# jdm365/SuffixArray

Hardware: AMD Instinct MI355X
Metric: sa_build_chars_per_s (higher is better)
Workload: dtype u8 text / u32 narrow keys / u32 suffix indices / i64 output

## Files before the change

### suffixarray_amd/csrc/big_build.hpp

```cpp
#pragma once
#include "sa_build.hpp"

namespace sa {
namespace big {

constexpr int BG_BLOCK = 512;
constexpr int BG_ITEMS = 16;
constexpr u32 BG_TILE = BG_BLOCK * BG_ITEMS;
constexpr int BG_WAVES = BG_BLOCK / WAVE;

__global__ __launch_bounds__(BG_BLOCK) void bg_hist_kernel(const u64* __restrict__ keys, u64 cnt, int shift, u32 ntiles, u32* __restrict__ th) {
    constexpr int CS = 257;
    __shared__ u32 s_h[8 * CS];
    for (int i = threadIdx.x; i < 8 * CS; i += BG_BLOCK) s_h[i] = 0;
    __syncthreads();
    u32* my = s_h + (threadIdx.x & 7) * CS;
    const u64 base = (u64)blockIdx.x * BG_TILE;
#pragma unroll 4
    for (int it = 0; it < BG_ITEMS; ++it) {
        const u64 j = base + (u64)it * BG_BLOCK + threadIdx.x;
        if (j < cnt) atomicAdd(&my[(u32)(keys[j] >> shift) & 255u], 1u);
    }
    sync_lds();
    if (threadIdx.x < 256) {
// ... 294 lines not shown
                ok = ea ? !eb : (!eb && inv[a + 1] < inv[b + 1]);
            }
        }
        if (!ok) atomicAdd(bad, 1ull);
    }
}

struct BigStats {
    u32 sigma = 0, bits_per_symbol = 0, initial_chars = 0, sort_passes = 0, rounds = 0;
    u64 tied_after_sort = 0, tied_total = 0;
    float total_ms = 0.f;
};

struct BigBuilder {
    hipStream_t stream = nullptr;
    DevBuf keysA, keysB, idxB, isa, th, off, part, fpart, small;
    DevBuf l_slot[2], l_idx[2], l_gid[2], r_key2, r_perm, r_k1, r_p1, r_gk, r_nk2;
    BigStats stats;

    void destroy() {
        DevBuf* all[] = {&keysA, &keysB, &idxB, &isa, &th, &off, &part, &fpart, &small, &l_slot[0], &l_slot[1], &l_idx[0], &l_idx[1], &l_gid[0],
                         &l_gid[1], &r_key2, &r_perm, &r_k1, &r_p1, &r_gk, &r_nk2};
        for (DevBuf* b : all) b->release();
    }
    ~BigBuilder() { destroy(); }

    int sort_pairs(u64* k0, u64* v0, u64* k1, u64* v1, u64 cnt, int bits, u64** kres, u64** vres) {
        *kres = k0; *vres = v0;
        if (cnt < 2 || bits <= 0) return 0;
        const u64 nt64 = (cnt + BG_TILE - 1) / BG_TILE;
        if (nt64 > 0x7FFFFFFFull) return fail(SA_HIP_EINVAL, "big sort: too many tiles");
        const u32 ntiles = (u32)nt64;
        const u64 len = (u64)RADIX * ntiles;
        const u64 nparts = (len + SC_TILE - 1) / SC_TILE;
        int rc;
        if ((rc = th.ensure(len * 4 + 64))) return rc;
        if ((rc = off.ensure(len * 8 + 64))) return rc;
        if ((rc = part.ensure((nparts + 1) * 8 + 64))) return rc;
        u64 *ki = k0, *vi = v0, *ko = k1, *vo = v1;
        for (int shift = 0; shift < bits; shift += 8) {
            hipLaunchKernelGGL(bg_hist_kernel, dim3(ntiles), dim3(BG_BLOCK), 0, stream, (const u64*)ki, cnt, shift, ntiles, th.as<u32>());
            hipLaunchKernelGGL(bg_scan_reduce_kernel, dim3((u32)nparts), dim3(SC_BLOCK), 0, stream, (const u32*)th.as<u32>(), len, part.as<u64>());
            hipLaunchKernelGGL(bg_scan_parts_kernel, dim3(1), dim3(SC_BLOCK), 0, stream, part.as<u64>(), nparts);
            hipLaunchKernelGGL(bg_scan_apply_kernel, dim3((u32)nparts), dim3(SC_BLOCK), 0, stream, (const u32*)th.as<u32>(), len, (const u64*)part.as<u64>(),
                               off.as<u64>());
            hipLaunchKernelGGL(bg_scatter_kernel, dim3(ntiles), dim3(BG_BLOCK), 0, stream, (const u64*)ki, (const u64*)vi, ko, vo, cnt, shift, ntiles,
                               (const u64*)off.as<u64>());
            u64* t = ki; ki = ko; ko = t;
            t = vi; vi = vo; vo = t;
            ++stats.sort_passes;
        }
        SA_HIP_CHECK(hipGetLastError());
        *kres = ki; *vres = vi;
        return 0;
    }

    int flags_pass(const u64* kA, const u64* kB, const u64* slot, const u64* idx, u64 m, int out, u64* m_out, u64* g_out) {
        const u64 nt64 = (m + BG_TILE - 1) / BG_TILE;
        if (nt64 > 0x7FFFFFFFull) return fail(SA_HIP_EINVAL, "big flags: too many tiles");
        const u32 ntiles = (u32)nt64;
        int rc;
        if ((rc = fpart.ensure(((size_t)ntiles + 1) * sizeof(FlagAgg) + 64))) return rc;
        FlagArgs a{};
        a.kA = kA; a.kB = kB; a.slot = slot; a.idx = idx; a.m = m; a.isa = isa.as<u64>();
        hipLaunchKernelGGL(bg_flags_reduce_kernel, dim3(ntiles), dim3(BG_BLOCK), 0, stream, a, fpart.as<FlagAgg>());
        hipLaunchKernelGGL(bg_flags_scan_kernel, dim3(1), dim3(BG_BLOCK), 0, stream, fpart.as<FlagAgg>(), (u64)ntiles);
        FlagAgg tot;
        SA_HIP_CHECK(hipMemcpyAsync(&tot, fpart.as<FlagAgg>() + ntiles, sizeof tot, hipMemcpyDeviceToHost, stream));
        SA_HIP_CHECK(hipStreamSynchronize(stream));
        *m_out = tot.nact; *g_out = tot.nhead;
        if ((rc = l_slot[out].ensure((size_t)tot.nact * 8 + 64))) return rc;
        if ((rc = l_idx[out].ensure((size_t)tot.nact * 8 + 64))) return rc;
        if ((rc = l_gid[out].ensure((size_t)tot.nact * 8 + 64))) return rc;
        a.out_slot = l_slot[out].as<u64>(); a.out_idx = l_idx[out].as<u64>(); a.out_gid = l_gid[out].as<u64>();
        hipLaunchKernelGGL(bg_flags_apply_kernel, dim3(ntiles), dim3(BG_BLOCK), 0, stream, a, (const FlagAgg*)fpart.as<FlagAgg>());
        SA_HIP_CHECK(hipGetLastError());
        return 0;
    }

    int build(const u8* text_dev, u64 n, u64* sa_out) {
        return build_with(n, sa_out, [&](u64* keys, u64* idx, int* key_bits, u64* h0) -> int {
            u64* dh = small.as<u64>();
            SA_HIP_CHECK(hipMemsetAsync(dh, 0, 256 * sizeof(u64), stream));
            hipLaunchKernelGGL(byte_hist_kernel, dim3(stream_grid(n, 256 * 64)), dim3(256), 0, stream, text_dev, n, dh);
            u64 freq[256];
            SA_HIP_CHECK(hipMemcpyAsync(freq, dh, sizeof freq, hipMemcpyDeviceToHost, stream));
            SA_HIP_CHECK(hipStreamSynchronize(stream));
            CodeMap map;
            memset(&map, 0, sizeof map);
            u32 sigma = 0;
            for (int c = 0; c < 256; ++c) if (freq[c]) map.code[c] = (u16)(++sigma);
            int b = bits_for((u64)sigma + 1);
            if (b == 0) b = 1;
            int k = 64 / b;
            if ((u64)k > n) k = (int)n;
            if (k < 1) k = 1;
            stats.sigma = sigma; stats.bits_per_symbol = (u32)b; stats.initial_chars = (u32)k;
            hipLaunchKernelGGL(bg_keygen_kernel, dim3((u32)((n + 4095) / 4096)), dim3(256), 0, stream, text_dev, n, map, b, k, keys, idx);
            *key_bits = k * b;
            *h0 = (u64)k;
            return 0;
        });
    }

    template <class KeyGen>
    int build_with(u64 n, u64* sa_out, KeyGen&& keygen) {
        stats = BigStats{};
        if (n == 0) return 0;
        int rc;
        hipEvent_t e0 = nullptr, e1 = nullptr;
        SA_HIP_CHECK(hipEventCreate(&e0));
        SA_HIP_CHECK(hipEventCreate(&e1));
        struct EvGuard { hipEvent_t a, b; ~EvGuard() { (void)hipEventDestroy(a); (void)hipEventDestroy(b); } } guard{e0, e1};
        if ((rc = small.ensure(4096))) return rc;
        if ((rc = keysA.ensure(n * 8 + 64))) return rc;
        if ((rc = keysB.ensure(n * 8 + 64))) return rc;
        if ((rc = idxB.ensure(n * 8 + 64))) return rc;
        if ((rc = isa.ensure(n * 8 + 64))) return rc;
        {
            const u64 ntiles = (n + BG_TILE - 1) / BG_TILE, len = (u64)RADIX * ntiles;
            if ((rc = th.ensure(len * 4 + 64)) || (rc = off.ensure(len * 8 + 64)) || (rc = part.ensure(((len + SC_TILE - 1) / SC_TILE + 1) * 8 + 64)) ||
                (rc = fpart.ensure((ntiles + 1) * sizeof(FlagAgg) + 64))) return rc;
        }
        SA_HIP_CHECK(hipEventRecord(e0, stream));
        int key_bits = 0;
        u64 h0 = 1;
        if ((rc = keygen(keysA.as<u64>(), sa_out, &key_bits, &h0))) return rc;
        if (h0 < 1) h0 = 1;
        u64 *kres, *vres;
        if ((rc = sort_pairs(keysA.as<u64>(), sa_out, keysB.as<u64>(), idxB.as<u64>(), n, key_bits, &kres, &vres))) return rc;
        if (vres != sa_out) SA_HIP_CHECK(hipMemcpyAsync(sa_out, vres, n * 8, hipMemcpyDeviceToDevice, stream));
        u64 M = 0, G = 0;
        int cur = 0;
        if ((rc = flags_pass(kres, nullptr, nullptr, sa_out, n, cur, &M, &G))) return rc;
        stats.tied_after_sort = M;
        keysA.release(); keysB.release(); idxB.release(); th.release(); off.release();
        const int rbits = bits_for(n + 2);
        for (u64 h = h0; M > 0; h *= 2) {
            stats.tied_total += M;
            ++stats.rounds;
            if ((rc = r_key2.ensure(M * 8 + 64)) || (rc = r_perm.ensure(M * 8 + 64)) || (rc = r_k1.ensure(M * 8 + 64)) || (rc = r_p1.ensure(M * 8 + 64)) ||
                (rc = r_gk.ensure(M * 8 + 64)) || (rc = r_nk2.ensure(M * 8 + 64))) return rc;
            const u32 grid = stream_grid(M, 1024);
            hipLaunchKernelGGL(bg_key2_kernel, dim3(grid), dim3(256), 0, stream, (const u64*)l_idx[cur].as<u64>(), M, n, h, (const u64*)isa.as<u64>(),
                               r_key2.as<u64>(), r_perm.as<u64>());
            SA_HIP_CHECK(hipMemcpyAsync(r_gk.p, r_key2.p, M * 8, hipMemcpyDeviceToDevice, stream));
            u64 *k1, *p1;
            if ((rc = sort_pairs(r_gk.as<u64>(), r_perm.as<u64>(), r_k1.as<u64>(), r_p1.as<u64>(), M, rbits, &k1, &p1))) return rc;
            u64* gk = (k1 == r_gk.as<u64>()) ? r_k1.as<u64>() : r_gk.as<u64>();
            u64* pfree = (p1 == r_perm.as<u64>()) ? r_p1.as<u64>() : r_perm.as<u64>();
            hipLaunchKernelGGL(bg_gather_kernel, dim3(grid), dim3(256), 0, stream, (const u64*)l_gid[cur].as<u64>(), (const u64*)p1, M, gk);
            u64 *k2, *p2;
            if ((rc = sort_pairs(gk, p1, k1, pfree, M, bits_for(G + 1), &k2, &p2))) return rc;
            const int nxt = cur ^ 1;
            if ((rc = l_idx[nxt].ensure(M * 8 + 64))) return rc;
            hipLaunchKernelGGL(bg_permute_kernel, dim3(grid), dim3(256), 0, stream, (const u64*)l_idx[cur].as<u64>(), (const u64*)r_key2.as<u64>(),
                               (const u64*)p2, (const u64*)l_slot[cur].as<u64>(), M, l_idx[nxt].as<u64>(), r_nk2.as<u64>(), sa_out);
            SA_HIP_CHECK(hipMemcpyAsync(r_perm.p, l_idx[nxt].p, M * 8, hipMemcpyDeviceToDevice, stream));
            u64 M2 = 0, G2 = 0;
            if ((rc = flags_pass(l_gid[cur].as<u64>(), r_nk2.as<u64>(), l_slot[cur].as<u64>(), r_perm.as<u64>(), M, nxt, &M2, &G2))) return rc;
            M = M2; G = G2; cur = nxt;
            if (h > n) break;
        }
        SA_HIP_CHECK(hipEventRecord(e1, stream));
        SA_HIP_CHECK(hipStreamSynchronize(stream));
        (void)hipEventElapsedTime(&stats.total_ms, e0, e1);
        if (M) return fail(SA_HIP_EHIP, "big build: rounds ended with tied suffixes");
// ... 27 lines not shown
```

### suffixarray_amd/csrc/common.hpp

```cpp
#pragma once
#include <hip/hip_runtime.h>
#include <cstdint>
#include <cstdio>
#include <cstdlib>
#include <cstring>
#include <string>
#include <new>

#include "../../include/sa_hip.h"

namespace sa {

using u8 = uint8_t;
using u16 = uint16_t;
using u32 = uint32_t;
using u64 = uint64_t;

constexpr int WAVE = 64;

inline std::string& last_error() {
    static thread_local std::string s;
    return s;
}
inline int fail(int code, const char* what, const char* detail = nullptr) {
    std::string& e = last_error();
    e = what;
    if (detail) { e += ": "; e += detail; }
    return code;
}

#define SA_HIP_CHECK(expr)                                                                 \
    do {                                                                                   \
        hipError_t _e = (expr);                                                            \
        if (_e != hipSuccess) {                                                            \
            char _b[256];                                                                  \
            snprintf(_b, sizeof _b, "%s:%d %s", __FILE__, __LINE__, hipGetErrorString(_e)); \
            return ::sa::fail(_e == hipErrorOutOfMemory ? SA_HIP_ENOMEM : SA_HIP_EHIP, #expr, _b); \
        }                                                                                  \
    } while (0)

__host__ __device__ inline u32 div_up(u64 a, u64 b) { return (u32)((a + b - 1) / b); }

__host__ __device__ __forceinline__ u32 hits_of_range(const sa_hip_pair_u32 rg) {
    return (rg.first != 0xFFFFFFFFu && (u32)(rg.second - rg.first + 1u) != 0u) ? rg.second - rg.first + 1u : 0u;
}

inline int bits_for(u64 count) {
    int b = 0;
    while (b < 64 && (1ull << b) < count) ++b;
    return b;
}

#if defined(__HIPCC__)
__device__ __forceinline__ u64 lanemask_lt() {
    return (1ull << (threadIdx.x & 63)) - 1ull;
}

__device__ __forceinline__ void sync_lds() {
    asm volatile("s_waitcnt lgkmcnt(0)" ::: "memory");
    __syncthreads();
}
#endif

struct HostU64Array {
    u64* p = nullptr;
    size_t n = 0;
    HostU64Array() = default;
    HostU64Array(const HostU64Array&) = delete;
    HostU64Array& operator=(const HostU64Array&) = delete;
    ~HostU64Array() { free(p); }
    void clear() { free(p); p = nullptr; n = 0; }
    void adopt(u64* malloced, size_t count) { clear(); p = malloced; n = count; }
    void assign(const u64* first, const u64* last) {
        const size_t count = (size_t)(last - first);
        u64* q = static_cast<u64*>(malloc((count ? count : 1) * sizeof(u64)));
        if (!q) throw std::bad_alloc();
        if (count) memcpy(q, first, count * sizeof(u64));
        clear(); p = q; n = count;
    }
    size_t size() const { return n; }
    bool empty() const { return n == 0; }
    const u64* data() const { return p; }
    const u64* begin() const { return p; }
    const u64* end() const { return p + n; }
    const u64& operator[](size_t i) const { return p[i]; }
    const u64& back() const { return p[n - 1]; }
};

inline const char* diag_env(const char* name) {
    static const bool on = [] { const char* d = getenv("SA_HIP_DIAG"); return d && atoi(d) != 0; }();
    return on ? getenv(name) : nullptr;
}

struct CodeMap {
    u16 code[256];
};

struct DeviceStatus {
    u32 error;
    u32 pad[3];
};

}
```

### suffixarray_amd/csrc/radix_narrow.hpp

```cpp
#pragma once
#include "radix_sort.hpp"
#include <vector>

namespace sa {

constexpr int NARROW_MAX_PASSES = 6;
constexpr int SEG_ITEMS = 24;

struct SegPlan {
    u32 bstart[RADIX + 1];
    u32 tprefix[RADIX + 1];
    u32 cfirst[NCHUNK + 1];
};

__global__ __launch_bounds__(256) void seg_plan_kernel(const u32* __restrict__ hist_top, u32 tile, SegPlan* __restrict__ plan) {
    __shared__ uint2 s_w[4];
    __shared__ u32 s_tp[RADIX + 1];
    const int d = threadIdx.x;
    u32 size = 0;
#pragma unroll
    for (int c = 0; c < NCHUNK; ++c) size += hist_top[c * RADIX + d];
    const u32 tiles = (u32)(((u64)size + tile - 1) / tile);
    uint2 tot;
    const uint2 ex = block_scan_excl<4>(make_uint2(size, tiles), make_uint2(0, 0), ScanSum{}, s_w, &tot);
// ... 195 lines not shown
        }
    }
    sync_lds();
    if (has_next) {
        for (int i = tid; i < RADIX; i += BLOCK) {
            const u32 v = s_whist[i];
            if (v) atomicAdd(&a.next_hist[bucket * RADIX + i], v);
        }
    }
    if (LATEV) load_vals();
    u32* s_vals = s_keys;
#pragma unroll
    for (int j = 0; j < ITEMS; ++j)
        if (FULL || (woff + j * WAVE) < tile_n) s_vals[pos[j]] = val[j];
    __syncthreads();
    if (LAST && a.vals_out64) {
#pragma unroll
        for (int k = 0; k < ITEMS; ++k) {
            const u32 p = k * BLOCK + tid;
            if (FULL || p < tile_n) { const u32 v = s_vals[p]; a.vals_out[gidx[k]] = v; a.vals_out64[gidx[k]] = (int64_t)v; }
        }
        return;
    }
#pragma unroll
    for (int k = 0; k < ITEMS; ++k) {
        const u32 p = k * BLOCK + tid;
        if (FULL || p < tile_n) a.vals_out[gidx[k]] = s_vals[p];
    }
}

template <int BLOCK, int ITEMS, bool LAST, bool LATEV = true>
__global__ __launch_bounds__(BLOCK, (ITEMS > 16) ? 4 : (LATEV ? 6 : 4)) void seg_onesweep_kernel(SegPassArgs a) {
    constexpr int WAVES = BLOCK / WAVE;
    constexpr u32 TILE = BLOCK * ITEMS;
    __shared__ __attribute__((aligned(16))) u32 s_keys[TILE];
    __shared__ u32 s_whist[WAVES * RADIX];
    __shared__ u32 s_gdelta[RADIX];
    __shared__ u32 s_wsum[RADIX / WAVE];
    __shared__ u32 s_t[RADIX + 1];
    __shared__ u32 s_b[RADIX + 1];
    __shared__ u32 s_c[NCHUNK + 1];
    __shared__ u32 s_flat;

    const int tid = threadIdx.x;
    u32 home = 0, t_home = 0;
    if (tid == 0) {
        home = xcc_id();
        t_home = atomicAdd(&a.ticket[home], 1u);
    }
    for (int i = tid; i <= RADIX; i += BLOCK) { s_t[i] = a.plan->tprefix[i]; s_b[i] = a.plan->bstart[i]; }
    if (tid <= NCHUNK) s_c[tid] = a.plan->cfirst[tid];
    for (int i = tid; i < WAVES * RADIX; i += BLOCK) s_whist[i] = 0;
    __syncthreads();
    if (tid == 0) {
        u32 flat = 0xFFFFFFFFu;
        if (t_home < s_c[home + 1] - s_c[home]) flat = s_c[home] + t_home;
        for (int k = 1; k < NCHUNK && flat == 0xFFFFFFFFu; ++k) {
            const u32 c = (home + k) & (NCHUNK - 1);
            const u32 cnt = s_c[c + 1] - s_c[c];
            if (cnt == 0) continue;
            const u32 t = atomicAdd(&a.ticket[c], 1u);
            if (t < cnt) flat = s_c[c] + t;
        }
        s_flat = flat;
    }
    __syncthreads();
    const u32 flat = s_flat;
    if (flat == 0xFFFFFFFFu) return;
    const u32 bucket = seg_bucket_of(s_t, flat);
    const u32 first_flat = s_t[bucket];
    const u32 start = s_b[bucket] + (flat - first_flat) * TILE;
    const u32 rest = s_b[bucket + 1] - start;
    if (rest >= TILE)
        seg_tile<true, BLOCK, ITEMS, LAST, LATEV>(a, flat, first_flat, bucket, start, TILE, s_keys, s_whist, s_gdelta, s_wsum);
    else
        seg_tile<false, BLOCK, ITEMS, LAST, LATEV>(a, flat, first_flat, bucket, start, rest, s_keys, s_whist, s_gdelta, s_wsum);
}

}
#include "radix_split.hpp"
namespace sa {

constexpr int TOP_HIST_COPIES = 8;
template <int C8>
__global__ __launch_bounds__(256) void top_hist_kernel(const u8* __restrict__ text, const u16* __restrict__ map, u64 n, int b,
                                                       SortGeom g, u32* __restrict__ hist, int low_k0 = 0) {
    constexpr int CS = RADIX + 1;
    constexpr u32 SPAN = 256 * 16;
    __shared__ u32 s_h[TOP_HIST_COPIES * CS];
    __shared__ u8 s_map[256];
    s_map[threadIdx.x] = (u8)map[threadIdx.x];
    for (int i = threadIdx.x; i < TOP_HIST_COPIES * CS; i += 256) s_h[i] = 0;
    __syncthreads();
    u32* my = s_h + (threadIdx.x & (TOP_HIST_COPIES - 1)) * CS;
    constexpr int c8 = C8;
    const u32 wmask = (1u << (c8 * b)) - 1u;
    const int dshift = c8 * b - 8;
    const u64 nspans = (n + SPAN - 1) / SPAN;
    const u64 per = (nspans + gridDim.x - 1) / gridDim.x;
    const u64 s_lo = (u64)blockIdx.x * per;
    const u64 s_hi = (s_lo + per < nspans) ? s_lo + per : nspans;
    auto flush = [&](u32 chunk) {
        sync_lds();
        u32 v = 0;
#pragma unroll
        for (int k = 0; k < TOP_HIST_COPIES; ++k) { v += s_h[k * CS + threadIdx.x]; s_h[k * CS + threadIdx.x] = 0; }
        if (v) atomicAdd(&hist[chunk * RADIX + threadIdx.x], v);
        sync_lds();
    };
    if (s_lo >= s_hi) return;
    u32 cur = chunk_of_tile((u32)((s_lo * SPAN) / g.tile), g.tpc);
    for (u64 sp = s_lo; sp < s_hi; ++sp) {
        const u64 base = sp * SPAN;
        const u32 c = chunk_of_tile((u32)(base / g.tile), g.tpc);
        if (c != cur) { flush(cur); cur = c; }
        const u64 p0 = base + (u64)threadIdx.x * 16;
        if (p0 < n) {
            const u64 off = low_k0 ? (u64)(low_k0 - c8) : 0;
            uint4 x0, x1;
            __builtin_memcpy(&x0, text + p0 + off, 16);
            __builtin_memcpy(&x1, text + p0 + off + 16, 16);
            const u32 w[8] = {x0.x, x0.y, x0.z, x0.w, x1.x, x1.y, x1.z, x1.w};
            const u64 first = p0 + off;
            const u32 live = (first >= n) ? 0u : ((n - first < 32) ? (u32)(n - first) : 32u);
            const u32 npos = (n - p0 < 16) ? (u32)(n - p0) : 16u;
            u32 win = 0;
#pragma unroll
            for (int k = 0; k < 16 + c8 - 1; ++k) {
                const u32 byte = (w[k >> 2] >> ((k & 3) * 8)) & 255u;
                const u32 code = ((u32)k < live) ? (u32)s_map[byte] : 0u;
                win = ((win << b) | code) & wmask;
                const int i = k - (c8 - 1);
                if (i >= 0 && (u32)i < npos) atomicAdd(&my[low_k0 ? (win & 255u) : (win >> dshift)], 1u);
            }
        }
    }
    flush(cur);
}

struct TextPassArgs {
    const u8* text;
    const u16* map;
    u64 n;
    int b, k0, begin_bit;
    u32* keys_out32;
    u16* ext_out16;
    u32* vals_out;
    SortGeom g;
    const u32* digit_base;
    u64* status;
    u32* ticket;
    u32 epoch;
    DeviceStatus* dstat;
    u32 incl_mask;
    u32* cursor;
    int owned;
};
constexpr u32 TOP_CURSOR_STRIDE = 64;
constexpr int TEXT_HALO = 64;
#ifndef SA_TEXT_ITEMS
#define SA_TEXT_ITEMS 16
#endif
constexpr int TEXT_ITEMS = SA_TEXT_ITEMS;
constexpr u32 TEXT_TILE = 512u * TEXT_ITEMS;

__device__ __forceinline__ void shl_or_inplace(u32& acc, u32 x, int s) {
    asm("v_lshl_or_b32 %0, %1, %2, %0" : "+v"(acc) : "v"(x), "s"(s));
}

template <bool FULL, int BLOCK, bool EXT, bool CLAIM = false>
__device__ __forceinline__ void text_top_tile(const TextPassArgs& a, const u32 tile, const u32 chunk,
                                              const u32 tile_n, u32* s_keys, u32* s_whist, u32* s_gdelta, u32* s_wsum,
                                              u8* s_code, const u8* s_map, u16* s_ext) {
    constexpr int WAVES = BLOCK / WAVE;
    constexpr int ITEMS = TEXT_ITEMS;
    constexpr u32 TILE = BLOCK * ITEMS;
    static_assert(TILE % 16 == 0, "16-byte text loads");
    const int tid = threadIdx.x, lane = tid & 63, wave = tid >> 6;
    const u32 first_tile = chunk * a.g.tpc;
    const u64 tile_base = (u64)tile * TILE;
    const u32 woff = (u32)wave * (WAVE * ITEMS) + lane;

    const u32 dbase = (tid < RADIX) ? a.digit_base[(CLAIM ? 0u : chunk) * RADIX + tid] : 0u;

    auto stage16 = [&](u32 local, auto checked) {
        constexpr bool CHECK = decltype(checked)::value;
        const u64 p0 = tile_base + local;
        uint4 x = make_uint4(0, 0, 0, 0);
        if (!CHECK || p0 < a.n) x = *reinterpret_cast<const uint4*>(a.text + p0);
        const u32 w[4] = {x.x, x.y, x.z, x.w};
        const u32 live = CHECK ? (u32)((a.n > p0) ? ((a.n - p0 < 16) ? (a.n - p0) : 16) : 0) : 16u;
        u32 o[4] = {0, 0, 0, 0};
#pragma unroll
        for (int k = 0; k < 16; ++k) {
            const u32 byte = (w[k >> 2] >> ((k & 3) * 8)) & 255u;
            const u32 code = (!CHECK || (u32)k < live) ? (u32)s_map[byte] : 0u;
            o[k >> 2] |= code << ((k & 3) * 8);
        }
        *reinterpret_cast<uint4*>(s_code + local) = make_uint4(o[0], o[1], o[2], o[3]);
    };
    for (u32 local = (u32)tid * 16u; local < TILE; local += BLOCK * 16u) {
        if (FULL) stage16(local, std::false_type{}); else stage16(local, std::true_type{});
    }
    if (tid < TEXT_HALO / 16) stage16(TILE + (u32)tid * 16u, std::true_type{});
    __syncthreads();

    u32 hi[ITEMS], lo[ITEMS];
#pragma unroll
    for (int j = 0; j < ITEMS; ++j) { hi[j] = 0; lo[j] = 0; }
    const u8* cp = s_code + woff;
    {
        int c = 0;
        for (; c < a.k0 && 64 - a.b * (c + 1) >= 32; ++c, ++cp) {
            const int s_hi = 32 - a.b * (c + 1);
#pragma unroll
            for (int j = 0; j < ITEMS; ++j) shl_or_inplace(hi[j], (u32)cp[j * WAVE], s_hi);
        }
        if (c < a.k0 && 64 - a.b * c > 32) {
            const int sh = 64 - a.b * (c + 1);
#pragma unroll
            for (int j = 0; j < ITEMS; ++j) {
                const u32 code = cp[j * WAVE];
                hi[j] |= code >> (32 - sh);
                lo[j] |= code << sh;
            }
            ++c; ++cp;
        }
        for (; c < a.k0; ++c, ++cp) {
            const int sh = 64 - a.b * (c + 1);
#pragma unroll
            for (int j = 0; j < ITEMS; ++j) shl_or_inplace(lo[j], (u32)cp[j * WAVE], sh);
        }
    }
    u32 key[ITEMS];
    u32 ext[EXT ? ITEMS : 1];
    const int kb0 = EXT ? a.begin_bit + 16 : a.begin_bit;
#pragma unroll
    for (int j = 0; j < ITEMS; ++j) {
        key[j] = (kb0 >= 32) ? (hi[j] >> (kb0 - 32)) : __builtin_amdgcn_alignbit(hi[j], lo[j], (u32)kb0);
// ... 28 lines not shown
    if (tid < RADIX) {
        for (int i = 0; i < wave; ++i) excl += s_wsum[i];
#pragma unroll
        for (int w = 0; w < WAVES; ++w) s_whist[w * RADIX + tid] += excl;
    }
    __syncthreads();

    u8* s_dig = s_code;
    u32 pos[ITEMS];
#pragma unroll
    for (int j = 0; j < ITEMS; ++j) {
        const u32 d = rd[j] >> 16;
        pos[j] = wh[d] + (rd[j] & 0xFFFFu);
        if (FULL || (woff + j * WAVE) < tile_n) {
            s_keys[pos[j]] = key[j]; s_dig[pos[j]] = (u8)d;
            if (EXT) s_ext[pos[j]] = (u16)ext[j];
        }
    }
    __syncthreads();

    if (tid < RADIX) {
        u32 prefix = claim;
        if (!CLAIM && tile > first_tile) {
            prefix = lookback_prefix(a.status, tile, first_tile, (u32)tid, a.epoch, a.dstat);
            if (((tile - first_tile) & a.incl_mask) == a.incl_mask)
                __hip_atomic_store(&a.status[(u64)tile * RADIX + tid], pack_status(a.epoch, FLAG_INCL, prefix + count),
                                   __ATOMIC_RELAXED, __HIP_MEMORY_SCOPE_AGENT);
        }
        s_gdelta[tid] = dbase + prefix - excl;
    }
    __syncthreads();

    u32 gidx[ITEMS];
#pragma unroll
    for (int k = 0; k < ITEMS; ++k) {
        const u32 p = k * BLOCK + tid;
        if (FULL || p < tile_n) {
            gidx[k] = s_gdelta[s_dig[p]] + p;
            a.keys_out32[gidx[k]] = s_keys[p];
            if (EXT) a.ext_out16[gidx[k]] = s_ext[p];
        }
    }
    __syncthreads();
    u32* s_vals = s_keys;
#pragma unroll
    for (int j = 0; j < ITEMS; ++j)
        if (FULL || (woff + j * WAVE) < tile_n) s_vals[pos[j]] = (u32)tile_base + woff + j * WAVE;
    __syncthreads();
#pragma unroll
    for (int k = 0; k < ITEMS; ++k) {
        const u32 p = k * BLOCK + tid;
        if (FULL || p < tile_n) a.vals_out[gidx[k]] = s_vals[p];
    }
}

constexpr int TOP_OWNED_W = 24;
constexpr int TOP_OWNED_KMAX = TOP_OWNED_W - 15;
constexpr int TOP_FINE_BITS = 3;
constexpr u32 TOP_FINE_BINS = (u32)RADIX << TOP_FINE_BITS;
inline bool text_owned_applies(int b, int k0) { return k0 >= 1 && k0 <= TOP_OWNED_KMAX && b * k0 >= 8 + TOP_FINE_BITS && b * k0 <= 40; }

template <bool FULL, int BLOCK>
__device__ __forceinline__ void text_top_owned_tile(const TextPassArgs& a, const u32 tile, const u32 chunk, const u32 tile_n, u32* s_keys,
                                                    u32* s_fine, u32* s_gdelta, u32* s_wsum, u8* s_dig, const u8* s_map) {
    constexpr int ITEMS = 16, W = TOP_OWNED_W, F = TOP_FINE_BITS;
    constexpr u32 TILE = BLOCK * ITEMS;
    static_assert(TEXT_ITEMS == ITEMS, "the tiles of the pass's geometry");
    static_assert(TOP_FINE_BINS == 4u * BLOCK, "four fine bins per thread");
    static_assert((TILE & (TILE - 1)) == 0 && TILE <= (1u << 13) && 8 + F + 13 <= 32, "(fine bin, rank) in one register");
    static_assert(W % 4 == 0 && W > 16 && W <= 32, "a 16-byte load and a shorter one");
    const int tid = threadIdx.x, lane = tid & 63, wave = tid >> 6;
    const u64 tile_base = (u64)tile * TILE;
    const u32 own = (u32)tid * ITEMS;

    const u32 cd = chunk * RADIX + (u32)(tid >> 1);
    const u32 dbase = (tid & 1) ? 0u : a.digit_base[cd];

    const long long start = (long long)(tile_base + own) + (a.k0 - (W - 15));
    const long long n = (long long)a.n;
    u32 x[W / 4];
#pragma unroll
    for (int i = 0; i < W / 4; ++i) x[i] = 0;
    if (start >= 0) {
        if (FULL || start < n) __builtin_memcpy(&x[0], a.text + start, 16);
        if (FULL || start + 16 < n) __builtin_memcpy(&x[4], a.text + start + 16, W - 16);
    } else {
#pragma unroll
        for (int i = 0; i < W; ++i) {
            const long long q = start + i;
            if (q >= 0 && q < n) x[i >> 2] |= (u32)a.text[q] << ((i & 3) * 8);
        }
    }
    const u32 live = FULL ? (u32)W : (u32)((start >= n) ? 0 : ((n - start < W) ? (n - start) : W));

    const u32 up = 32u - (u32)a.b;
    const u32 fshift = (u32)(a.b * a.k0 - 8 - F);
    const u32 kmask = (a.b * a.k0 >= 32) ? 0xFFFFFFFFu : ((1u << (a.b * a.k0)) - 1u);
    u32 whi = 0, wlo = 0;
    u32 key[ITEMS], pk[ITEMS];
#pragma unroll
    for (int i = 0; i < W; ++i) {
        const u32 byte = (x[i >> 2] >> ((i & 3) * 8)) & 255u;
        const u32 code = (FULL || (u32)i < live) ? (u32)s_map[byte] : 0u;
        whi = __builtin_amdgcn_alignbit(whi, wlo, up);
        wlo = (wlo << a.b) | code;
        if (i >= W - ITEMS) {
            const int j = i - (W - ITEMS);
            key[j] = wlo & kmask;
            const u32 fine = __builtin_amdgcn_alignbit(whi, wlo, fshift) & (TOP_FINE_BINS - 1u);
            const u32 slot = (FULL || own + (u32)j < tile_n) ? fine : TOP_FINE_BINS;
            pk[j] = (fine << 13) | atomicAdd(&s_fine[slot], 1u);
        }
    }
    sync_lds();

    const uint4 c = *reinterpret_cast<const uint4*>(s_fine + 4 * tid);
    const u32 tot = c.x + c.y + c.z + c.w;
    const u32 dcount = tot + __shfl_xor(tot, 1);
    u32 claim = 0;
    if (!(tid & 1) && dcount) claim = atomicAdd(&a.cursor[cd * TOP_CURSOR_STRIDE], dcount);
    const u32 incl = wave_scan_incl(tot, ScanSum{});
    if (lane == 63) s_wsum[wave] = incl;
    __syncthreads();
    u32 excl = incl - tot;
    for (int i = 0; i < wave; ++i) excl += s_wsum[i];
    *reinterpret_cast<uint4*>(s_fine + 4 * tid) = make_uint4(excl, excl + c.x, excl + c.x + c.y, excl + c.x + c.y + c.z);
    __syncthreads();

    u32 pos[ITEMS];
#pragma unroll
    for (int j = 0; j < ITEMS; ++j) {
        const u32 fine = pk[j] >> 13;
        pos[j] = (s_fine[fine] + (pk[j] & 0x1FFFu)) & (TILE - 1u);
        if (FULL || own + (u32)j < tile_n) { s_keys[pos[j]] = key[j]; s_dig[pos[j]] = (u8)(fine >> F); }
    }
    if (!(tid & 1)) s_gdelta[tid >> 1] = dbase + claim - excl;
    __syncthreads();

    u32 gidx[ITEMS];
#pragma unroll
    for (int k = 0; k < ITEMS; ++k) {
        const u32 p = k * BLOCK + tid;
        if (FULL || p < tile_n) {
            gidx[k] = s_gdelta[s_dig[p]] + p;
            a.keys_out32[gidx[k]] = s_keys[p];
        }
    }
    __syncthreads();
    u32* s_vals = s_keys;
#pragma unroll
    for (int j = 0; j < ITEMS; ++j)
        if (FULL || own + (u32)j < tile_n) s_vals[pos[j]] = (u32)tile_base + own + (u32)j;
    __syncthreads();
#pragma unroll
    for (int k = 0; k < ITEMS; ++k) {
        const u32 p = k * BLOCK + tid;
        if (FULL || p < tile_n) a.vals_out[gidx[k]] = s_vals[p];
    }
}

template <int BLOCK, bool EXT = false, bool CLAIM = false>
__global__ __launch_bounds__(BLOCK, (TEXT_ITEMS > 16 || EXT) ? 4 : 6) void text_top_pass_kernel(TextPassArgs a) {
    constexpr int WAVES = BLOCK / WAVE;
    constexpr u32 TILE = BLOCK * TEXT_ITEMS;
    __shared__ __attribute__((aligned(16))) u32 s_keys[TILE];
    __shared__ __attribute__((aligned(16))) u32 s_whist[WAVES * RADIX + 4];
    __shared__ u32 s_gdelta[RADIX];
    __shared__ u32 s_wsum[WAVES];
// ... 189 lines not shown
            }
        }
    }
    sync_lds();
    if (has_next) {
        for (int i = tid; i < NCHUNK * RADIX; i += BLOCK) {
            const u32 v = s_whist[i];
            if (v) atomicAdd(&a.next_hist[i], v);
        }
    }
    u32* s_vals = reinterpret_cast<u32*>(s_keys);
#pragma unroll
    for (int j = 0; j < ITEMS; ++j)
        if (FULL || (woff + j * WAVE) < tile_n) s_vals[pos[j]] = (u32)tile_base + woff + j * WAVE;
    __syncthreads();
#pragma unroll
    for (int k = 0; k < ITEMS; ++k) {
        const u32 p = k * BLOCK + tid;
        if (FULL || p < tile_n) a.vals_out[gidx[k]] = s_vals[p];
    }
}

template <int BLOCK>
__global__ __launch_bounds__(BLOCK, 4) void text_low_pass_kernel(TextLowArgs t) {
    constexpr int WAVES = BLOCK / WAVE;
    constexpr u32 TILE = BLOCK * SORT_ITEMS;
    constexpr int WH = (WAVES * RADIX > NCHUNK * RADIX) ? WAVES * RADIX : NCHUNK * RADIX;
    static_assert(TILE * 8 >= TILE + TEXT_HALO, "the staged codes fit the key array's LDS");
    __shared__ __attribute__((aligned(16))) u64 s_keys[TILE];
    __shared__ u32 s_whist[WH];
    __shared__ uint2 s_tab[RADIX];
    __shared__ u32 s_wsum[RADIX / WAVE];
    __shared__ u8 s_map[256];
    __shared__ u32 s_tile;
    __shared__ u32 s_chunk;
    const SortPassArgs& a = t.p;
    const int tid = threadIdx.x;
    if (tid == 0) {
        u32 tile = 0xFFFFFFFFu, chunk = 0;
        const u32 home = xcc_id();
        for (int k = 0; k < NCHUNK; ++k) {
            const u32 c = (home + k) & (NCHUNK - 1);
            const u32 first = c * a.g.tpc;
            if (first >= a.g.tiles) continue;
            const u32 cnt = (a.g.tiles - first) < a.g.tpc ? (a.g.tiles - first) : a.g.tpc;
            const u32 x = atomicAdd(&a.ticket[c], 1u);
            if (x < cnt) { tile = first + x; chunk = c; break; }
        }
        s_tile = tile;
        s_chunk = chunk;
    }
    if (tid < 256) s_map[tid] = (u8)t.map[tid];
    for (int i = tid; i < WAVES * RADIX; i += BLOCK) s_whist[i] = 0;
    __syncthreads();
    const u32 tile = s_tile;
    if (tile == 0xFFFFFFFFu) return;
    const u32 chunk = s_chunk;
    const u64 rest = t.n - (u64)tile * TILE;
    if (rest >= (u64)TILE)
        text_low_tile<true, BLOCK>(t, tile, chunk, TILE, s_keys, s_whist, s_tab, s_wsum, s_map);
    else
        text_low_tile<false, BLOCK>(t, tile, chunk, (u32)rest, s_keys, s_whist, s_tab, s_wsum, s_map);
}

struct NarrowWorkspace {
    SegPlan* plan = nullptr;
    u32* hist = nullptr;
    u32* base = nullptr;
    u32* tickets = nullptr;
    u16* map_dev = nullptr;
    CodeMap map_host;
    bool split_enabled = true;
    u32* split_hist = nullptr;
    u32* split_base = nullptr;
    u32* split_cursor = nullptr;
    u32* top_cursor = nullptr;
    static size_t top_cursor_bytes() { return (size_t)NCHUNK * RADIX * TOP_CURSOR_STRIDE * sizeof(u32); }
    bool top_claims = true;
    bool top_owned = true;
    u32* split_sub = nullptr;
    u32* host_word = nullptr;
    static size_t split_table_bytes() { return (size_t)RADIX * SPLIT_NB * sizeof(u32); }
    static size_t split_sub_words() { return ((size_t)RADIX << SPLIT_BITS) + 1; }
    u32* split_levels_dev() const { return split_sub + split_sub_words(); }
    u32 split_cap = LOCAL_CAP;
    int local_bin_bits = 12;
    bool split_flags = true;
    bool local_big = false;
    bool local_persist = true;
    u32 local_grid_force = 0;
    u32 local_grid[6] = {};
    int persist_grid(const void* kernel, int block, int slot, u32 nsub, u32* grid) {
        if (!local_grid[slot]) {
            int dev = 0, cus = 0, per_cu = 0;
            SA_HIP_CHECK(hipGetDevice(&dev));
            SA_HIP_CHECK(hipDeviceGetAttribute(&cus, hipDeviceAttributeMultiprocessorCount, dev));
            SA_HIP_CHECK(hipOccupancyMaxActiveBlocksPerMultiprocessor(&per_cu, kernel, block, 0));
            local_grid[slot] = (u32)((per_cu > 0 ? per_cu : 1) * (cus > 0 ? cus : 1));
        }
        const u32 g = local_grid_force ? local_grid_force : local_grid[slot];
        *grid = g < nsub ? g : nsub;
        return 0;
    }
    int split_items = 28;
    static size_t hist_bytes() { return (size_t)NARROW_MAX_PASSES * RADIX * RADIX * sizeof(u32); }
    int init() {
        SA_HIP_CHECK(hipMalloc(&plan, sizeof(SegPlan)));
        SA_HIP_CHECK(hipMalloc(&hist, hist_bytes()));
        SA_HIP_CHECK(hipMalloc(&base, (size_t)RADIX * RADIX * sizeof(u32)));
        SA_HIP_CHECK(hipMalloc(&tickets, (size_t)NARROW_MAX_PASSES * NCHUNK * sizeof(u32)));
        SA_HIP_CHECK(hipMalloc(&map_dev, sizeof(CodeMap)));
        SA_HIP_CHECK(hipMalloc(&split_hist, split_table_bytes()));
        SA_HIP_CHECK(hipMalloc(&split_base, split_table_bytes()));
        SA_HIP_CHECK(hipMalloc(&split_cursor, split_table_bytes()));
        SA_HIP_CHECK(hipMalloc(&top_cursor, top_cursor_bytes()));
        SA_HIP_CHECK(hipMalloc(&split_sub, (split_sub_words() + 16) * sizeof(u32)));
        SA_HIP_CHECK(hipHostMalloc(reinterpret_cast<void**>(&host_word), 64, hipHostMallocDefault));
        if (const char* e = diag_env("SA_HIP_SPLIT")) split_enabled = atoi(e) != 0;
        if (const char* e = diag_env("SA_HIP_TOP_CLAIMS")) top_claims = atoi(e) != 0;
        if (const char* e = diag_env("SA_HIP_TOP_OWNED")) top_owned = atoi(e) != 0;
        if (const char* e = diag_env("SA_HIP_LOCAL_BIG")) local_big = atoi(e) != 0;
        if (const char* e = diag_env("SA_HIP_LOCAL_PERSIST")) local_persist = atoi(e) != 0;
        if (const char* e = diag_env("SA_HIP_LOCAL_GRID")) { const int v = atoi(e); local_grid_force = v > 0 ? (u32)v : 0u; }
        if (const char* e = diag_env("SA_HIP_SPLIT_FLAGS")) split_flags = atoi(e) != 0;
        if (const char* e = diag_env("SA_HIP_LOCAL_BINS")) local_bin_bits = (atoi(e) == 11) ? 11 : 12;
        if (const char* e = diag_env("SA_HIP_SPLIT_ITEMS")) { const int v = atoi(e); split_items = (v == 24 || v == 28) ? v : 32; }
        if (const char* e = diag_env("SA_HIP_SPLIT_CAP")) { const int v = atoi(e); if (v >= 64 && v <= (int)LOCAL_CAP) split_cap = (u32)v; }
        return 0;
    }
    void destroy() {
        if (plan) (void)hipFree(plan);
        if (hist) (void)hipFree(hist);
        if (base) (void)hipFree(base);
        if (tickets) (void)hipFree(tickets);
        if (map_dev) (void)hipFree(map_dev);
        if (split_hist) (void)hipFree(split_hist);
        if (split_base) (void)hipFree(split_base);
        if (split_cursor) (void)hipFree(split_cursor);
        if (top_cursor) (void)hipFree(top_cursor);
        if (split_sub) (void)hipFree(split_sub);
        if (host_word) (void)hipHostFree(host_word);
        map_dev = nullptr;
        plan = nullptr; hist = nullptr; base = nullptr; tickets = nullptr;
        split_hist = split_base = split_sub = split_cursor = top_cursor = nullptr; host_word = nullptr;
    }
};

inline bool narrow_sort_applies(const RadixWorkspace& ws, u64 n, int begin_bit) {
    return ws.block == 512 && begin_bit >= 24 && begin_bit < 56 && n >= (1u << 22) &&
           n / ws.tile() + RADIX + 1 <= ws.max_tiles;
}

struct TextSource {
    const u8* text;
    int b, k0;
};
inline bool text_pass_applies(int b, int k0) { return b <= 8 && k0 - 1 <= TEXT_HALO; }

inline int text_histogram(RadixWorkspace& ws, NarrowWorkspace& nw, hipStream_t stream, const u8* text, const CodeMap& map,
                          u32 n, int b, u32 tile, int low_k0) {
    nw.map_host = map;
    SA_HIP_CHECK(hipMemcpyAsync(nw.map_dev, nw.map_host.code, sizeof(CodeMap), hipMemcpyHostToDevice, stream));
    const SortGeom g = make_geom(n, tile);
    const u32 spans = div_up(n, 4096);
    const dim3 grid(spans < 2048u ? spans : 2048u), block(256);
    decltype(&top_hist_kernel<1>) kernel;
    switch ((8 + b - 1) / b) {
        case 1: kernel = top_hist_kernel<1>; break;
        case 2: kernel = top_hist_kernel<2>; break;
        case 3: kernel = top_hist_kernel<3>; break;
        case 4: kernel = top_hist_kernel<4>; break;
        default: kernel = top_hist_kernel<8>; break;
    }
    hipLaunchKernelGGL(kernel, grid, block, 0, stream, text, nw.map_dev, (u64)n, b, g, ws.hist(0), low_k0);
    return 0;
}

struct WideTextCtx {
    const u8* text;
    const u16* map;
    u64 n;
    int b, k0;
};
inline void launch_text_low_pass(void* ctx, hipStream_t stream, const SortPassArgs& a, u32 grid) {
    const WideTextCtx* c = static_cast<const WideTextCtx*>(ctx);
    TextLowArgs t;
    t.p = a; t.text = c->text; t.map = c->map; t.n = c->n; t.b = c->b; t.k0 = c->k0;
    hipLaunchKernelGGL((text_low_pass_kernel<512>), dim3(grid), dim3(512), 0, stream, t);
}

enum TopForm { TOP_STABLE, TOP_CLAIM, TOP_EXT };
inline int launch_text_top(RadixWorkspace& ws, NarrowWorkspace& nw, hipStream_t stream, const TextSource& src, u32 n, int begin_bit,
                           TopForm form, u32* keys_out32, u16* ext_out16, u32* vals_out) {
    const bool claim = form == TOP_CLAIM, ext = form == TOP_EXT;
    const SortGeom g = make_geom(n, TEXT_TILE);
    TextPassArgs t;
    t.text = src.text; t.map = nw.map_dev; t.n = n; t.b = src.b; t.k0 = src.k0; t.begin_bit = begin_bit;
    t.keys_out32 = keys_out32; t.ext_out16 = ext_out16; t.vals_out = vals_out; t.g = g; t.digit_base = ws.base();
    t.status = ws.status; t.ticket = ws.tickets(); t.epoch = ws.epoch; t.dstat = ws.dstat; t.incl_mask = SA_INCL_MASK;
    t.cursor = ext ? nullptr : nw.top_cursor;
    t.owned = (claim && nw.top_owned && TEXT_ITEMS == 16 && text_owned_applies(src.b, src.k0)) ? 1 : 0;
    if (claim) SA_HIP_CHECK(hipMemsetAsync(nw.top_cursor, 0, NarrowWorkspace::top_cursor_bytes(), stream));
    return ws.timed_pass(stream, 1, n, (u64)n * (ext ? 11u : 9u), [&] {
        if (claim) hipLaunchKernelGGL((text_top_pass_kernel<512, false, true>), dim3(g.tiles), dim3(512), 0, stream, t);
        else if (!ext) hipLaunchKernelGGL((text_top_pass_kernel<512>), dim3(g.tiles), dim3(512), 0, stream, t);
        else hipLaunchKernelGGL((text_top_pass_kernel<512, true>), dim3(g.tiles), dim3(512), 0, stream, t);
    });
}

struct NarrowSortResult {
    u64* keys = nullptr;
    u32* vals = nullptr;
    int rb = 0;
    u32 max_group = 0;
    bool flags_done = false;
};

inline int narrow_top_digit(RadixWorkspace& ws, NarrowWorkspace& nw, hipStream_t stream, const u64* keys_in, u32* keys_out32, u32* vals_out,
                            u32 n, int begin_bit, const TextSource* src, bool claim) {
    int rc;
    if ((rc = ws.next_epoch(stream))) return rc;
    hipLaunchKernelGGL(radix_scan_hist_kernel, dim3(1), dim3(256), 0, stream, ws.hist(0), ws.base());
    if (src) return launch_text_top(ws, nw, stream, *src, n, begin_bit, claim ? TOP_CLAIM : TOP_STABLE, keys_out32, nullptr, vals_out);
    SortPassArgs a;
    a.keys_in = keys_in; a.vals_in = nullptr; a.keys_out = nullptr; a.vals_out = vals_out;
    a.g = make_geom(n, ws.tile()); a.shift = 56; a.mask = 255u; a.next_shift = -1; a.next_mask = 0; a.digit_base = ws.base();
    a.next_hist = nullptr; a.status = ws.status; a.ticket = ws.tickets(); a.epoch = ws.epoch; a.dstat = ws.dstat;
    a.home_mode = 0; a.incl_mask = SA_INCL_MASK;
    a.keys_out32 = keys_out32; a.narrow_shift = begin_bit;
    return ws.timed_pass(stream, 1, n, (u64)n * 16u, [&] {
        hipLaunchKernelGGL((radix_onesweep_kernel<512, 0, true>), dim3(a.g.tiles), dim3(512), 0, stream, a);
    });
}

struct SplitKernels {
    using Hist = decltype(&split_hist_kernel<512, 24>);
    using Split = decltype(&seg_split_kernel<512, 24>);
    Hist hist;
    Split split;
};
inline SplitKernels split_kernels(int split_items) {
    const int i = (split_items == 32) ? 0 : (split_items == 28) ? 1 : 2;
    static const SplitKernels::Hist hist[3] = {split_hist_kernel<512, 32>, split_hist_kernel<512, 28>, split_hist_kernel<512, 24>};
    static const SplitKernels::Split split[3] = {seg_split_kernel<512, 32>, seg_split_kernel<512, 28>, seg_split_kernel<512, 24>};
    return {hist[i], split[i]};
}

struct SplitLevel {
    int rb;
    bool big;
};
inline SplitLevel choose_split_level(const u32* host_word, int hb, int lo_bits, u32 split_cap, bool local_big) {
    int rb = -1;
    bool big = local_big;
    if (!big)
        for (int k = 1; k <= hb; ++k)
            if (host_word[k] <= split_cap) { rb = k; break; }
    if (rb < 0 && split_cap == LOCAL_CAP) {
        for (int k = 1; k <= hb; ++k)
            if (host_word[k] <= LOCAL_CAP_BIG && lo_bits - k >= 12) { rb = k; big = true; break; }
        if (rb < 0) big = false;
    }
    return {rb, big};
}

inline int narrow_plan_look(NarrowWorkspace& nw, hipStream_t stream, const u32* keys32, int lo_bits, int hb, u32 split_flat_max,
                            SplitLevel* level) {
    SA_HIP_CHECK(hipMemsetAsync(nw.split_hist, 0, NarrowWorkspace::split_table_bytes(), stream));
    SA_HIP_CHECK(hipMemsetAsync(nw.split_levels_dev(), 0, 16 * sizeof(u32), stream));
    const u32 tpb = 4;
    hipLaunchKernelGGL(split_kernels(nw.split_items).hist, dim3(div_up(split_flat_max, tpb)), dim3(512), 0, stream, keys32, nw.plan,
                       lo_bits - hb, (1u << hb) - 1u, nw.split_hist, tpb);
    hipLaunchKernelGGL(split_levels_kernel, dim3(RADIX), dim3(SPLIT_NB), 0, stream, (const u32*)nw.split_hist, hb, nw.split_levels_dev());
    SA_HIP_CHECK(hipMemcpyAsync(nw.host_word, nw.split_levels_dev(), 16 * sizeof(u32), hipMemcpyDeviceToHost, stream));
    SA_HIP_CHECK(hipStreamSynchronize(stream));
    *level = choose_split_level(nw.host_word, hb, lo_bits, nw.split_cap, nw.local_big);
    return 0;
}

inline int narrow_split_pass(RadixWorkspace& ws, NarrowWorkspace& nw, hipStream_t stream, const u32* keys_in, const u32* vals_in,
                             u32* keys_out, u32* vals_out, u32 n, int lo_bits, int hb, int rb, u32 split_flat_max) {
    int rc;
    hipLaunchKernelGGL(split_scan_kernel, dim3(RADIX), dim3(SPLIT_NB), 0, stream, (const u32*)nw.split_hist, nw.plan, hb, rb,
                       nw.split_base, nw.split_sub);
    SA_HIP_CHECK(hipMemsetAsync(nw.split_cursor, 0, NarrowWorkspace::split_table_bytes(), stream));
    if ((rc = ws.next_epoch(stream))) return rc;
    SplitPassArgs a;
    a.keys_in = keys_in; a.vals_in = vals_in;
    a.keys_out = keys_out; a.vals_out = vals_out;
    a.plan = nw.plan; a.shift = lo_bits - rb; a.mask = (1u << rb) - 1u; a.digit_base = nw.split_base;
    a.ticket = nw.tickets; a.cursor = nw.split_cursor;
    return ws.timed_pass(stream, 2, n, (u64)n * 16u, [&] {
        hipLaunchKernelGGL(split_kernels(nw.split_items).split, dim3(split_flat_max), dim3(512), 0, stream, a);
    });
}

struct LocalKernels {
    using Persist = decltype(&local_persist_kernel<12, true>);
    using Finish = decltype(&local_finish_kernel<12, true>);
    Persist persist;
    Finish finish;
    int block, row;
};
inline LocalKernels local_kernels(bool big, bool flags, int bb) {
    const int row = big ? (flags ? 0 : 1) : 2 + (flags ? 0 : 2) + (bb == 12 ? 0 : 1);
    static const LocalKernels::Persist persist[6] = {
        local_persist_kernel<12, true, LOCAL_BLOCK_BIG>, local_persist_kernel<12, false, LOCAL_BLOCK_BIG>,
        local_persist_kernel<12, true>, local_persist_kernel<11, true>, local_persist_kernel<12, false>, local_persist_kernel<11, false>};
    static const LocalKernels::Finish finish[6] = {
        local_finish_kernel<12, true, LOCAL_BLOCK_BIG>, local_finish_kernel<12, false, LOCAL_BLOCK_BIG>,
        local_finish_kernel<12, true>, local_finish_kernel<11, true>, local_finish_kernel<12, false>, local_finish_kernel<11, false>};
    return {persist[row], finish[row], big ? LOCAL_BLOCK_BIG : LOCAL_BLOCK, row};
}

inline int narrow_local_pass(RadixWorkspace& ws, NarrowWorkspace& nw, hipStream_t stream, const u32* keys_in, const u32* vals_in,
                             u32* keys_out, u32* vals_out, int64_t* vals_out64, u32 n, int begin_bit, int rb, bool big,
                             const LocalFlagsRequest* flags_req, bool* flags_done) {
    int rc;
    const int lo_bits = 56 - begin_bit;
    const int rest_bits = lo_bits - rb;
    LocalArgs l;
    l.keys_in = keys_in; l.vals_in = vals_in;
    l.keys_out = keys_out; l.vals_out = vals_out; l.vals_out64 = vals_out64;
    l.sub = nw.split_sub;
    const int bb = (big || (rest_bits >= 12 && nw.local_bin_bits == 12)) ? 12 : 11;
    l.bin_shift = rest_bits - bb;
    l.dstat = ws.dstat;
    l.dir = DirArgs{}; l.counts = nullptr; l.lite = LiteArgs{}; l.lo_shift = begin_bit; l.rb = rb; l.n = n;
    const u32 nsub = (u32)RADIX << rb;
    bool with_flags = false;
    if (nw.split_flags && flags_req && flags_req->prepare) {
        const int fr = flags_req->prepare(flags_req->ctx, nsub, &l);
        if (fr < 0) return fr;
        with_flags = (fr == 0) && l.dir.dir && l.dir.dbits >= 8 + rb && l.dir.dbits - 8 - rb <= bb && l.dir.dbits - 8 <= lo_bits;
    }
    const LocalKernels k = local_kernels(big, with_flags, bb);
    u32 pgrid = 0;
    if (nw.local_persist && (rc = nw.persist_grid(reinterpret_cast<const void*>(k.persist), k.block, k.row, nsub, &pgrid))) return rc;
    rc = ws.timed_pass(stream, 3, n, (u64)n * 16u + (vals_out64 ? (u64)n * 8u : 0u), [&] {
        if (nw.local_persist) hipLaunchKernelGGL(k.persist, dim3(pgrid), dim3(k.block), 0, stream, l, (const u32*)nw.split_sub, nsub, nw.tickets + NCHUNK, LOCAL_RUN);
        else hipLaunchKernelGGL(k.finish, dim3(nsub), dim3(k.block), 0, stream, l);
    });
    if (rc) return rc;
    *flags_done = with_flags;
    SA_HIP_CHECK(hipGetLastError());
    return 0;
}

inline int split_debug_check(NarrowWorkspace& nw, hipStream_t stream, const u32* keys_split, const u32* keys_out, const u32* vals_out,
                             u32 n, int lo_bits, int hb, int rb) {
    const int dshift = lo_bits - rb;
    const u32 dmask = (1u << rb) - 1u;
    const u32 nsub = (u32)RADIX << rb;
    std::vector<u32> sub(nsub + 1), k1(n), k2(n), v2(n), bst(RADIX + 1);
    SA_HIP_CHECK(hipStreamSynchronize(stream));
    SA_HIP_CHECK(hipMemcpy(sub.data(), nw.split_sub, (size_t)(nsub + 1) * 4, hipMemcpyDeviceToHost));
    SA_HIP_CHECK(hipMemcpy(k1.data(), keys_split, (size_t)n * 4, hipMemcpyDeviceToHost));
    SA_HIP_CHECK(hipMemcpy(k2.data(), keys_out, (size_t)n * 4, hipMemcpyDeviceToHost));
    SA_HIP_CHECK(hipMemcpy(v2.data(), vals_out, (size_t)n * 4, hipMemcpyDeviceToHost));
    SA_HIP_CHECK(hipMemcpy(bst.data(), nw.plan->bstart, (size_t)(RADIX + 1) * 4, hipMemcpyDeviceToHost));
    u64 bad_sub = 0, bad_split = 0, bad_sorted = 0, bad_mono = 0;
    u32 first_split = ~0u, first_sorted = ~0u;
    for (u32 i = 0; i < nsub; ++i) {
        if (sub[i] > sub[i + 1] || sub[i + 1] > n) { ++bad_mono; continue; }
        if ((i & (((u32)1 << rb) - 1)) == 0 && sub[i] != bst[i >> rb]) ++bad_sub;
        for (u32 j = sub[i]; j < sub[i + 1]; ++j) {
            if (((k1[j] >> dshift) & dmask) != (i & dmask)) { ++bad_split; if (first_split == ~0u) first_split = j; }
            if (j > sub[i] && (k2[j - 1] > k2[j] || (k2[j - 1] == k2[j] && v2[j - 1] >= v2[j]))) { ++bad_sorted; if (first_sorted == ~0u) first_sorted = j; }
        }
    }
    fprintf(stderr, "[sa_hip] split debug: n=%u rb=%d hb=%d nsub=%u sub[0]=%u sub[last]=%u | table: %llu not monotone, %llu off the bucket starts | split pass: %llu records in the wrong group (first %u) | local pass: %llu out of order (first %u)\n",
            n, rb, hb, nsub, sub[0], sub[nsub], (unsigned long long)bad_mono, (unsigned long long)bad_sub, (unsigned long long)bad_split, first_split,
            (unsigned long long)bad_sorted, first_sorted);
    return 0;
}

inline int narrow_declined(RadixWorkspace& ws, NarrowWorkspace& nw, hipStream_t stream, u32* keys_out32, u32* vals_out, u32 n,
                           int begin_bit, const TextSource* src, bool top_claimed, u32 split_tile_n, u32 seg_tile_n) {
    int rc;
    if (top_claimed) {
        SA_HIP_CHECK(hipMemsetAsync(ws.tickets(), 0, NCHUNK * sizeof(u32), stream));
        if ((rc = ws.next_epoch(stream))) return rc;
        if ((rc = launch_text_top(ws, nw, stream, *src, n, begin_bit, TOP_STABLE, keys_out32, nullptr, vals_out))) return rc;
    }
    if (split_tile_n != seg_tile_n)
        hipLaunchKernelGGL(seg_plan_kernel, dim3(1), dim3(256), 0, stream, ws.hist(0), seg_tile_n, nw.plan);
    return 0;
}

inline int narrow_lsd_passes(RadixWorkspace& ws, NarrowWorkspace& nw, hipStream_t stream, u64* keysA, u32* valsA, u64* keysB, u32* valsB,
                             u32 n, int begin_bit, bool keep_narrow, int64_t* vals_res64, NarrowSortResult* res) {
    int rc;
    const int lo_bits = 56 - begin_bit;
    const int np = (lo_bits + RADIX_BITS - 1) / RADIX_BITS;
    const u32 flat_max = n / (512u * SEG_ITEMS) + 1 + RADIX;
    SA_HIP_CHECK(hipMemsetAsync(nw.hist, 0, NarrowWorkspace::hist_bytes(), stream));
    {
        const u32 tpb = 4;
        const u32 mask0 = (1u << ((np == 1) ? lo_bits : RADIX_BITS)) - 1u;
        hipLaunchKernelGGL((seg_hist_kernel<512, SEG_ITEMS>), dim3(div_up(flat_max, tpb)), dim3(512), 0, stream,
                           reinterpret_cast<const u32*>(keysB), nw.plan, 0, mask0, nw.hist, tpb);
    }
    u32* kin = reinterpret_cast<u32*>(keysB); u32* vin = valsB;
    u32* kout = reinterpret_cast<u32*>(keysA); u32* vout = valsA;
    for (int p = 0; p < np; ++p) {
        if ((rc = ws.next_epoch(stream))) return rc;
        const bool last = (p == np - 1);
        const int bits_p = last ? (lo_bits - RADIX_BITS * (np - 1)) : RADIX_BITS;
        hipLaunchKernelGGL(seg_scan_kernel, dim3(RADIX), dim3(256), 0, stream, nw.hist + (size_t)p * RADIX * RADIX, nw.plan, nw.base);
        SegPassArgs a;
        a.keys_in = kin; a.vals_in = vin; a.keys_out = kout; a.keys_out64 = keep_narrow ? nullptr : reinterpret_cast<u64*>(kout);
        a.vals_out = vout;
        a.vals_out64 = last ? vals_res64 : nullptr;
        a.plan = nw.plan;
        a.shift = RADIX_BITS * p;
        a.mask = (1u << bits_p) - 1u;
        a.next_shift = last ? -1 : RADIX_BITS * (p + 1);
        const int bits_n = (p + 1 == np - 1) ? (lo_bits - RADIX_BITS * (np - 1)) : RADIX_BITS;
        a.next_mask = last ? 0u : ((1u << bits_n) - 1u);
        a.digit_base = nw.base;
        a.next_hist = last ? nullptr : nw.hist + (size_t)(p + 1) * RADIX * RADIX;
        a.status = ws.status; a.ticket = nw.tickets + p * NCHUNK; a.epoch = ws.epoch; a.dstat = ws.dstat;
        a.lo_shift = begin_bit; a.incl_mask = SA_INCL_MASK;
        const u64 pass_bytes = (u64)n * ((last && !keep_narrow) ? 20u : 16u) + ((last && vals_res64) ? (u64)n * 8u : 0u);
        rc = ws.timed_pass(stream, last ? 3 : 2, n, pass_bytes, [&] {
            if (last) hipLaunchKernelGGL((seg_onesweep_kernel<512, SEG_ITEMS, true>), dim3(flat_max), dim3(512), 0, stream, a);
            else hipLaunchKernelGGL((seg_onesweep_kernel<512, SEG_ITEMS, false>), dim3(flat_max), dim3(512), 0, stream, a);
        });
        if (rc) return rc;
        std::swap(kin, kout);
        std::swap(vin, vout);
    }
    SA_HIP_CHECK(hipGetLastError());
    res->keys = reinterpret_cast<u64*>(kin);
    res->vals = vin;
    return 0;
}

inline int radix_sort_narrow(RadixWorkspace& ws, NarrowWorkspace& nw, hipStream_t stream, u64* keysA, u32* valsA, u64* keysB,
                             u32* valsB, u32 n, int begin_bit, NarrowSortResult* res, const TextSource* src = nullptr,
                             bool keep_narrow = false, int64_t* vals_res64 = nullptr, const LocalFlagsRequest* flags_req = nullptr) {
    int rc;
    *res = NarrowSortResult{};
    const int lo_bits = 56 - begin_bit;
    u32* const k32A = reinterpret_cast<u32*>(keysA);
    u32* const k32B = reinterpret_cast<u32*>(keysB);
    SA_HIP_CHECK(hipMemsetAsync(nw.tickets, 0, (size_t)NARROW_MAX_PASSES * NCHUNK * sizeof(u32), stream));
    const bool try_split = nw.split_enabled && keep_narrow && ws.block == 512 && lo_bits - LOCAL_BIN_BITS >= 1;
    const bool optimistic = try_split && src && nw.top_claims;
    if ((rc = narrow_top_digit(ws, nw, stream, keysA, k32B, valsB, n, begin_bit, src, optimistic))) return rc;
    const u32 seg_tile_n = 512u * SEG_ITEMS;
    const u32 split_tile_n = 512u * (u32)nw.split_items;
    hipLaunchKernelGGL(seg_plan_kernel, dim3(1), dim3(256), 0, stream, ws.hist(0), try_split ? split_tile_n : seg_tile_n, nw.plan);
    if (try_split) {
        const int hb = (lo_bits - LOCAL_BIN_BITS < SPLIT_BITS) ? lo_bits - LOCAL_BIN_BITS : SPLIT_BITS;
        const u32 split_flat_max = n / split_tile_n + 1 + RADIX;
        SplitLevel lv;
        if ((rc = narrow_plan_look(nw, stream, k32B, lo_bits, hb, split_flat_max, &lv))) return rc;
        res->max_group = nw.host_word[lv.rb > 0 ? lv.rb : hb];
        if (lv.rb > 0) {
            if ((rc = narrow_split_pass(ws, nw, stream, k32B, valsB, k32A, valsA, n, lo_bits, hb, lv.rb, split_flat_max))) return rc;
            if ((rc = narrow_local_pass(ws, nw, stream, k32A, valsA, k32B, valsB, vals_res64, n, begin_bit, lv.rb, lv.big, flags_req,
                                        &res->flags_done))) return rc;
            if (diag_env("SA_HIP_SPLIT_DEBUG") && (rc = split_debug_check(nw, stream, k32A, k32B, valsB, n, lo_bits, hb, lv.rb))) return rc;
            res->rb = lv.rb;
            res->keys = keysB;
            res->vals = valsB;
            return 0;
        }
        if ((rc = narrow_declined(ws, nw, stream, k32B, valsB, n, begin_bit, src, optimistic, split_tile_n, seg_tile_n))) return rc;
    }
    return narrow_lsd_passes(ws, nw, stream, keysA, valsA, keysB, valsB, n, begin_bit, keep_narrow, vals_res64, res);
}

}
```

### suffixarray_amd/csrc/radix_split.hpp

```cpp
#pragma once
#include "flags_common.hpp"

namespace sa {

#ifndef SA_ABL
#define SA_ABL 0
#endif
constexpr int SPLIT_BITS = 10;
constexpr int SPLIT_NB = 1 << SPLIT_BITS;
constexpr u32 LOCAL_CAP = 8192;
constexpr int LOCAL_BLOCK = 512;
constexpr int LOCAL_ITEMS = (int)(LOCAL_CAP / LOCAL_BLOCK);
constexpr u32 LOCAL_CAP_BIG = 16384;
constexpr int LOCAL_BLOCK_BIG = 1024;
constexpr u32 LOCAL_RUN = 8;
constexpr int LOCAL_BIN_BITS = 11;
constexpr int SPLIT_HIST_COPIES = 4;

template <int BLOCK, int ITEMS>
__global__ __launch_bounds__(BLOCK) void split_hist_kernel(const u32* __restrict__ keys, const SegPlan* __restrict__ plan, int shift,
                                                           u32 mask, u32* __restrict__ hist, u32 tiles_per_block) {
    constexpr u32 TILE = BLOCK * ITEMS;
    constexpr int CS = SPLIT_NB + 1;
    __shared__ u32 s_h[SPLIT_HIST_COPIES * CS];
    __shared__ u32 s_t[RADIX + 1];
    for (int i = threadIdx.x; i <= RADIX; i += BLOCK) s_t[i] = plan->tprefix[i];
    for (int i = threadIdx.x; i < SPLIT_HIST_COPIES * CS; i += BLOCK) s_h[i] = 0;
    __syncthreads();
    const u32 F = s_t[RADIX];
    const u32 f_lo = blockIdx.x * tiles_per_block;
    const u32 f_hi = (f_lo + tiles_per_block < F) ? f_lo + tiles_per_block : F;
    if (f_lo >= f_hi) return;
    u32* my = s_h + (threadIdx.x & (SPLIT_HIST_COPIES - 1)) * CS;
    auto flush = [&](u32 bucket) {
        sync_lds();
        for (int d = threadIdx.x; d < SPLIT_NB; d += BLOCK) {
            u32 v = 0;
#pragma unroll
            for (int k = 0; k < SPLIT_HIST_COPIES; ++k) { v += s_h[k * CS + d]; s_h[k * CS + d] = 0; }
            if (v) atomicAdd(&hist[bucket * SPLIT_NB + d], v);
        }
        sync_lds();
    };
    u32 cur = seg_bucket_of(s_t, f_lo);
    for (u32 f = f_lo; f < f_hi; ++f) {
        const u32 b = seg_bucket_of(s_t, f);
        if (b != cur) { flush(cur); cur = b; }
        const u32 start = plan->bstart[b] + ((f - s_t[b]) * TILE);
        const u32 end = plan->bstart[b + 1];
        const u32 len = (end - start) < TILE ? (end - start) : TILE;
        if (len == TILE) {
            u32 k[ITEMS];
#pragma unroll
            for (int j = 0; j < ITEMS; ++j) k[j] = keys[start + j * BLOCK + threadIdx.x];
#pragma unroll
            for (int j = 0; j < ITEMS; ++j) atomicAdd(&my[(k[j] >> shift) & mask], 1u);
        } else {
            for (u32 l = threadIdx.x; l < len; l += BLOCK) atomicAdd(&my[(keys[start + l] >> shift) & mask], 1u);
        }
    }
    flush(cur);
}

__global__ __launch_bounds__(SPLIT_NB) void split_levels_kernel(const u32* __restrict__ hist, int hb, u32* __restrict__ levels) {
    __shared__ u32 s_p[SPLIT_NB + 1];
    __shared__ u32 s_w[SPLIT_NB / WAVE];
    const int b = blockIdx.x, d = threadIdx.x, lane = d & 63, w = d >> 6;
    const u32 c = hist[b * SPLIT_NB + d];
    s_p[d + 1] = block_scan_excl<SPLIT_NB / WAVE>(c, 0u, ScanSum{}, s_w) + c;
    if (d == 0) s_p[0] = 0;
    __syncthreads();
    __shared__ u32 s_lv[SPLIT_BITS + 1][SPLIT_NB / WAVE];
    for (int k = 0; k <= hb; ++k) {
        const int g = hb - k;
        u32 v = 0;
        if (d < (1 << k)) v = s_p[(d + 1) << g] - s_p[d << g];
#pragma unroll
        for (int o = 32; o > 0; o >>= 1) { const u32 t = __shfl_down(v, o); v = t > v ? t : v; }
        if (lane == 0) s_lv[k][w] = v;
    }
    __syncthreads();
    if (d <= hb) {
        u32 v = 0;
        for (int i = 0; i < SPLIT_NB / WAVE; ++i) v = s_lv[d][i] > v ? s_lv[d][i] : v;
        if (v) atomicMax(&levels[d], v);
    }
}

__global__ __launch_bounds__(SPLIT_NB) void split_scan_kernel(const u32* __restrict__ hist, const SegPlan* __restrict__ plan, int hb, int rb,
                                                              u32* __restrict__ base, u32* __restrict__ sub) {
    __shared__ u32 s_w[SPLIT_NB / WAVE];
    const int b = blockIdx.x, d = threadIdx.x;
    const u32 run = plan->bstart[b] + block_scan_excl<SPLIT_NB / WAVE>(hist[b * SPLIT_NB + d], 0u, ScanSum{}, s_w);
    const int g = hb - rb;
    u32 out = 0;
    if (d < (1 << hb) && (d & ((1 << g) - 1)) == 0) {
        out = run;
        sub[((u32)b << rb) + (u32)(d >> g)] = run;
    }
    __shared__ u32 s_o[SPLIT_NB];
    s_o[d] = 0;
    __syncthreads();
    if (d < (1 << hb) && (d & ((1 << g) - 1)) == 0) s_o[d >> g] = out;
    __syncthreads();
    base[b * SPLIT_NB + d] = s_o[d];
    if (d == 0 && b == RADIX - 1) sub[(u32)RADIX << rb] = plan->bstart[RADIX];
}

struct SplitPassArgs {
    const u32* keys_in;
    const u32* vals_in;
    u32* keys_out;
    u32* vals_out;
    const SegPlan* plan;
    int shift;
    u32 mask;
    const u32* digit_base;
    u32* ticket;
    u32* cursor;
};

template <bool FULL, int BLOCK, int ITEMS>
__device__ __forceinline__ void split_tile(const SplitPassArgs& a, const u32 bucket, const u32 start, const u32 tile_n,
                                           u32* s_keys, u32* s_cnt, u32* s_gdelta, u32* s_wsum) {
    static_assert(SPLIT_NB == 2 * BLOCK, "two bins per thread");
    const int tid = threadIdx.x, lane = tid & 63, wave = tid >> 6;
    const u32 woff = (u32)wave * (WAVE * ITEMS) + lane;

    const uint2 dbase = *reinterpret_cast<const uint2*>(a.digit_base + (size_t)bucket * SPLIT_NB + 2 * tid);

    u32 key[ITEMS];
    const u32* kin = a.keys_in + start;
#pragma unroll
    for (int j = 0; j < ITEMS; ++j) {
        const u32 p = woff + j * WAVE;
        key[j] = (FULL || p < tile_n) ? kin[p] : 0u;
    }
    u32 pos[ITEMS];
#pragma unroll
    for (int j = 0; j < ITEMS; ++j) {
        const u32 d = (key[j] >> a.shift) & a.mask;
        pos[j] = atomicAdd(&s_cnt[(FULL || (woff + j * WAVE) < tile_n) ? d : (u32)SPLIT_NB], 1u);
    }
    sync_lds();

    const uint2 c = *reinterpret_cast<const uint2*>(s_cnt + 2 * tid);
    u32 claim0 = 0, claim1 = 0;
    {
        const u32 ci = bucket * SPLIT_NB + 2u * (u32)tid;
        if (c.x) claim0 = atomicAdd(&a.cursor[ci], c.x);
        if (c.y) claim1 = atomicAdd(&a.cursor[ci + 1], c.y);
    }
    const u32 tot = c.x + c.y;
    const u32 incl = wave_scan_incl(tot, ScanSum{});
    if (lane == 63) s_wsum[wave] = incl;
    __syncthreads();
    u32 excl = incl - tot;
    for (int i = 0; i < wave; ++i) excl += s_wsum[i];
    *reinterpret_cast<uint2*>(s_cnt + 2 * tid) = make_uint2(excl, excl + c.x);
    __syncthreads();

#pragma unroll
    for (int j = 0; j < ITEMS; ++j) {
        pos[j] += s_cnt[(key[j] >> a.shift) & a.mask];
        if (FULL || (woff + j * WAVE) < tile_n) s_keys[pos[j]] = key[j];
    }
    __syncthreads();

    *reinterpret_cast<uint2*>(s_gdelta + 2 * tid) = make_uint2(dbase.x + claim0 - excl, dbase.y + claim1 - (excl + c.x));
    __syncthreads();

    static_assert(ITEMS % 2 == 0 && BLOCK * ITEMS <= 65536, "positions packed as 16-bit pairs");
    u32 pp[ITEMS / 2];
#pragma unroll
    for (int j = 0; j < ITEMS / 2; ++j) pp[j] = pos[2 * j] | (pos[2 * j + 1] << 16);
    u32 gidx[ITEMS];
#pragma unroll
    for (int k = 0; k < ITEMS; ++k) {
        const u32 p = k * BLOCK + tid;
        if (FULL || p < tile_n) {
            const u32 kk = s_keys[p];
            gidx[k] = s_gdelta[(kk >> a.shift) & a.mask] + p;
            a.keys_out[gidx[k]] = kk;
        }
    }
    u32 val[ITEMS];
    const u32* vin = a.vals_in + start;
#pragma unroll
    for (int j = 0; j < ITEMS; ++j) {
        const u32 p = woff + j * WAVE;
        val[j] = (FULL || p < tile_n) ? vin[p] : 0u;
    }
    __syncthreads();
    u32* s_vals = s_keys;
#pragma unroll
    for (int j = 0; j < ITEMS; ++j)
        if (FULL || (woff + j * WAVE) < tile_n) s_vals[(pp[j >> 1] >> ((j & 1) * 16)) & 0xFFFFu] = val[j];
    __syncthreads();
#pragma unroll
    for (int k = 0; k < ITEMS; ++k) {
        const u32 p = k * BLOCK + tid;
        if (FULL || p < tile_n) a.vals_out[gidx[k]] = s_vals[p];
    }
}

template <int BLOCK, int ITEMS>
__global__ __launch_bounds__(BLOCK, 4) void seg_split_kernel(SplitPassArgs a) {
    constexpr u32 TILE = BLOCK * ITEMS;
    __shared__ __attribute__((aligned(16))) u32 s_keys[TILE];
    __shared__ __attribute__((aligned(16))) u32 s_cnt[SPLIT_NB + 4];
    __shared__ __attribute__((aligned(16))) u32 s_gdelta[SPLIT_NB];
    __shared__ u32 s_wsum[BLOCK / WAVE];
    __shared__ u32 s_t[RADIX + 1];
    __shared__ u32 s_b[RADIX + 1];
    __shared__ u32 s_c[NCHUNK + 1];
    __shared__ u32 s_flat;

    const int tid = threadIdx.x;
    u32 home = 0, t_home = 0;
    if (tid == 0) {
        home = xcc_id();
        t_home = atomicAdd(&a.ticket[home], 1u);
    }
    for (int i = tid; i <= RADIX; i += BLOCK) { s_t[i] = a.plan->tprefix[i]; s_b[i] = a.plan->bstart[i]; }
    if (tid <= NCHUNK) s_c[tid] = a.plan->cfirst[tid];
    for (int i = tid; i < SPLIT_NB + 4; i += BLOCK) s_cnt[i] = 0;
    __syncthreads();
    if (tid == 0) {
        u32 flat = 0xFFFFFFFFu;
        if (t_home < s_c[home + 1] - s_c[home]) flat = s_c[home] + t_home;
        for (int k = 1; k < NCHUNK && flat == 0xFFFFFFFFu; ++k) {
            const u32 c = (home + k) & (NCHUNK - 1);
            const u32 cnt = s_c[c + 1] - s_c[c];
            if (cnt == 0) continue;
            const u32 t = atomicAdd(&a.ticket[c], 1u);
            if (t < cnt) flat = s_c[c] + t;
        }
        s_flat = flat;
    }
    __syncthreads();
    const u32 flat = s_flat;
    if (flat == 0xFFFFFFFFu) return;
    const u32 bucket = seg_bucket_of(s_t, flat);
    const u32 first_flat = s_t[bucket];
    const u32 start = s_b[bucket] + (flat - first_flat) * TILE;
    const u32 rest = s_b[bucket + 1] - start;
    if (rest >= TILE) split_tile<true, BLOCK, ITEMS>(a, bucket, start, TILE, s_keys, s_cnt, s_gdelta, s_wsum);
    else split_tile<false, BLOCK, ITEMS>(a, bucket, start, rest, s_keys, s_cnt, s_gdelta, s_wsum);
}

struct LocalArgs {
    const u32* keys_in;
    const u32* vals_in;
    u32* keys_out;
    u32* vals_out;
    int64_t* vals_out64;
    const u32* sub;
    int bin_shift;
    DeviceStatus* dstat;
    DirArgs dir;
    uint2* counts;
    LiteArgs lite;
    int lo_shift;
    int rb;
    u32 n;
};

struct LocalFlagsRequest {
    int (*prepare)(void* ctx, u32 nsub, LocalArgs* l) = nullptr;
    void* ctx = nullptr;
};

template <int BB, bool FLAGS, int BLOCK, bool PERSIST, typename Mid>
__device__ __forceinline__ void local_finish_sub(const LocalArgs& a, const u32 sb, const u32 s, const u32 m, u32 (&key)[LOCAL_ITEMS],
                                                 u32 (&val)[LOCAL_ITEMS], u64* s_rec, u32* s_cw, u32* s_wsum, Mid&& mid) {
    constexpr int ITEMS = LOCAL_ITEMS;
    constexpr int NB = 1 << BB, WORDS = NB / 2, WPT = WORDS / BLOCK;
    const int tid = threadIdx.x, lane = tid & 63, wave = tid >> 6;
    const int g2 = FLAGS ? a.dir.dbits - 8 - a.rb : 0;
    const u32 dfirst = FLAGS ? (sb << g2) : 0u;
    const u32 nd = FLAGS ? (1u << g2) : 0u;

    u32 r[ITEMS];
#pragma unroll
    for (int j = 0; j < ITEMS; ++j) {
        const u32 p = (u32)j * BLOCK + tid;
        r[j] = 0;
        if ((u32)j * BLOCK < m && p < m) {
            const u32 b = (key[j] >> a.bin_shift) & (u32)(NB - 1);
            const u32 sh = (b & 1u) * 16u;
            r[j] = (atomicAdd(&s_cw[b >> 1], 1u << sh) >> sh) & 0xFFFFu;
        }
    }
    sync_lds();

    {
        u32 cw[WPT];
        u32 tot = 0;
#pragma unroll
        for (int i = 0; i < WPT; ++i) { cw[i] = s_cw[WPT * tid + i]; tot += (cw[i] & 0xFFFFu) + (cw[i] >> 16); }
        const u32 incl = wave_scan_incl(tot, ScanSum{});
        if (lane == 63) s_wsum[wave] = incl;
        __syncthreads();
        u32 run = incl - tot;
        for (int i = 0; i < wave; ++i) run += s_wsum[i];
#pragma unroll
        for (int i = 0; i < WPT; ++i) {
            const u32 c0 = cw[i] & 0xFFFFu, c1 = cw[i] >> 16;
            s_cw[WPT * tid + i] = run | ((run + c0) << 16);
            run += c0 + c1;
        }
        if (tid == BLOCK - 1) s_cw[WORDS] = m;
    }
    __syncthreads();
    const u16* s_st = reinterpret_cast<const u16*>(s_cw);

#pragma unroll
    for (int j = 0; j < ITEMS; ++j) {
        const u32 p = (u32)j * BLOCK + tid;
        if ((u32)j * BLOCK < m && p < m) {
            const u32 slot = (u32)s_st[(key[j] >> a.bin_shift) & (u32)(NB - 1)] + r[j];
            s_rec[slot] = ((u64)key[j] << 32) | (u64)val[j];
        }
    }
    __syncthreads();
    if (FLAGS && !(SA_ABL & 1)) for (u32 e = tid; e < nd; e += BLOCK) a.dir.dir[dfirst + e] = s + (u32)s_st[e << (BB - g2)];

    u64 rec[ITEMS];
#pragma unroll
    for (int j = 0; j < ITEMS; ++j) {
        const u32 p = (u32)j * BLOCK + tid;
        rec[j] = 0; r[j] = 0;
        if ((u32)j * BLOCK < m && p < m) {
            const u64 x = s_rec[p];
            const u32 bin = ((u32)(x >> 32) >> a.bin_shift) & (u32)(NB - 1);
            const u32 lo = s_st[bin], hi = s_st[bin + 1];
            u32 cnt = 0;
            for (u32 q = lo; q < hi; q += 2) {
                const u64 y0 = s_rec[q], y1 = s_rec[q + 1];
                cnt += (y0 < x) ? 1u : 0u;
                cnt += (q + 1 < hi && y1 < x) ? 1u : 0u;
            }
            rec[j] = x;
            r[j] = lo + cnt;
        }
    }
    __syncthreads();
    if (PERSIST) {
#pragma unroll
        for (int i = 0; i < WPT; ++i) s_cw[WPT * tid + i] = 0;
    }
#pragma unroll
    for (int j = 0; j < ITEMS; ++j) {
        const u32 p = (u32)j * BLOCK + tid;
        if ((u32)j * BLOCK < m && p < m) s_rec[r[j]] = rec[j];
    }
    if (FLAGS && tid == 0) { const u64 ones = ~(u64)(m >> 31); s_rec[m] = ones; }
    __syncthreads();
    mid();

    auto stage_pair = [&](u32 p) {
        const u64 x = s_rec[p], xn = s_rec[p + 1];
        const bool starts = (p == 0) || ((u32)(s_rec[p - 1] >> 32) != (u32)(x >> 32));
        u32 at = atomicAdd(&a.counts[sb].x, starts ? 2u : 1u);
        if (at + (starts ? 2u : 1u) > LITE_CAP) __hip_atomic_store(a.lite.overflow, 1u, __ATOMIC_RELAXED, __HIP_MEMORY_SCOPE_AGENT);
        if (starts) {
            atomicAdd(&a.counts[sb].y, 1u);
            if (at < LITE_CAP) {
                const u64 row = (u64)sb * LITE_CAP + at;
                a.lite.st_pos[row] = s + p; a.lite.st_idx[row] = (u32)x; a.lite.st_head[row] = 1;
            }
            ++at;
        }
        if (at < LITE_CAP) {
            const u64 row = (u64)sb * LITE_CAP + at;
            a.lite.st_pos[row] = s + p + 1; a.lite.st_idx[row] = (u32)xn; a.lite.st_head[row] = 0;
        }
    };
    if (FLAGS) {
        if (!(SA_ABL & 4))
        for (u32 p = (u32)tid * 16u + 15u; p + 1 < m; p += (u32)BLOCK * 16u)
            if ((u32)(s_rec[p] >> 32) == (u32)(s_rec[p + 1] >> 32)) stage_pair(p);
    }
    u32 tmask = 0;
#pragma unroll
    for (int j = 0; j < ITEMS; ++j) {
        const u32 p = (u32)j * BLOCK + tid;
        if ((u32)j * BLOCK < m) {
            const u64 x = s_rec[p];
            const u32 k = (u32)(x >> 32);
            if (p < m) {
                a.keys_out[s + p] = k;
                a.vals_out[s + p] = (u32)x;
                if (a.vals_out64) a.vals_out64[s + p] = (int64_t)(u32)x;
            }
            if (FLAGS && !(SA_ABL & 2)) {
                const u32 kn = (u32)__builtin_amdgcn_update_dpp((int)~k, (int)k, 0x101, 0xF, 0xF, false);
                tmask |= (kn == k && p + 1 < m) ? (1u << j) : 0u;
            }
        }
    }
    if (FLAGS) {
        while (tmask) {
            const u32 j = (u32)__builtin_ctz(tmask);
            tmask &= tmask - 1u;
            stage_pair(j * BLOCK + (u32)tid);
        }
    }
}

template <int BLOCK>
__device__ __forceinline__ void local_load(const LocalArgs& a, const u32 s, const u32 m, u32 (&key)[LOCAL_ITEMS], u32 (&val)[LOCAL_ITEMS]) {
    const u32* kin = a.keys_in + s;
    const u32* vin = a.vals_in + s;
#pragma unroll
    for (int j = 0; j < LOCAL_ITEMS; ++j) {
        const u32 p = (u32)j * BLOCK + threadIdx.x;
        key[j] = 0; val[j] = 0;
        if ((u32)j * BLOCK < m && p < m) { key[j] = kin[p]; val[j] = vin[p]; }
    }
}

template <bool FLAGS, int BLOCK>
__device__ __forceinline__ bool local_short_sub(const LocalArgs& a, const u32 sb, const u32 s, const u32 m, const u32 cap) {
    if (m == 0) {
        if (FLAGS && !(SA_ABL & 8)) {
            const int g2 = a.dir.dbits - 8 - a.rb;
            const u32 dfirst = sb << g2, nd = 1u << g2;
            for (u32 e = threadIdx.x; e < nd; e += BLOCK) a.dir.dir[dfirst + e] = s;
        }
        return true;
    }
    if (m > cap) {
        if (threadIdx.x == 0) __hip_atomic_store(&a.dstat->error, 1u, __ATOMIC_RELAXED, __HIP_MEMORY_SCOPE_AGENT);
        return true;
    }
    if (!FLAGS && m == 1) {
        if (threadIdx.x == 0) {
            const u32 k = a.keys_in[s], v = a.vals_in[s];
            a.keys_out[s] = k; a.vals_out[s] = v;
            if (a.vals_out64) a.vals_out64[s] = (int64_t)v;
        }
        return true;
    }
    return false;
}

template <int BB, bool FLAGS, int BLOCK = LOCAL_BLOCK>
__global__ __launch_bounds__(BLOCK, 4) void local_finish_kernel(LocalArgs a) {
    constexpr u32 CAP = (u32)BLOCK * LOCAL_ITEMS;
    constexpr int NB = 1 << BB, WORDS = NB / 2, WPT = WORDS / BLOCK;
    static_assert(WPT >= 1 && WPT * BLOCK == WORDS, "the scan covers the counters exactly");
    static_assert(CAP < 65536, "16-bit counters and starts");
    __shared__ __attribute__((aligned(16))) u64 s_rec[CAP + 2];
    __shared__ __attribute__((aligned(16))) u32 s_cw[WORDS + 4];
    __shared__ u32 s_wsum[BLOCK / WAVE];
    const u32 sb = blockIdx.x;
    const u32 s = a.sub[sb];
    const u32 m = a.sub[sb + 1] - s;
    if (FLAGS && threadIdx.x == 0 && sb == gridDim.x - 1) a.dir.dir[1u << a.dir.dbits] = a.n;
    if (local_short_sub<FLAGS, BLOCK>(a, sb, s, m, CAP)) return;
#pragma unroll
    for (int i = 0; i < WPT; ++i) s_cw[WPT * threadIdx.x + i] = 0;
    __syncthreads();
    u32 key[LOCAL_ITEMS], val[LOCAL_ITEMS];
    local_load<BLOCK>(a, s, m, key, val);
    local_finish_sub<BB, FLAGS, BLOCK, false>(a, sb, s, m, key, val, s_rec, s_cw, s_wsum, [] {});
}

__device__ __forceinline__ u32 wave_lower_bound(const u32* __restrict__ sub, const u32 nsub, const u64 t) {
    const u32 lane = threadIdx.x & 63u;
    u32 lo = 0, hi = nsub;
    while (lo < hi) {
        const u32 step = (hi - lo + 63u) / 64u;
        const u32 i = lo + lane * step;
        const u32 c = (u32)__popcll(__ballot(i < hi && (u64)sub[i] < t));
        if (c == 0) break;
        const u32 nlo = lo + (c - 1u) * step + 1u;
        hi = (lo + c * step < hi) ? lo + c * step : hi;
        lo = nlo;
    }
    return lo;
}

template <int BB, bool FLAGS, int BLOCK = LOCAL_BLOCK>
__global__ __launch_bounds__(BLOCK, 4) void local_persist_kernel(LocalArgs a, const u32* __restrict__ sub, u32 nsub, u32* ticket, u32 run) {
    constexpr u32 CAP = (u32)BLOCK * LOCAL_ITEMS;
    constexpr int NB = 1 << BB, WORDS = NB / 2, WPT = WORDS / BLOCK;
    static_assert(WPT >= 1 && WPT * BLOCK == WORDS, "the scan covers the counters exactly");
    static_assert(CAP < 65536, "16-bit counters and starts");
    static_assert(BLOCK >= (NCHUNK - 1) * WAVE, "a wave per region bound");
    __shared__ __attribute__((aligned(16))) u64 s_rec[CAP + 2];
    __shared__ __attribute__((aligned(16))) u32 s_cw[WORDS + 4];
    __shared__ u32 s_wsum[BLOCK / WAVE];
    __shared__ u32 s_reg[NCHUNK + 1];
    __shared__ u32 s_run[2];
    const int tid = threadIdx.x;
    {
        const u32 v = (u32)(tid >> 6);
        if (v + 1 < (u32)NCHUNK) {
            const u32 b = wave_lower_bound(sub, nsub, (u64)(v + 1) * sub[nsub] / NCHUNK);
            if ((tid & 63) == 0) s_reg[v + 1] = b;
        }
        if (tid == 0) { s_reg[0] = 0; s_reg[NCHUNK] = nsub; }
    }
#pragma unroll
    for (int i = 0; i < WPT; ++i) s_cw[WPT * tid + i] = 0;
    __syncthreads();
    const u32 home = xcc_id() & (NCHUNK - 1);
    u32 lo = 0, hi = 0;
    auto grab = [&] {
        if (tid == 0) {
            u32 r0 = 0, r1 = 0;
            for (int k = 0; k < NCHUNK; ++k) {
                const u32 c = (home + (u32)k) & (NCHUNK - 1);
                const u32 b0 = s_reg[c], b1 = s_reg[c + 1];
                if (b0 >= b1) continue;
                const u64 st = (u64)b0 + (u64)atomicAdd(&ticket[c], 1u) * run;
                if (st < b1) { r0 = (u32)st; r1 = (st + run < b1) ? (u32)(st + run) : b1; break; }
            }
            s_run[0] = r0; s_run[1] = r1;
        }
        __syncthreads();
        lo = __builtin_amdgcn_readfirstlane(s_run[0]);
        hi = __builtin_amdgcn_readfirstlane(s_run[1]);
        __syncthreads();
    };
    auto next = [&](u32 i, u32& s, u32& m) -> u32 {
        for (;; ++i) {
            if (i >= hi) {
                grab();
                if (lo >= hi) return nsub;
                i = lo;
            }
            s = sub[i]; m = sub[i + 1] - s;
            if (FLAGS && tid == 0 && i == nsub - 1) a.dir.dir[1u << a.dir.dbits] = a.n;
            if (!local_short_sub<FLAGS, BLOCK>(a, i, s, m, CAP)) return i;
        }
    };
    u32 key[LOCAL_ITEMS], val[LOCAL_ITEMS];
    u32 s = 0, m = 0;
    u32 i = next(0, s, m);
    if (i < nsub) local_load<BLOCK>(a, s, m, key, val);
    while (i < nsub) {
        u32 ns = 0, nm = 0;
        const u32 nx = next(i + 1, ns, nm);
        local_finish_sub<BB, FLAGS, BLOCK, true>(a, i, s, m, key, val, s_rec, s_cw, s_wsum, [&] {
            if (nx < nsub) local_load<BLOCK>(a, ns, nm, key, val);
        });
        i = nx; s = ns; m = nm;
    }
}

}
```

### suffixarray_amd/csrc/sa_build.hpp

```cpp
#pragma once
#include <cmath>
#include <cstdlib>
#include <vector>

#include "common.hpp"
#include "radix_narrow.hpp"
#include "radix_narrow48.hpp"
#include "round_sort.hpp"
#include "group_finish.hpp"
#include "period_finish.hpp"

namespace sa {

constexpr int TEXT_PAD = 256;
constexpr int BLD_BLOCK = 256;
constexpr int BLD_ITEMS = 16;
constexpr int BLD_TILE = BLD_BLOCK * BLD_ITEMS;
constexpr u32 NONE32 = 0xFFFFFFFFu;


constexpr int HIST_COPIES = 8;
__global__ __launch_bounds__(256) void byte_hist_kernel(const u8* __restrict__ text, u64 n, u64* __restrict__ hist) {
    constexpr int CS = 257;
    __shared__ u32 s_h[HIST_COPIES * CS];
    for (int i = threadIdx.x; i < HIST_COPIES * CS; i += 256) s_h[i] = 0;
    __syncthreads();
    u32* my = s_h + (threadIdx.x & (HIST_COPIES - 1)) * CS;
    const u64 nvec = n / 16;
    const uint4* v = reinterpret_cast<const uint4*>(text);
    const u64 stride = (u64)gridDim.x * blockDim.x;
    for (u64 i = (u64)blockIdx.x * blockDim.x + threadIdx.x; i < nvec; i += stride) {
        const uint4 x = v[i];
        const u32 w[4] = {x.x, x.y, x.z, x.w};
#pragma unroll
        for (int k = 0; k < 4; ++k) {
            atomicAdd(&my[w[k] & 255u], 1u);
            atomicAdd(&my[(w[k] >> 8) & 255u], 1u);
            atomicAdd(&my[(w[k] >> 16) & 255u], 1u);
            atomicAdd(&my[w[k] >> 24], 1u);
        }
    }
    if (blockIdx.x == 0) {
        for (u64 i = nvec * 16 + threadIdx.x; i < n; i += blockDim.x) atomicAdd(&my[text[i]], 1u);
    }
    sync_lds();
    u32 c = 0;
#pragma unroll
    for (int k = 0; k < HIST_COPIES; ++k) c += s_h[k * CS + threadIdx.x];
    if (c) atomicAdd((unsigned long long*)&hist[threadIdx.x], (unsigned long long)c);
}

constexpr u32 PILOT_SAMPLES = 1u << 17;
constexpr u32 PILOT_SLOTS = 1u << 20;
__global__ __launch_bounds__(256) void pilot_kernel(const u8* __restrict__ text, u64 n, int w, unsigned long long* __restrict__ table,
                                                    u32* __restrict__ dups) {
    const u32 s = blockIdx.x * blockDim.x + threadIdx.x;
    if (s >= PILOT_SAMPLES) return;
    const u64 p = (n - 8) / PILOT_SAMPLES * s;
    u64 v;
    __builtin_memcpy(&v, text + p, 8);
    if (w < 8) v &= (1ull << (8 * w)) - 1ull;
    const unsigned long long key = v * 0x9E3779B97F4A7C15ull | 1ull;
    u32 slot = (u32)(key >> 40) & (PILOT_SLOTS - 1);
    for (int probe = 0; probe < 16; ++probe) {
        const unsigned long long old = atomicCAS(&table[slot], 0ull, key);
        if (old == 0ull) return;
        if (old == key) { atomicAdd(dups, 1u); return; }
        slot = (slot + 1) & (PILOT_SLOTS - 1);
    }
}

__global__ __launch_bounds__(BLD_BLOCK) void keygen_kernel(const u8* __restrict__ text, u64 n, CodeMap map, int b,
                                                           int k0, u64* __restrict__ keys, SortGeom g, int shift0,
                                                           u32 mask0, u32* __restrict__ ghist) {
    __shared__ u16 s_map[256];
    __shared__ u16 s_codes[BLD_TILE + 64 + 16];
    __shared__ u32 s_h[RADIX];
    s_map[threadIdx.x] = map.code[threadIdx.x];
    s_h[threadIdx.x] = 0;
    const u64 ntiles = (n + BLD_TILE - 1) / BLD_TILE;
    const u64 per = (ntiles + gridDim.x - 1) / gridDim.x;
    const u64 t_lo = (u64)blockIdx.x * per;
    const u64 t_hi = (t_lo + per < ntiles) ? t_lo + per : ntiles;
    u32 cur_chunk = chunk_of_tile((u32)((t_lo * BLD_TILE) >> g.tile_shift), g.tpc);
    for (u64 tile = t_lo; tile < t_hi; ++tile) {
        const u64 base = tile * BLD_TILE;
        if (ghist) {
            const u32 c = chunk_of_tile((u32)(base >> g.tile_shift), g.tpc);
            if (c != cur_chunk) { hist_flush(s_h, ghist, cur_chunk); cur_chunk = c; }
        }
        sync_lds();
        {
            uint4 x = make_uint4(0, 0, 0, 0);
            if (base + (u64)threadIdx.x * 16 < n) x = *reinterpret_cast<const uint4*>(text + base + (u64)threadIdx.x * 16);
            const u32 w[4] = {x.x, x.y, x.z, x.w};
#pragma unroll
            for (int k = 0; k < 16; ++k) {
                const u64 p = base + (u64)threadIdx.x * 16 + k;
                const u32 byte = (w[k >> 2] >> ((k & 3) * 8)) & 255u;
                s_codes[threadIdx.x * 16 + k] = (p < n) ? s_map[byte] : (u16)0;
            }
        }
        if (threadIdx.x < 64 + 16) {
            const u64 p = base + BLD_TILE + threadIdx.x;
            s_codes[BLD_TILE + threadIdx.x] = (p < n) ? s_map[text[p]] : (u16)0;
        }
        sync_lds();
#pragma unroll 4
        for (int it = 0; it < BLD_ITEMS; ++it) {
            const u32 l = it * BLD_BLOCK + threadIdx.x;
            const u64 p = base + l;
            if (p < n) {
                u64 key = 0;
                int sh = 64;
                for (int j = 0; j < k0; ++j) {
                    sh -= b;
                    key |= (u64)s_codes[l + j] << sh;
                }
                keys[p] = key;
                if (ghist) atomicAdd(&s_h[(u32)(key >> shift0) & mask0], 1u);
            }
        }
    }
    if (ghist && t_lo < t_hi) hist_flush(s_h, ghist, cur_chunk);
// ... 744 lines not shown
    s_map[threadIdx.x] = map.code[threadIdx.x];
    __syncthreads();
    const u64 stride = (u64)gridDim.x * blockDim.x;
    for (u64 j = (u64)blockIdx.x * blockDim.x + threadIdx.x; j < n; j += stride) {
        const u64 start = sa[j];
        u64 key = 0;
        int sh = 64;
        for (int i = 0; i < k0; ++i) {
            const u64 p = start + i;
            sh -= b;
            const u64 c = (p < n) ? (u64)s_map[text[p]] : 0ull;
            key |= c << sh;
        }
        keys[j] = key;
    }
}

__global__ __launch_bounds__(256) void dir_build_kernel(const u64* __restrict__ keys, u64 n, int dbits, u32* __restrict__ dir,
                                                        const u32* __restrict__ coarse, int cbits) {
    const u64 nb = (1ull << dbits) + 1;
    const u64 stride = (u64)gridDim.x * blockDim.x;
    for (u64 bkt = (u64)blockIdx.x * blockDim.x + threadIdx.x; bkt < nb; bkt += stride) {
        u64 lo = 0, hi = n;
        if (bkt == nb - 1) lo = n;
        else {
            const u64 bound = bkt << (64 - dbits);
            if (coarse) {
                const u64 cb = bkt >> (dbits - cbits);
                lo = coarse[cb];
                hi = coarse[cb + 1];
            }
            while (lo < hi) {
                const u64 mid = (lo + hi) >> 1;
                if (keys[mid] < bound) lo = mid + 1; else hi = mid;
            }
        }
        dir[bkt] = (u32)lo;
    }
}


struct DevBuf {
    void* p = nullptr;
    size_t cap = 0;
    int ensure(size_t bytes) {
        if (bytes <= cap) return 0;
        if (p) (void)hipFree(p);
        p = nullptr; cap = 0;
        SA_HIP_CHECK(hipMalloc(&p, bytes));
        cap = bytes;
        return 0;
    }
    void release() { if (p) (void)hipFree(p); p = nullptr; cap = 0; }
    template <class T> T* as() const { return reinterpret_cast<T*>(p); }
};

inline u32 stream_grid(u64 work_items, u32 per_block) {
    u64 g = (work_items + per_block - 1) / per_block;
    if (g > 256u * 8u) g = 256u * 8u;
    if (g == 0) g = 1;
    return (u32)g;
}

#ifndef SA_FLAGS_GRID
#define SA_FLAGS_GRID 32768
#endif

struct Builder {
    hipStream_t stream = nullptr;
    u64 n_max = 0;
    DevBuf text, keys0, keys1, vals0, vals1, flags, counts, small, isa;
    DevBuf apos0, apos1, apos2, aidx, gid, rkeys0, rkeys1, ridx0, ridx1, lf, tile_last, carry;
    RadixWorkspace radix;
    NarrowWorkspace narrow;
    bool partial_char = true;
    bool narrow48 = true;
    u32* sa = nullptr;
    DevBuf sa_own;
    u64 n = 0;
    u32 max_suffix_length = 0;
    u64 freq[256];
    sa_hip_build_stats stats;
    hipEvent_t ev_begin = nullptr, ev_end = nullptr;
    int chunk_rounds_before_doubling = 2;
    bool adaptive_doubling = true;
    int initial_chars_override = 0;
    double pilot_dup_share = 0.0;
    DevBuf pilot;
    bool fuse_hist = true;
    bool fuse_directory = true;
    bool text_top_pass = true;
    bool wide_text_pass = true;
    bool narrow_sort = true;
    DevBuf partial, dbg, done;
    bool tiny_finisher = true;
    bool local_rounds = true;
    DevBuf gstart, loc_tiles, big_keys, big_vals;
    bool group_finish = true;
    bool fin_left_failed = false;
    bool fin_left_fast = true;
    DevBuf fin_left_gid;
    bool fin_useful = true;
    bool use_pilot = true;
    DevBuf fin_flag;
    bool period_finish = true;
    int per_skip = 0, per_fails = 0;
    DevBuf per_gd, per_bad, per_table, per_dec, per_tf, per_carry;
    u32* lst_cur = nullptr;
    u32* lst_nxt = nullptr;
    bool lst_first = true, lst_keep_first = false;
    void swap_lists() {
        if (lst_keep_first && lst_first) { lst_cur = lst_nxt; lst_nxt = apos2.as<u32>(); }
        else { u32* t = lst_cur; lst_cur = lst_nxt; lst_nxt = t; }
        lst_first = false;
    }
    u32 fin_count_max = FIN_COUNT_MAX;
    int fin_radix_chars = FIN_RADIX_CHARS;
    u64 local_records = 0, big_records = 0;
    LocTile one_tile{};
    bool debug_rounds = false;
    const u64* qkeys = nullptr;
    DevBuf qkeys2;
    DevBuf qskeys;
    bool k2_ready = false;
    int q_k2n = 0;
    const u32* qkeys32 = nullptr;
    const u32* q_bstart = nullptr;
    int q_lo_shift = 0;
    bool narrow_k = true;
    DevBuf qdir;
    CodeMap qmap;
    int q_b = 0, q_k0 = 0, q_dbits = 0;
    bool dir_ready = false;
    bool dir_by_local_pass = false;
    int sector_search = 2;

    bool narrow48_possible(int b) const {
        return narrow_sort && narrow48 && fuse_hist && text_top_pass && radix.block == 512 && b <= 8 && n >= (1u << 22) &&
               n / (512u * SEG48_LAST_ITEMS) + RADIX + 1 <= radix.max_tiles;
    }
    int choose_initial_chars(int b, u32 L) const {
        const int kmax = (narrow48_possible(b) && 56 / b >= 6) ? 56 / b : 64 / b;
        int k = kmax;
        if (initial_chars_override > 0) {
            k = initial_chars_override < kmax ? initial_chars_override : kmax;
        } else {
            double c2 = 0.0;
            for (int c = 0; c < 256; ++c) { const double pr = (double)freq[c] / (double)n; c2 += pr * pr; }
            if (c2 < 0.999999) {
                const double need = std::log(0.02 / (double)n) / std::log(c2);
                int kk = (int)std::ceil(need);
                if (kk < 1) kk = 1;
                const double d_eff = 1.0 / std::pow(c2, 8.0);
                const double s_n = (double)PILOT_SAMPLES;
                const double iid_share = 1.0 + d_eff * std::expm1(-s_n / d_eff) / s_n;
                if (kk < kmax && pilot_dup_share <= iid_share + 0.03) {
                    const int passes = (kk * b + RADIX_BITS - 1) / RADIX_BITS;
                    kk = (passes * RADIX_BITS) / b;
                    k = kk < kmax ? kk : kmax;
                }
            }
        }
        if (L && (u32)k > L) k = (int)L;
        return k < 1 ? 1 : k;
    }

    u8* mbox = nullptr;
    enum : size_t { MB_FREQ = 0, MB_PILOT = 2048, MB_TOTALS = 2064, MB_STATUS = 2112, MB_BIG = 2240, MB_FT = 2304, MB_BEST = 2560, MB_BYTES = 4096 };
    int init(u64 nmax, hipStream_t s) {
        stream = s;
        n_max = nmax;
        if (!mbox) SA_HIP_CHECK(hipHostMalloc(reinterpret_cast<void**>(&mbox), MB_BYTES, hipHostMallocDefault));
        const u64 cap = nmax ? nmax : 1;
        int rc;
        if ((rc = text.ensure(cap + TEXT_PAD + 16))) return rc;
        if ((rc = small.ensure(4096))) return rc;
        int sort_block = 512;
        if (const char* e = diag_env("SA_HIP_SORT_BLOCK")) sort_block = (atoi(e) == 256) ? 256 : 512;
        if (const char* e = diag_env("SA_HIP_INITIAL_CHARS")) initial_chars_override = atoi(e);
        if (const char* e = diag_env("SA_HIP_CHUNK_ROUNDS")) chunk_rounds_before_doubling = atoi(e);
        if (const char* e = diag_env("SA_HIP_ADAPTIVE_DOUBLING")) adaptive_doubling = atoi(e) != 0;
        if (const char* e = diag_env("SA_HIP_FUSE_HIST")) fuse_hist = atoi(e) != 0;
        if (const char* e = diag_env("SA_HIP_FUSE_DIR")) fuse_directory = atoi(e) != 0;
        if (const char* e = diag_env("SA_HIP_NARROW")) narrow_sort = atoi(e) != 0;
        if (const char* e = diag_env("SA_HIP_NARROW48")) narrow48 = atoi(e) != 0;
        if (const char* e = diag_env("SA_HIP_PARTIAL_CHAR")) partial_char = atoi(e) != 0;
        if (const char* e = diag_env("SA_HIP_TEXT_PASS")) text_top_pass = atoi(e) != 0;
        if (const char* e = diag_env("SA_HIP_WIDE_TEXT_PASS")) wide_text_pass = atoi(e) != 0;
        if (const char* e = diag_env("SA_HIP_NARROW_K")) narrow_k = atoi(e) != 0;
        if (const char* e = diag_env("SA_HIP_TINY")) tiny_finisher = atoi(e) != 0;
        if (const char* e = diag_env("SA_HIP_LITE_FLAGS")) lite_flags = atoi(e) != 0;
        if (const char* e = diag_env("SA_HIP_LOCAL_ROUNDS")) local_rounds = atoi(e) != 0;
        if (const char* e = diag_env("SA_HIP_GROUP_FINISH")) group_finish = atoi(e) != 0;
        if (const char* e = diag_env("SA_HIP_FIN_LEFT_FAST")) fin_left_fast = atoi(e) != 0;
        if (const char* e = diag_env("SA_HIP_PILOT")) use_pilot = atoi(e) != 0;
        if (const char* e = diag_env("SA_HIP_PERIOD_FINISH")) period_finish = atoi(e) != 0;
        if (const char* e = diag_env("SA_HIP_SECTOR_SEARCH")) sector_search = atoi(e);
        if (const char* e = diag_env("SA_HIP_FIN_COUNT_MAX")) fin_count_max = (u32)atoi(e);
        if (const char* e = diag_env("SA_HIP_FIN_RADIX_CHARS")) fin_radix_chars = atoi(e);
        if (const char* e = diag_env("SA_HIP_DEBUG_ROUNDS")) debug_rounds = atoi(e) != 0;
        if (debug_rounds) { radix.debug_hook = &Builder::sort_debug_hook; radix.debug_ctx = this; }
        if ((rc = radix.init(cap, sort_block))) return rc;
        if ((rc = narrow.init())) return rc;
        SA_HIP_CHECK(hipEventCreate(&ev_begin));
        SA_HIP_CHECK(hipEventCreate(&ev_end));
        memset(&stats, 0, sizeof stats);
        memset(freq, 0, sizeof freq);
        return 0;
    }
    int ensure_key_buffers(u64 count, bool narrow) {
        const size_t bytes = (size_t)(count ? count : 1) * (narrow ? 4 : 8) + 64;
        int rc;
        if ((rc = keys0.ensure(bytes))) return rc;
        return keys1.ensure(bytes);
    }
    int ensure_build_buffers() {
        const u64 cap = n_max ? n_max : 1;
        int rc;
        if ((rc = vals0.ensure(cap * 4))) return rc;
        if ((rc = vals1.ensure(cap * 4))) return rc;
        if ((rc = flags.ensure(cap + 64))) return rc;
        if ((rc = counts.ensure((size_t)div_up(cap, BLD_TILE) * sizeof(uint2) + 64))) return rc;
        return 0;
    }
    void destroy() {
        DevBuf* all[] = {&text, &keys0, &keys1, &vals0, &vals1, &flags, &counts, &small, &isa, &apos0, &apos1, &apos2, &aidx,
                         &gid, &rkeys0, &rkeys1, &ridx0, &ridx1, &lf, &tile_last, &carry, &sa_own, &partial, &qdir, &dbg, &done, &pilot,
                         &gstart, &loc_tiles, &big_keys, &big_vals, &fin_flag, &fin_left_gid, &lite_stage, &qkeys2, &qskeys, &per_gd, &per_bad, &per_table, &per_dec, &per_tf, &per_carry};
        for (DevBuf* b : all) b->release();
        radix.destroy();
        narrow.destroy();
        if (ev_begin) (void)hipEventDestroy(ev_begin);
        if (ev_end) (void)hipEventDestroy(ev_end);
        ev_begin = ev_end = nullptr;
        if (mbox) (void)hipHostFree(mbox);
        mbox = nullptr;
    }

    int prepare_text(u64 n_, CodeMap& map, u32& sigma, int& b) {
        n = n_;
        SA_HIP_CHECK(hipMemsetAsync(text.as<u8>() + n, 0, TEXT_PAD + 16, stream));
        u64* dh = small.as<u64>();
        SA_HIP_CHECK(hipMemsetAsync(dh, 0, 256 * sizeof(u64), stream));
        if (n) hipLaunchKernelGGL(byte_hist_kernel, dim3(stream_grid(n, 256 * 64)), dim3(256), 0, stream, text.as<u8>(), n, dh);
        static_assert(sizeof freq == 2048, "mailbox layout");
        SA_HIP_CHECK(hipMemcpyAsync(mbox + MB_FREQ, dh, sizeof freq, hipMemcpyDeviceToHost, stream));
        u32 pilot_dups = 0;
        pilot_dup_share = 0.0;
        const bool run_pilot = use_pilot && n >= (u64)16 * PILOT_SAMPLES;
        if (run_pilot) {
            int rc = pilot.ensure((size_t)PILOT_SLOTS * 8 + 64);
            if (rc) return rc;
            SA_HIP_CHECK(hipMemsetAsync(pilot.p, 0, (size_t)PILOT_SLOTS * 8 + 64, stream));
            u32* pd = reinterpret_cast<u32*>(pilot.as<u8>() + (size_t)PILOT_SLOTS * 8);
            hipLaunchKernelGGL(pilot_kernel, dim3(PILOT_SAMPLES / 256), dim3(256), 0, stream, text.as<u8>(), n, 8,
                               pilot.as<unsigned long long>(), pd);
            SA_HIP_CHECK(hipMemcpyAsync(mbox + MB_PILOT, pd, 4, hipMemcpyDeviceToHost, stream));
        }
        SA_HIP_CHECK(hipStreamSynchronize(stream));
        memcpy(freq, mbox + MB_FREQ, sizeof freq);
        if (run_pilot) memcpy(&pilot_dups, mbox + MB_PILOT, 4);
        if (run_pilot) pilot_dup_share = (double)pilot_dups / (double)PILOT_SAMPLES;
        sigma = 0;
        memset(&map, 0, sizeof map);
        for (int c = 0; c < 256; ++c)
            if (freq[c]) map.code[c] = (u16)(++sigma);
        b = bits_for((u64)sigma + 1);
        if (b == 0) b = 1;
        return 0;
    }

    DeviceStatus status_seen{};
    u32 lite_overflow_seen = 0;
    bool status_fresh = false;
    int read_totals(u32* totals_host) {
        static_assert(sizeof(DeviceStatus) <= MB_BIG - MB_STATUS, "mailbox layout");
        SA_HIP_CHECK(hipMemcpyAsync(mbox + MB_TOTALS, small.as<u8>() + 2048, 3 * sizeof(u32), hipMemcpyDeviceToHost, stream));
        SA_HIP_CHECK(hipMemcpyAsync(mbox + MB_STATUS, radix.dstat, sizeof status_seen, hipMemcpyDeviceToHost, stream));
        SA_HIP_CHECK(hipStreamSynchronize(stream));
        memcpy(totals_host, mbox + MB_TOTALS, 2 * sizeof(u32));
        memcpy(&lite_overflow_seen, mbox + MB_TOTALS + 2 * sizeof(u32), sizeof(u32));
        memcpy(&status_seen, mbox + MB_STATUS, sizeof status_seen);
        status_fresh = true;
        return 0;
    }
    u32* totals_dev() { return reinterpret_cast<u32*>(small.as<u8>() + 2048); }

    int check_device_status() {
        DeviceStatus st;
        if (status_fresh) {
            st = status_seen;
            status_fresh = false;
        } else {
            SA_HIP_CHECK(hipMemcpyAsync(mbox + MB_STATUS, radix.dstat, sizeof st, hipMemcpyDeviceToHost, stream));
            SA_HIP_CHECK(hipStreamSynchronize(stream));
            memcpy(&st, mbox + MB_STATUS, sizeof st);
        }
        if (st.error != 0) {
            (void)hipMemsetAsync(radix.dstat, 0, sizeof(DeviceStatus), stream);
            return fail(SA_HIP_EINTERNAL, "device look-back spin limit expired");
        }
        return 0;
    }

    int scan_counts(u32 tiles, u32* totals_host) {
        const u32 parts = div_up(tiles, 1024);
        int rc = partial.ensure((size_t)parts * sizeof(uint2) + 64);
        if (rc) return rc;
        hipLaunchKernelGGL(counts_reduce_kernel, dim3(parts), dim3(1024), 0, stream, counts.as<uint2>(), tiles, partial.as<uint2>());
        hipLaunchKernelGGL(counts_scan_partials_kernel, dim3(1), dim3(1024), 0, stream, partial.as<uint2>(), parts, totals_dev());
        hipLaunchKernelGGL(counts_apply_kernel, dim3(parts), dim3(1024), 0, stream, counts.as<uint2>(), tiles, partial.as<uint2>());
        return read_totals(totals_host);
    }

    void launch_compact(const u8* lf_in, u32 cnt, u32 active, const u32* src_pos, const u32* src_idx, u32* dst_pos,
                        u32* dst_idx, u32* dst_gid) {
        const u32 tiles = div_up(cnt, BLD_TILE);
#ifndef SA_DENSE_DIV
#define SA_DENSE_DIV 100
#endif
        if ((u64)active * SA_DENSE_DIV >= cnt)
            hipLaunchKernelGGL(compact_dense_kernel, dim3(tiles), dim3(BLD_BLOCK), 0, stream, lf_in, cnt, counts.as<uint2>(), src_pos,
                               src_idx, dst_pos, dst_idx, dst_gid);
        else
            hipLaunchKernelGGL(compact_kernel, dim3(tiles), dim3(BLD_BLOCK), 0, stream, lf_in, cnt, counts.as<uint2>(), src_pos,
                               src_idx, dst_pos, dst_idx, dst_gid);
    }

    int compact_lists(u32& M, u32& G, const u32* tot) {
        if (tot[0] >= M) return 0;
        if (tot[0]) {
            SA_HIP_CHECK(hipMemcpyAsync(ridx0.p, aidx.p, (size_t)M * 4, hipMemcpyDeviceToDevice, stream));
            launch_compact(lf.as<u8>(), M, tot[0], lst_cur, ridx0.as<u32>(), lst_nxt, aidx.as<u32>(), gid.as<u32>());
            swap_lists();
        }
        M = tot[0];
        G = tot[1];
        return 0;
    }

    int flags_and_counts(const u64* keys, u32 cnt, u8* lf_out, const u32* apos, const u32* sidx, u32* totals_host,
                         bool with_directory = false, const NarrowKeys* nk = nullptr) {
        const u32 tiles = div_up(cnt, BLD_TILE);
        DirArgs d{};
        if (with_directory) {
            int rc = directory_layout(cnt);
            if (rc) return rc;
            d.dir = qdir.as<u32>();
            d.dbits = q_dbits;
            const u64 nb = (1ull << q_dbits) + 1;
            d.gaps = reinterpret_cast<uint4*>(qdir.as<u8>() + dir_gap_offset(nb));
            d.gap_cap = dir_gap_cap(nb);
            d.gap_count = reinterpret_cast<u32*>(small.as<u8>() + 3584);
            d.dstat = radix.dstat;
            SA_HIP_CHECK(hipMemsetAsync(d.gap_count, 0, 4, stream));
        }
        const u32 fgrid = (SA_FLAGS_GRID && tiles > (u32)SA_FLAGS_GRID) ? (u32)SA_FLAGS_GRID : tiles;
        if (nk)
            hipLaunchKernelGGL(flags_kernel<true>, dim3(fgrid), dim3(BLD_BLOCK), 0, stream, (const u64*)nullptr, *nk, cnt, lf_out,
                               counts.as<uint2>(), apos, sidx, sa, flags.as<u8>(), d);
        else
            hipLaunchKernelGGL(flags_kernel<false>, dim3(fgrid), dim3(BLD_BLOCK), 0, stream, keys, NarrowKeys{}, cnt, lf_out,
                               counts.as<uint2>(), apos, sidx, sa, flags.as<u8>(), d);
        if (with_directory) {
            hipLaunchKernelGGL(dir_fill_kernel, dim3(1024), dim3(256), 0, stream, d);
            dir_ready = true;
        }
        return scan_counts(tiles, totals_host);
    }

    bool lite_flags = true;
    bool flags_valid = true;
    LiteArgs lite{};
    NarrowKeys lite_nk{};
    DevBuf lite_stage;
    DirArgs split_dir{};
    u32 lite_tiles = 0;
    static int split_flags_prepare(void* ctx, u32 nsub, LocalArgs* l) {
        Builder* b = static_cast<Builder*>(ctx);
        int rc = b->directory_layout(b->n);
        if (rc) return rc;
        if ((rc = b->counts.ensure((size_t)nsub * sizeof(uint2) + 64))) return rc;
        if ((rc = b->lite_stage.ensure((size_t)nsub * LITE_CAP * 9 + 64))) return rc;
        DirArgs d{};
        d.dir = b->qdir.as<u32>();
        d.dbits = b->q_dbits;
        const u64 nb = (1ull << b->q_dbits) + 1;
        d.gaps = reinterpret_cast<uint4*>(b->qdir.as<u8>() + dir_gap_offset(nb));
        d.gap_cap = dir_gap_cap(nb);
        d.gap_count = reinterpret_cast<u32*>(b->small.as<u8>() + 3584);
        d.dstat = b->radix.dstat;
        SA_HIP_CHECK(hipMemsetAsync(d.gap_count, 0, 4, b->stream));
        b->lite.sa = nullptr;
        b->lite.st_pos = b->lite_stage.as<u32>();
        b->lite.st_idx = b->lite.st_pos + (size_t)nsub * LITE_CAP;
        b->lite.st_head = reinterpret_cast<u8*>(b->lite.st_idx + (size_t)nsub * LITE_CAP);
        b->lite.overflow = b->totals_dev() + 2;
        SA_HIP_CHECK(hipMemsetAsync(b->lite.overflow, 0, 4, b->stream));
        SA_HIP_CHECK(hipMemsetAsync(b->counts.p, 0, (size_t)nsub * sizeof(uint2), b->stream));
        b->split_dir = d;
        b->lite_tiles = nsub;
        l->dir = d;
        l->counts = b->counts.as<uint2>();
        l->lite = b->lite;
        return 0;
    }
    int flags_after_split(const NarrowKeys& nk, u32* totals_host, bool* overflow) {
        dir_ready = true;
        dir_by_local_pass = true;
        lite_nk = nk;
        int rc = scan_counts(lite_tiles, totals_host);
        if (rc) return rc;
        *overflow = lite_overflow_seen != 0;
        return 0;
    }
    int flags_lite_pass(const NarrowKeys& nk, u32 cnt, void* stage, u32* totals_host, bool* overflow) {
        const u32 tiles = div_up(cnt, BLD_TILE);
        lite_tiles = tiles;
        int rc = directory_layout(cnt);
        if (rc) return rc;
        DirArgs d{};
        d.dir = qdir.as<u32>();
        d.dbits = q_dbits;
        const u64 nb = (1ull << q_dbits) + 1;
        d.gaps = reinterpret_cast<uint4*>(qdir.as<u8>() + dir_gap_offset(nb));
        d.gap_cap = dir_gap_cap(nb);
        d.gap_count = reinterpret_cast<u32*>(small.as<u8>() + 3584);
        d.dstat = radix.dstat;
        SA_HIP_CHECK(hipMemsetAsync(d.gap_count, 0, 4, stream));
        lite.sa = sa;
        lite.st_pos = static_cast<u32*>(stage);
        lite.st_idx = lite.st_pos + (size_t)tiles * LITE_CAP;
        lite.st_head = reinterpret_cast<u8*>(lite.st_idx + (size_t)tiles * LITE_CAP);
        lite.overflow = totals_dev() + 2;
        lite_nk = nk;
        SA_HIP_CHECK(hipMemsetAsync(lite.overflow, 0, 4, stream));
        SA_HIP_CHECK(hipMemsetAsync(counts.p, 0, (size_t)tiles * sizeof(uint2), stream));
        const u32 fgrid = (SA_FLAGS_GRID && tiles > (u32)SA_FLAGS_GRID) ? (u32)SA_FLAGS_GRID : tiles;
        hipLaunchKernelGGL(flags_lite_kernel, dim3(fgrid), dim3(BLD_BLOCK), 0, stream, nk, cnt, counts.as<uint2>(), d, lite);
        hipLaunchKernelGGL(dir_fill_kernel, dim3(1024), dim3(256), 0, stream, d);
        dir_ready = true;
        if ((rc = scan_counts(tiles, totals_host))) return rc;
        *overflow = lite_overflow_seen != 0;
        return 0;
    }
    int materialise_flags() {
        if (flags_valid) return 0;
        const u32 n32 = (u32)n;
        const u32 tiles = div_up(n32, BLD_TILE);
        const u32 fgrid = (SA_FLAGS_GRID && tiles > (u32)SA_FLAGS_GRID) ? (u32)SA_FLAGS_GRID : tiles;
        hipLaunchKernelGGL(flags_kernel<true>, dim3(fgrid), dim3(BLD_BLOCK), 0, stream, (const u64*)nullptr, lite_nk, n32, flags.as<u8>(),
                           counts.as<uint2>(), (const u32*)nullptr, (const u32*)nullptr, sa, flags.as<u8>(), DirArgs{});
        flags_valid = true;
        SA_HIP_CHECK(hipGetLastError());
        return 0;
    }

    int scatter_ranks(const u8* lf_in, u32 cnt, const u32* posmap, const u32* idx) {
        const u32 tiles = div_up(cnt, BLD_TILE);
        int rc;
        if ((rc = tile_last.ensure((size_t)tiles * 4 + 64))) return rc;
        if ((rc = carry.ensure((size_t)tiles * 4 + 64))) return rc;
        hipLaunchKernelGGL(tile_last_head_kernel, dim3(tiles), dim3(BLD_BLOCK), 0, stream, lf_in, cnt, posmap, tile_last.as<u32>());
        hipLaunchKernelGGL(scan_last_head_kernel, dim3(1), dim3(1024), 0, stream, tile_last.as<u32>(), tiles, carry.as<u32>());
        hipLaunchKernelGGL(scatter_ranks_kernel, dim3(tiles), dim3(BLD_BLOCK), 0, stream, lf_in, cnt, posmap, idx,
                           carry.as<u32>(), isa.as<u32>());
        return 0;
    }

    static void sort_debug_hook(void* ctx, int pass, int npasses, int shift, u32 mask, const u64* kin, const u32* vin,
                                const u64* keys, const u32* vals, u32 cnt) {
        Builder* b = static_cast<Builder*>(ctx);
        if (b->dbg.ensure((size_t)b->n * 4 + 16)) return;
        u64* dd = reinterpret_cast<u64*>(b->small.as<u8>() + 3072);
        u64 dups[49];
        (void)hipMemsetAsync(b->dbg.p, 0, (size_t)b->n * 4, b->stream);
        (void)hipMemsetAsync(dd, 0, sizeof dups, b->stream);
        hipLaunchKernelGGL(dbg_dup_kernel, dim3(stream_grid(cnt, 1024)), dim3(256), 0, b->stream, vals, (u64)cnt, b->dbg.as<u32>(), dd);
        (void)hipMemcpyAsync(dups, dd, sizeof dups, hipMemcpyDeviceToHost, b->stream);
        (void)hipStreamSynchronize(b->stream);
        if (dups[0]) {
            fprintf(stderr, "[sa_hip]   sort pass %d/%d over %u records: %llu duplicate values; slot pairs:", pass, npasses, cnt, (unsigned long long)dups[0]);
            for (u64 k = 0; k < dups[0] && k < 24; ++k) fprintf(stderr, " (%llu,%llu)", (unsigned long long)dups[1 + 2 * k], (unsigned long long)dups[2 + 2 * k]);
            fprintf(stderr, "\n");
        }
        (void)keys;
    }

    static int dir_coarse_bits(int d) { return d > 16 ? 14 : 0; }
    static size_t dir_gap_offset(u64 nb) { return (((size_t)nb + (1u << 14) + 1) * 4 + 15) & ~(size_t)15; }
    static u32 dir_gap_cap(u64 nb) { return (u32)(nb / DIR_INLINE + nb / DIR_PIECE + 4); }
    int directory_layout(u64 count) {
        int lg = 0;
        while ((1ull << lg) < count) ++lg;
        int d = lg - 3;
        if (d < 8) d = 8;
        if (d > 27) d = 27;
        if (const char* e = diag_env("SA_HIP_DIR_BITS")) { const int v = atoi(e); if (v >= 8 && v <= 28) d = v; }
        q_dbits = d;
        const u64 nb = (1ull << d) + 1;
        return qdir.ensure(dir_gap_offset(nb) + (size_t)dir_gap_cap(nb) * sizeof(uint4));
    }

    int build_directory() {
        if ((!qkeys && !qkeys32) || n < 2) { qkeys = nullptr; qkeys32 = nullptr; k2_ready = false; return 0; }
        if (qkeys32 && !dir_ready) return fail(SA_HIP_EINTERNAL, "narrow keys without a fused directory");
        if (dir_ready) {
            const u64 n16 = ((1ull << q_dbits) + 1) / 4;
            if (const char* e = diag_env("SA_HIP_DIR_TOUCH")) { if (atoi(e) == 0) return 0; }
            hipLaunchKernelGGL(dir_touch_kernel, dim3(stream_grid(n16, 256)), dim3(256), 0, stream, qdir.as<uint4>(), n16,
                               reinterpret_cast<u32*>(small.as<u8>() + 3588));
            return 0;
        }
        int rc = directory_layout(n);
        if (rc) return rc;
        const int d = q_dbits;
        const u64 nb = (1ull << d) + 1;
        const int cbits = dir_coarse_bits(d);
        const u64 ncb = cbits ? (1ull << cbits) + 1 : 0;
        u32* fine = qdir.as<u32>();
        u32* coarse = cbits ? fine + nb : nullptr;
        if (cbits)
            hipLaunchKernelGGL(dir_build_kernel, dim3(stream_grid(ncb, 256)), dim3(256), 0, stream, qkeys, n, cbits, coarse,
                               (const u32*)nullptr, 0);
        hipLaunchKernelGGL(dir_build_kernel, dim3(stream_grid(nb, 256)), dim3(256), 0, stream, qkeys, n, d, fine, (const u32*)coarse, cbits);
        SA_HIP_CHECK(hipGetLastError());
        return 0;
    }

    int prepare_query_from_sa(const CodeMap& map, int b, u32 L) {
        qkeys = nullptr;
        qkeys32 = nullptr;
        dir_ready = false;
        k2_ready = false;
        if (n < 2) return 0;
        const int k0 = choose_initial_chars(b, L);
        int rc = keys0.ensure((size_t)n * 8 + 64);
        if (rc) return rc;
        hipLaunchKernelGGL(gather_keys_kernel, dim3(stream_grid(n, 256)), dim3(256), 0, stream, text.as<u8>(), n, map, b, k0,
                           (const u32*)sa, keys0.as<u64>());
        qkeys = keys0.as<u64>();
        qmap = map; q_b = b; q_k0 = k0;
        return build_directory();
    }

    int verify(u64* violations) {
        *violations = 0;
        if (n == 0) return 0;
        int rc = isa.ensure((size_t)n * 4);
        if (rc) return rc;
        u64* bad = reinterpret_cast<u64*>(small.as<u8>() + 3072);
        SA_HIP_CHECK(hipMemsetAsync(bad, 0, 8, stream));
        SA_HIP_CHECK(hipMemsetAsync(isa.p, 0xFF, (size_t)n * 4, stream));
        const u32 g = stream_grid(n, 1024);
        hipLaunchKernelGGL(verify_scatter_kernel, dim3(g), dim3(256), 0, stream, (const u32*)sa, n, isa.as<u32>(), bad);
        if (max_suffix_length == 0)
            hipLaunchKernelGGL(verify_order_kernel, dim3(g), dim3(256), 0, stream, text.as<u8>(), (const u32*)sa, isa.as<u32>(), n, bad);
        else
            hipLaunchKernelGGL(verify_truncated_kernel, dim3(g), dim3(256), 0, stream, text.as<u8>(), (const u32*)sa, isa.as<u32>(), n,
                               max_suffix_length, bad);
        SA_HIP_CHECK(hipMemcpyAsync(violations, bad, 8, hipMemcpyDeviceToHost, stream));
        SA_HIP_CHECK(hipStreamSynchronize(stream));
        return 0;
    }

    int round_sort(u64* k0, const u32* vsrc, u32* v0, u64* k1, u32* v1, u32 M, u32 G, int begin_bit, int end_bit, int gid_shift,
                   u64** kres, u32** vres) {
        int rc;
        auto global_sort = [&]() -> int {
            SA_HIP_CHECK(hipMemcpyAsync(v0, vsrc, (size_t)M * 4, hipMemcpyDeviceToDevice, stream));
            return radix_sort_pairs(radix, stream, k0, v0, k1, v1, M, begin_bit, end_bit, false, false, kres, vres);
        };
        int top = (gid_shift < 64 - LOC_GID_BITS) ? gid_shift + LOC_GID_BITS : 64;
        if (top > end_bit) top = end_bit;
        if (!local_rounds || G == 0 || top <= begin_bit || (M > LOC_CAP && (u64)M > (u64)G * (LOC_CAP / 2)))
            return global_sort();
        u32 ntiles = div_up(M, LOC_TILE);
        if ((rc = gstart.ensure(((size_t)G + 2) * 4))) return rc;
        if ((rc = loc_tiles.ensure((size_t)ntiles * sizeof(LocTile) + 64))) return rc;
        u32* total_dev = reinterpret_cast<u32*>(small.as<u8>() + 3616);
        u32 big = 0;
        if (M <= LOC_CAP) {
            one_tile.begin = 0; one_tile.local_end = M; one_tile.end = M; one_tile.big_off = 0;
            SA_HIP_CHECK(hipMemcpyAsync(loc_tiles.p, &one_tile, sizeof one_tile, hipMemcpyHostToDevice, stream));
            ntiles = 1;
        } else {
        hipLaunchKernelGGL(group_starts_kernel, dim3(stream_grid(M, 1024)), dim3(256), 0, stream, gid.as<u32>(), M, G, gstart.as<u32>());
        hipLaunchKernelGGL((loc_plan_kernel<LOC_TILE, LOC_CAP>), dim3(div_up(ntiles, 256)), dim3(256), 0, stream, gid.as<u32>(), gstart.as<u32>(), M, ntiles,
                           loc_tiles.as<LocTile>());
        hipLaunchKernelGGL(loc_scan_kernel, dim3(1), dim3(1024), 0, stream, loc_tiles.as<LocTile>(), ntiles, total_dev);
        SA_HIP_CHECK(hipMemcpyAsync(mbox + MB_BIG, total_dev, 4, hipMemcpyDeviceToHost, stream));
        SA_HIP_CHECK(hipStreamSynchronize(stream));
        memcpy(&big, mbox + MB_BIG, 4);
        if ((u64)big * 2 > M)
// ... 100 lines not shown
        if (ft_host[1] * 4 < ft_host[0]) fin_useful = false;
        if (debug_rounds)
            fprintf(stderr, "[sa_hip] finisher h=%llu M=%u G=%u tiles=%u (%llu non-empty): looked at %llu, resolved %llu -> M'=%u G'=%u; rounds %llu (%llu radix), "
                    "slots radix %llu counting %llu, active record-rounds %llu\n", (unsigned long long)h, M, G, ntiles, ft_host[6], ft_host[0], ft_host[1],
                    tot[0], tot[1], ft_host[2], ft_host[3], ft_host[4], ft_host[5], ft_host[7]);
        if (debug_rounds && ft_host[6])
            fprintf(stderr, "[sa_hip]   finisher (radix rounds %llu, radix slots %llu) cycles per tile (thread 0, clock64): fetch+keys %llu, counting sort %llu, radix sort %llu, regroup %llu, write-out %llu\n",
                    ft_host[3], ft_host[4], ft_host[8] / ft_host[6], ft_host[9] / ft_host[6], ft_host[10] / ft_host[6], ft_host[11] / ft_host[6], ft_host[12] / ft_host[6]);
        if (debug_rounds && ft_host[6]) {
            fprintf(stderr, "[sa_hip]   records by group size at entry [2^c, 2^(c+1)):");
            for (int c = 1; c < 13; ++c) fprintf(stderr, " %d:%llu", c, ft_host[16 + c]);
            fprintf(stderr, "\n");
        }
        if ((rc = compact_lists(M, G, tot))) return rc;
        return 0;
    }

    int run_period_finisher(bool have_isa, u32& M, u32& G, u32* tot) {
        int rc;
        if ((rc = gstart.ensure(((size_t)G + 2) * 4))) return rc;
        if ((rc = per_gd.ensure((size_t)G * 4 + 64))) return rc;
        if ((rc = per_bad.ensure((size_t)G + 64))) return rc;
        if ((rc = per_dec.ensure((size_t)G + 64))) return rc;
        if ((rc = per_table.ensure((size_t)PER_TABLE * sizeof(uint2)))) return rc;
        if ((rc = done.ensure((size_t)M + 64))) return rc;
        const u32 ntiles = div_up(n, PER_TILE);
        if ((rc = per_tf.ensure((size_t)ntiles * 4 + 64))) return rc;
        if ((rc = per_carry.ensure((size_t)ntiles * 4 + 64))) return rc;
        SA_HIP_CHECK(hipMemsetAsync(done.p, 0, (size_t)M, stream));
        hipLaunchKernelGGL(group_starts_kernel, dim3(stream_grid(M, 1024)), dim3(256), 0, stream, gid.as<u32>(), M, G, gstart.as<u32>());
        hipLaunchKernelGGL(per_init_kernel, dim3(stream_grid(G, 256)), dim3(256), 0, stream, aidx.as<u32>(), gstart.as<u32>(), G,
                           per_gd.as<u32>(), per_bad.as<u8>());
        hipLaunchKernelGGL(per_classify_kernel, dim3(stream_grid(M, 1024)), dim3(256), 0, stream, aidx.as<u32>(), gid.as<u32>(), gstart.as<u32>(), M,
                           per_gd.as<u32>(), per_bad.as<u8>());
        u32* best_dev = reinterpret_cast<u32*>(small.as<u8>() + 3720);
        u64 covered = 0;
        for (int iter = 0; iter < 4; ++iter) {
            SA_HIP_CHECK(hipMemsetAsync(per_table.p, 0, (size_t)PER_TABLE * sizeof(uint2), stream));
            hipLaunchKernelGGL(per_hist_kernel, dim3(stream_grid(G, 256)), dim3(256), 0, stream, gstart.as<u32>(), G, per_gd.as<u32>(),
                               per_bad.as<u8>(), per_table.as<uint2>());
            hipLaunchKernelGGL(per_pick_kernel, dim3(1), dim3(1024), 0, stream, per_table.as<uint2>(), best_dev);
            u32 best[2] = {0, 0};
            SA_HIP_CHECK(hipMemcpyAsync(mbox + MB_BEST, best_dev, 8, hipMemcpyDeviceToHost, stream));
            SA_HIP_CHECK(hipStreamSynchronize(stream));
            memcpy(best, mbox + MB_BEST, 8);
            if (debug_rounds) fprintf(stderr, "[sa_hip] period finisher M=%u G=%u: difference %u covers %u records\n", M, G, best[0], best[1]);
            if (best[0] == 0 || (u64)best[1] * 8 < M) break;
            covered += best[1];
            const u64 d = best[0];
            hipLaunchKernelGGL(per_tile_first_kernel, dim3(ntiles), dim3(256), 0, stream, text.as<u8>(), n, d, per_tf.as<u32>());
            hipLaunchKernelGGL(per_tile_scan_kernel, dim3(1), dim3(1024), 0, stream, per_tf.as<u32>(), ntiles, per_carry.as<u32>());
            PerArgs a;
            a.text = text.as<u8>(); a.n = n; a.d = d;
            a.aidx = aidx.as<u32>(); a.apos = lst_cur; a.gid = gid.as<u32>(); a.gstart = gstart.as<u32>(); a.gd = per_gd.as<u32>();
            a.bad = per_bad.as<u8>(); a.G = G; a.M = M; a.tile_first = per_tf.as<u32>(); a.carry = per_carry.as<u32>(); a.dec = per_dec.as<u8>();
            a.sa = sa; a.gflags = flags.as<u8>(); a.done = done.as<u8>(); a.isa = have_isa ? isa.as<u32>() : nullptr;
            hipLaunchKernelGGL(per_decide_kernel, dim3(stream_grid((u64)G * 64, 256)), dim3(256), 0, stream, a);
            hipLaunchKernelGGL(per_apply_kernel, dim3(stream_grid(M, 1024)), dim3(256), 0, stream, a);
        }
        if ((u64)covered * 8 < M) { per_skip = 2 << per_fails++; return 0; }
        const u32 tiles = div_up(M, BLD_TILE);
        hipLaunchKernelGGL(tiny_flags_kernel, dim3(tiles), dim3(BLD_BLOCK), 0, stream, gid.as<u32>(), done.as<u8>(), M, lf.as<u8>(),
                           counts.as<uint2>());
        if ((rc = scan_counts(tiles, tot))) return rc;
        stats.period_resolved += (u64)M - tot[0];
        if (debug_rounds) fprintf(stderr, "[sa_hip] period finisher: resolved %u of %u -> M'=%u G'=%u\n", M - tot[0], M, tot[0], tot[1]);
        if ((u64)(M - tot[0]) * 8 < M) per_skip = 2 << per_fails++;
        if ((rc = compact_lists(M, G, tot))) return rc;
        return 0;
    }

    int build(u64 n_, u32 L, int64_t* sa64_out = nullptr) {
        int rc;
        memset(&stats, 0, sizeof stats);
        local_records = big_records = 0;
        fin_useful = true;
        fin_left_failed = false;
        per_skip = per_fails = 0;
        radix.reset_stats();
        max_suffix_length = L;
        stats.n = n_;
        if (n_ > n_max) return fail(SA_HIP_EINVAL, "text longer than the index capacity");
        if ((rc = ensure_build_buffers())) return rc;
        SA_HIP_CHECK(hipEventRecord(ev_begin, stream));
        CodeMap map;
        u32 sigma = 0;
        int b = 1;
        if ((rc = prepare_text(n_, map, sigma, b))) return rc;
        stats.sigma = sigma;
        stats.bits_per_symbol = (u32)b;
        sa = vals0.as<u32>();
        qkeys = nullptr;
        qkeys32 = nullptr;
        dir_ready = false;
        dir_by_local_pass = false;
        k2_ready = false;
        stats.widen_fused = 0;
        if (n == 0) return finish_stats();
        if (n == 1) {
            SA_HIP_CHECK(hipMemsetAsync(sa, 0, 4, stream));
            SA_HIP_CHECK(hipMemsetAsync(flags.p, 1, 1, stream));
            if (sa64_out) SA_HIP_CHECK(hipMemsetAsync(sa64_out, 0, 8, stream));
            return finish_stats();
        }
        const int k0 = choose_initial_chars(b, L);
        stats.initial_chars = (u32)k0;
        const u32 n32 = (u32)n;

        SortPlan pl;
        const int begin_bit = 64 - b * k0;
        if ((rc = make_plan(radix, n32, begin_bit, 64, pl))) return rc;
        const bool narrow_path = narrow_sort && fuse_hist && narrow_sort_applies(radix, n, begin_bit);
        const bool narrow48_path = !narrow_path && narrow48_possible(b) && narrow48_applies(radix, n, begin_bit, b, k0);
        stats.narrow48 = narrow48_path ? 1u : 0u;
        if (fuse_hist) { if ((rc = radix_prepare(radix, stream))) return rc; }
        const bool text_pass = narrow_path && text_top_pass && text_pass_applies(b, k0);
        stats.text_top_pass = text_pass ? 1u : 0u;
        if ((rc = ensure_key_buffers(n, narrow_path && text_pass && narrow_k && fuse_directory))) return rc;
        if (diag_env("SA_HIP_DEBUG_ADDR"))
            fprintf(stderr, "[sa_hip] addr text=%p keys0=%p keys1=%p vals0=%p vals1=%p sa64=%p\n", text.p, keys0.p, keys1.p, vals0.p, vals1.p, (void*)sa64_out);
        const bool wide_text = !narrow_path && !narrow48_path && wide_text_pass && fuse_hist && radix.block == 512 && text_pass_applies(b, k0) &&
                               pl.npasses > 1 && n >= (1u << 16);
        stats.text_top_pass = (text_pass || wide_text || narrow48_path) ? 1u : 0u;
        if (text_pass || narrow48_path) {
            if ((rc = text_histogram(radix, narrow, stream, text.as<u8>(), map, n32, b, TEXT_TILE, 0))) return rc;
        } else if (wide_text) {
            if ((rc = text_histogram(radix, narrow, stream, text.as<u8>(), map, n32, b, radix.tile(), k0))) return rc;
        } else {
            hipLaunchKernelGGL(keygen_kernel, dim3(stream_grid(n, BLD_TILE)), dim3(BLD_BLOCK), 0, stream, text.as<u8>(), n, map, b,
                               k0, keys0.as<u64>(), pl.g, narrow_path ? 56 : pl.shift(0), narrow_path ? 255u : pl.mask(0),
                               fuse_hist ? radix.hist(0) : (u32*)nullptr);
        }
        u64* kres; u32* vres;
        bool flags_by_local_pass = false;
        const bool keep_narrow = narrow_path && narrow_k && fuse_directory;
        stats.narrow_k = keep_narrow ? 1u : 0u;
        if (narrow_path) {
            TextSource src;
            src.text = text.as<u8>(); src.b = b; src.k0 = k0;
            LocalFlagsRequest freq;
            if (keep_narrow && lite_flags) { freq.prepare = &Builder::split_flags_prepare; freq.ctx = this; }
            NarrowSortResult res;
            if ((rc = radix_sort_narrow(radix, narrow, stream, keys0.as<u64>(), vals0.as<u32>(), keys1.as<u64>(), vals1.as<u32>(),
                                        n32, begin_bit, &res, text_pass ? &src : nullptr, keep_narrow, sa64_out, &freq))) return rc;
            kres = res.keys; vres = res.vals;
            if (sa64_out) stats.widen_fused = 1;
            stats.split_plan = (u32)res.rb;
            stats.split_max = res.max_group;
            flags_by_local_pass = res.flags_done;
        } else if (narrow48_path) {
            TextSource src;
            src.text = text.as<u8>(); src.b = b; src.k0 = k0;
            int begin48 = begin_bit;
            if (partial_char && b * k0 < 56 && b * (k0 + 1) > 56 && (L == 0 || (u32)(k0 + 1) <= L) && text_pass_applies(b, k0 + 1)) {
                src.k0 = k0 + 1;
                begin48 = 8;
            }
            if ((rc = radix_sort_narrow48(radix, narrow, stream, keys0.as<u64>(), vals0.as<u32>(), keys1.as<u64>(), vals1.as<u32>(),
                                          n32, begin48, &kres, &vres, src, sa64_out))) return rc;
            if (sa64_out) stats.widen_fused = 1;
        } else {
            WideTextCtx wctx{text.as<u8>(), narrow.map_dev, n, b, k0};
            Pass0Launcher p0;
            p0.launch = &launch_text_low_pass; p0.ctx = &wctx; p0.bytes_per_record = 13;
            if ((rc = radix_sort_pairs(radix, stream, keys0.as<u64>(), vals0.as<u32>(), keys1.as<u64>(), vals1.as<u32>(), n32,
                                       begin_bit, 64, true, fuse_hist, &kres, &vres, wide_text ? &p0 : nullptr))) return rc;
// ... 97 lines not shown
            const bool shrinking = M_prev != 0 && (u64)M * 2 <= (u64)M_prev;
            bool use_chunk = (L != 0) || (chunk_done < chunk_rounds_before_doubling) || (adaptive_doubling && !have_isa && shrinking);
            int kc = 0;
            if (use_chunk) {
                kc = (64 - gb) / b;
                if (L && (u64)kc > L - h) kc = (int)(L - h);
                if (kc <= 0) use_chunk = false;
            }
            int begin_bit;
            u64 h_next;
            if (use_chunk) {
                hipLaunchKernelGGL(chunk_keys_kernel, dim3(stream_grid(M, 256)), dim3(256), 0, stream, text.as<u8>(), n, map, b,
                                   aidx.as<u32>(), gid.as<u32>(), M, (u32)h, kc, gb, rkeys0.as<u64>());
                begin_bit = 64 - gb - b * kc;
                h_next = h + kc;
                ++chunk_done;
                ++stats.chunk_rounds;
            } else {
                if (L != 0) return fail(SA_HIP_EINTERNAL, "truncated build cannot make progress");
                if (gb + rb > 64) return fail(SA_HIP_EINTERNAL, "composite key exceeds 64 bits");
                if (!have_isa) {
                    if ((rc = isa.ensure((size_t)n * 4))) return rc;
                    if ((rc = scatter_ranks(flags.as<u8>(), n32, nullptr, sa))) return rc;
                    have_isa = true;
                }
                hipLaunchKernelGGL(doubling_keys_kernel, dim3(stream_grid(M, 256)), dim3(256), 0, stream, isa.as<u32>(), n,
                                   aidx.as<u32>(), gid.as<u32>(), M, h, rb, rkeys0.as<u64>());
                begin_bit = 0;
                h_next = 2 * h;
                ++stats.doubling_rounds;
            }
            const int end_bit = use_chunk ? 64 : (gb + rb);
            if ((rc = round_sort(rkeys0.as<u64>(), aidx.as<u32>(), ridx0.as<u32>(), rkeys1.as<u64>(), ridx1.as<u32>(), M, G, begin_bit, end_bit,
                                 use_chunk ? (gb ? 64 - gb : 64) : rb, &kres, &vres))) return rc;
            if ((rc = flags_and_counts(kres, M, lf.as<u8>(), apos_cur, vres, tot))) return rc;
            if ((rc = check_device_status())) return rc;
            if (have_isa) {
                if ((rc = scatter_ranks(lf.as<u8>(), M, apos_cur, vres))) return rc;
            }
            if (debug_rounds) {
                u64 dups_sa = 0, dups_act = 0;
                if ((rc = dbg.ensure((size_t)n * 4 + 16))) return rc;
                u64* dd = reinterpret_cast<u64*>(small.as<u8>() + 3072);
                SA_HIP_CHECK(hipMemsetAsync(dbg.p, 0, (size_t)n * 4, stream));
                SA_HIP_CHECK(hipMemsetAsync(dd, 0, 49 * 8, stream));
                hipLaunchKernelGGL(dbg_dup_kernel, dim3(stream_grid(n, 1024)), dim3(256), 0, stream, (const u32*)sa, n, dbg.as<u32>(), dd);
                SA_HIP_CHECK(hipMemcpyAsync(&dups_sa, dd, 8, hipMemcpyDeviceToHost, stream));
                SA_HIP_CHECK(hipStreamSynchronize(stream));
                SA_HIP_CHECK(hipMemsetAsync(dbg.p, 0, (size_t)n * 4, stream));
                SA_HIP_CHECK(hipMemsetAsync(dd, 0, 49 * 8, stream));
                hipLaunchKernelGGL(dbg_dup_kernel, dim3(stream_grid(M, 1024)), dim3(256), 0, stream, (const u32*)vres, (u64)M, dbg.as<u32>(), dd);
                SA_HIP_CHECK(hipMemcpyAsync(&dups_act, dd, 8, hipMemcpyDeviceToHost, stream));
                SA_HIP_CHECK(hipStreamSynchronize(stream));
                fprintf(stderr, "[sa_hip] round %u %s h=%llu M=%u G=%u -> M'=%u G'=%u passes=%d dupSA=%llu dupActive=%llu\n", stats.rounds,
                        use_chunk ? "chunk" : "dbl", (unsigned long long)h, M, G, tot[0], tot[1], (end_bit - begin_bit + 7) / 8,
                        (unsigned long long)dups_sa, (unsigned long long)dups_act);
            }
            stats.active_total += M;
            ++stats.rounds;
            M_prev = M;
            h = h_next;
            const u32 M_next = tot[0];
            if (M_next && (L == 0 || h < L)) {
                launch_compact(lf.as<u8>(), M, M_next, apos_cur, vres, apos_nxt, aidx.as<u32>(), gid.as<u32>());
                swap_lists();
            }
            M = M_next;
            G = tot[1];
            if (stats.rounds > (debug_rounds ? 40u : 200u)) return fail(SA_HIP_EINTERNAL, "refinement did not converge");
        }
        stats.final_depth = (u32)(h > 0xFFFFFFFFull ? 0xFFFFFFFFull : h);
        if (sa64_out) {
            if (!stats.widen_fused)
                hipLaunchKernelGGL(widen_kernel, dim3(stream_grid(n / 4 + 1, 256)), dim3(256), 0, stream, (const u32*)sa, n, sa64_out);
            else if (M0 && !patched_by_tiny)
                hipLaunchKernelGGL(widen_patch_kernel, dim3(stream_grid(M0, 256)), dim3(256), 0, stream, (const u32*)apos0.as<u32>(), M0,
                                   (const u32*)sa, sa64_out);
        }
        if ((rc = build_directory())) return rc;
        return finish_stats();
    }

    int finish_stats() {
        SA_HIP_CHECK(hipEventRecord(ev_end, stream));
        SA_HIP_CHECK(hipEventSynchronize(ev_end));
        float ms = 0.f;
        SA_HIP_CHECK(hipEventElapsedTime(&ms, ev_begin, ev_end));
        int rc = radix.timer.flush();
        if (rc) return rc;
        stats.total_ms = ms;
        stats.radix_ms = radix.timer.total_ms;
        stats.radix_passes = (u32)radix.passes;
        stats.radix_records = radix.pass_records;
        stats.radix_bytes = radix.pass_bytes;
        for (int k = 0; k < PASS_KINDS; ++k) {
            stats.pass_ms[k] = radix.timer.kind_ms[k];
            stats.pass_bytes[k] = radix.timer.kind_bytes[k];
            stats.pass_launches[k] = (u32)radix.timer.kind_launches[k];
        }
        return 0;
    }
};

}
```

Measured before the change: 78.41 billion.

## Overlap pilot and directory touch on side stream, add NT-load variants

Runs the pilot sampling kernel and the directory touch kernel on a separate non-blocking stream joined by events, so they overlap with the byte histogram and later refinement work. Also merges several small zeroed buffers into one arena so that one memset covers them, and drops a few per-build memsets. The byte histogram is unrolled over several loads per thread. The top histogram is split into full and tail span paths. Nontemporal load variants are added but stay off unless a diagnostic environment variable enables them. The cross-stream ordering adds a risk of races if a join is missed.

```diff
diff --git a/suffixarray_amd/csrc/big_build.hpp b/suffixarray_amd/csrc/big_build.hpp
--- a/suffixarray_amd/csrc/big_build.hpp
+++ b/suffixarray_amd/csrc/big_build.hpp
@@ -400,7 +400,7 @@
         return build_with(n, sa_out, [&](u64* keys, u64* idx, int* key_bits, u64* h0) -> int {
             u64* dh = small.as<u64>();
             SA_HIP_CHECK(hipMemsetAsync(dh, 0, 256 * sizeof(u64), stream));
-            hipLaunchKernelGGL(byte_hist_kernel, dim3(stream_grid(n, 256 * 64)), dim3(256), 0, stream, text_dev, n, dh);
+            hipLaunchKernelGGL(byte_hist_kernel<false>, dim3(stream_grid(n, BYTE_HIST_PER_BLOCK)), dim3(256), 0, stream, text_dev, n, dh);
             u64 freq[256];
             SA_HIP_CHECK(hipMemcpyAsync(freq, dh, sizeof freq, hipMemcpyDeviceToHost, stream));
             SA_HIP_CHECK(hipStreamSynchronize(stream));
diff --git a/suffixarray_amd/csrc/common.hpp b/suffixarray_amd/csrc/common.hpp
--- a/suffixarray_amd/csrc/common.hpp
+++ b/suffixarray_amd/csrc/common.hpp
@@ -6,6 +6,7 @@
 #include <cstring>
 #include <string>
 #include <new>
+#include <type_traits>
 
 #include "../../include/sa_hip.h"
 
@@ -60,6 +61,32 @@
     asm volatile("s_waitcnt lgkmcnt(0)" ::: "memory");
     __syncthreads();
 }
+
+typedef u32 u32x4_native __attribute__((ext_vector_type(4)));
+template <bool NT>
+__device__ __forceinline__ uint4 load_stream(const uint4* p) {
+    if constexpr (NT) {
+        const u32x4_native x = __builtin_nontemporal_load(reinterpret_cast<const u32x4_native*>(p));
+        return make_uint4(x.x, x.y, x.z, x.w);
+    } else {
+        return *p;
+    }
+}
+template <bool NT, typename T>
+__device__ __forceinline__ T ld_stream(const T* p) {
+    if constexpr (NT) return __builtin_nontemporal_load(p);
+    else return *p;
+}
+template <bool NT, typename T>
+__device__ __forceinline__ void st_stream(T* p, T v) {
+    if constexpr (NT) __builtin_nontemporal_store(v, p);
+    else *p = v;
+}
+template <typename Body>
+__device__ __forceinline__ void with_nt(bool nt, Body&& body) {
+    if (nt) body(std::true_type{});
+    else body(std::false_type{});
+}
 #endif
 
 struct HostU64Array {
@@ -91,6 +118,11 @@
     static const bool on = [] { const char* d = getenv("SA_HIP_DIAG"); return d && atoi(d) != 0; }();
     return on ? getenv(name) : nullptr;
 }
+constexpr u32 NT_TEXT = 1;
+constexpr u32 NT_SPLIT = 2;
+constexpr u32 NT_LOCAL_LOAD = 4;
+constexpr u32 NT_LOCAL_STORE = 8;
+constexpr u32 NT_DEFAULT = 0;
 
 struct CodeMap {
     u16 code[256];
diff --git a/suffixarray_amd/csrc/radix_narrow.hpp b/suffixarray_amd/csrc/radix_narrow.hpp
--- a/suffixarray_amd/csrc/radix_narrow.hpp
+++ b/suffixarray_amd/csrc/radix_narrow.hpp
@@ -301,9 +301,39 @@
 namespace sa {
 
 constexpr int TOP_HIST_COPIES = 8;
-template <int C8>
+template <int C8, bool FULL, bool NT>
+__device__ __forceinline__ void top_hist_span(const u8* __restrict__ text, u64 n, u64 p0, u64 off, int b, int dshift, u32* my,
+                                              const u8* s_map) {
+    if (!FULL && p0 >= n) return;
+    uint4 x0, x1;
+    if constexpr (NT) {
+        typedef u32 u32x4_u __attribute__((ext_vector_type(4), aligned(1)));
+        const u32x4_u* q = reinterpret_cast<const u32x4_u*>(text + p0 + off);
+        const u32x4_native y0 = __builtin_nontemporal_load(q), y1 = __builtin_nontemporal_load(q + 1);
+        x0 = make_uint4(y0.x, y0.y, y0.z, y0.w);
+        x1 = make_uint4(y1.x, y1.y, y1.z, y1.w);
+    } else {
+        __builtin_memcpy(&x0, text + p0 + off, 16);
+        __builtin_memcpy(&x1, text + p0 + off + 16, 16);
+    }
+    const u32 w[8] = {x0.x, x0.y, x0.z, x0.w, x1.x, x1.y, x1.z, x1.w};
+    const u64 first = p0 + off;
+    const u32 live = FULL ? 32u : ((first >= n) ? 0u : ((n - first < 32) ? (u32)(n - first) : 32u));
+    const u32 npos = FULL ? 16u : ((n - p0 < 16) ? (u32)(n - p0) : 16u);
+    u32 win = 0;
+#pragma unroll
+    for (int k = 0; k < 16 + C8 - 1; ++k) {
+        const u32 byte = (w[k >> 2] >> ((k & 3) * 8)) & 255u;
+        const u32 code = (FULL || (u32)k < live) ? (u32)s_map[byte] : 0u;
+        win = (win << b) | code;
+        const int i = k - (C8 - 1);
+        if (i >= 0 && (FULL || (u32)i < npos)) atomicAdd(&my[(win >> dshift) & 255u], 1u);
+    }
+}
+
+template <int C8, bool NT>
 __global__ __launch_bounds__(256) void top_hist_kernel(const u8* __restrict__ text, const u16* __restrict__ map, u64 n, int b,
-                                                       SortGeom g, u32* __restrict__ hist, int low_k0 = 0) {
+                                                       SortGeom g, u32* __restrict__ hist, int low_k0) {
     constexpr int CS = RADIX + 1;
     constexpr u32 SPAN = 256 * 16;
     __shared__ u32 s_h[TOP_HIST_COPIES * CS];
@@ -312,9 +342,8 @@
     for (int i = threadIdx.x; i < TOP_HIST_COPIES * CS; i += 256) s_h[i] = 0;
     __syncthreads();
     u32* my = s_h + (threadIdx.x & (TOP_HIST_COPIES - 1)) * CS;
-    constexpr int c8 = C8;
-    const u32 wmask = (1u << (c8 * b)) - 1u;
-    const int dshift = c8 * b - 8;
+    const int dshift = low_k0 ? 0 : C8 * b - 8;
+    const u64 off = low_k0 ? (u64)(low_k0 - C8) : 0;
     const u64 nspans = (n + SPAN - 1) / SPAN;
     const u64 per = (nspans + gridDim.x - 1) / gridDim.x;
     const u64 s_lo = (u64)blockIdx.x * per;
@@ -334,25 +363,10 @@
         const u32 c = chunk_of_tile((u32)(base / g.tile), g.tpc);
         if (c != cur) { flush(cur); cur = c; }
         const u64 p0 = base + (u64)threadIdx.x * 16;
-        if (p0 < n) {
-            const u64 off = low_k0 ? (u64)(low_k0 - c8) : 0;
-            uint4 x0, x1;
-            __builtin_memcpy(&x0, text + p0 + off, 16);
-            __builtin_memcpy(&x1, text + p0 + off + 16, 16);
-            const u32 w[8] = {x0.x, x0.y, x0.z, x0.w, x1.x, x1.y, x1.z, x1.w};
-            const u64 first = p0 + off;
-            const u32 live = (first >= n) ? 0u : ((n - first < 32) ? (u32)(n - first) : 32u);
-            const u32 npos = (n - p0 < 16) ? (u32)(n - p0) : 16u;
-            u32 win = 0;
-#pragma unroll
-            for (int k = 0; k < 16 + c8 - 1; ++k) {
-                const u32 byte = (w[k >> 2] >> ((k & 3) * 8)) & 255u;
-                const u32 code = ((u32)k < live) ? (u32)s_map[byte] : 0u;
-                win = ((win << b) | code) & wmask;
-                const int i = k - (c8 - 1);
-                if (i >= 0 && (u32)i < npos) atomicAdd(&my[low_k0 ? (win & 255u) : (win >> dshift)], 1u);
-            }
-        }
+        if (base + off + SPAN + 16 <= n)
+            top_hist_span<C8, true, NT>(text, n, p0, off, b, dshift, my, s_map);
+        else
+            top_hist_span<C8, false, NT>(text, n, p0, off, b, dshift, my, s_map);
     }
     flush(cur);
 }
@@ -374,6 +388,7 @@
     u32 incl_mask;
     u32* cursor;
     int owned;
+    u32 nt;
 };
 constexpr u32 TOP_CURSOR_STRIDE = 64;
 constexpr int TEXT_HALO = 64;
@@ -568,8 +583,24 @@
 #pragma unroll
     for (int i = 0; i < W / 4; ++i) x[i] = 0;
     if (start >= 0) {
-        if (FULL || start < n) __builtin_memcpy(&x[0], a.text + start, 16);
-        if (FULL || start + 16 < n) __builtin_memcpy(&x[4], a.text + start + 16, W - 16);
+        with_nt(a.nt != 0, [&](auto NT) {
+            if constexpr (decltype(NT)::value) {
+                typedef u32 u32x4_u __attribute__((ext_vector_type(4), aligned(1)));
+                typedef u32 u32x2_u __attribute__((ext_vector_type(2), aligned(1)));
+                static_assert(W == 24, "a 16-byte load and an 8-byte one");
+                if (FULL || start < n) {
+                    const u32x4_native y = __builtin_nontemporal_load(reinterpret_cast<const u32x4_u*>(a.text + start));
+                    x[0] = y.x; x[1] = y.y; x[2] = y.z; x[3] = y.w;
+                }
+                if (FULL || start + 16 < n) {
+                    const u32x2_u y = __builtin_nontemporal_load(reinterpret_cast<const u32x2_u*>(a.text + start + 16));
+                    x[4] = y.x; x[5] = y.y;
+                }
+            } else {
+                if (FULL || start < n) __builtin_memcpy(&x[0], a.text + start, 16);
+                if (FULL || start + 16 < n) __builtin_memcpy(&x[4], a.text + start + 16, W - 16);
+            }
+        });
     } else {
 #pragma unroll
         for (int i = 0; i < W; ++i) {
@@ -925,7 +956,11 @@
     u32* host_word = nullptr;
     static size_t split_table_bytes() { return (size_t)RADIX * SPLIT_NB * sizeof(u32); }
     static size_t split_sub_words() { return ((size_t)RADIX << SPLIT_BITS) + 1; }
-    u32* split_levels_dev() const { return split_sub + split_sub_words(); }
+    u32* split_levels = nullptr;
+    u32* split_levels_dev() const { return split_levels; }
+    u8* zero_arena = nullptr;
+    static size_t arena_tickets_bytes() { return (((size_t)NARROW_MAX_PASSES * NCHUNK + 16) * sizeof(u32) + 255) & ~(size_t)255; }
+    static size_t zero_arena_bytes() { return arena_tickets_bytes() + top_cursor_bytes() + 2 * split_table_bytes(); }
     u32 split_cap = LOCAL_CAP;
     int local_bin_bits = 12;
     bool split_flags = true;
@@ -945,18 +980,22 @@
         *grid = g < nsub ? g : nsub;
         return 0;
     }
+    u32 nt_mask = NT_DEFAULT;
+    u32 hist_grid_force = 0;
     int split_items = 28;
     static size_t hist_bytes() { return (size_t)NARROW_MAX_PASSES * RADIX * RADIX * sizeof(u32); }
     int init() {
         SA_HIP_CHECK(hipMalloc(&plan, sizeof(SegPlan)));
         SA_HIP_CHECK(hipMalloc(&hist, hist_bytes()));
         SA_HIP_CHECK(hipMalloc(&base, (size_t)RADIX * RADIX * sizeof(u32)));
-        SA_HIP_CHECK(hipMalloc(&tickets, (size_t)NARROW_MAX_PASSES * NCHUNK * sizeof(u32)));
+        SA_HIP_CHECK(hipMalloc(reinterpret_cast<void**>(&zero_arena), zero_arena_bytes()));
+        tickets = reinterpret_cast<u32*>(zero_arena);
+        split_levels = tickets + NARROW_MAX_PASSES * NCHUNK;
+        top_cursor = reinterpret_cast<u32*>(zero_arena + arena_tickets_bytes());
+        split_hist = reinterpret_cast<u32*>(zero_arena + arena_tickets_bytes() + top_cursor_bytes());
+        split_cursor = reinterpret_cast<u32*>(zero_arena + arena_tickets_bytes() + top_cursor_bytes() + split_table_bytes());
         SA_HIP_CHECK(hipMalloc(&map_dev, sizeof(CodeMap)));
-        SA_HIP_CHECK(hipMalloc(&split_hist, split_table_bytes()));
         SA_HIP_CHECK(hipMalloc(&split_base, split_table_bytes()));
-        SA_HIP_CHECK(hipMalloc(&split_cursor, split_table_bytes()));
-        SA_HIP_CHECK(hipMalloc(&top_cursor, top_cursor_bytes()));
         SA_HIP_CHECK(hipMalloc(&split_sub, (split_sub_words() + 16) * sizeof(u32)));
         SA_HIP_CHECK(hipHostMalloc(reinterpret_cast<void**>(&host_word), 64, hipHostMallocDefault));
         if (const char* e = diag_env("SA_HIP_SPLIT")) split_enabled = atoi(e) != 0;
@@ -966,6 +1005,8 @@
         if (const char* e = diag_env("SA_HIP_LOCAL_PERSIST")) local_persist = atoi(e) != 0;
         if (const char* e = diag_env("SA_HIP_LOCAL_GRID")) { const int v = atoi(e); local_grid_force = v > 0 ? (u32)v : 0u; }
         if (const char* e = diag_env("SA_HIP_SPLIT_FLAGS")) split_flags = atoi(e) != 0;
+        if (const char* e = diag_env("SA_HIP_NT")) nt_mask = (u32)atoi(e) & 15u;
+        if (const char* e = diag_env("SA_HIP_HIST_GRID")) { const int v = atoi(e); hist_grid_force = (v > 0 && v <= 2048) ? (u32)v : 0u; }
         if (const char* e = diag_env("SA_HIP_LOCAL_BINS")) local_bin_bits = (atoi(e) == 11) ? 11 : 12;
         if (const char* e = diag_env("SA_HIP_SPLIT_ITEMS")) { const int v = atoi(e); split_items = (v == 24 || v == 28) ? v : 32; }
         if (const char* e = diag_env("SA_HIP_SPLIT_CAP")) { const int v = atoi(e); if (v >= 64 && v <= (int)LOCAL_CAP) split_cap = (u32)v; }
@@ -975,17 +1016,15 @@
         if (plan) (void)hipFree(plan);
         if (hist) (void)hipFree(hist);
         if (base) (void)hipFree(base);
-        if (tickets) (void)hipFree(tickets);
+        if (zero_arena) (void)hipFree(zero_arena);
         if (map_dev) (void)hipFree(map_dev);
-        if (split_hist) (void)hipFree(split_hist);
         if (split_base) (void)hipFree(split_base);
-        if (split_cursor) (void)hipFree(split_cursor);
-        if (top_cursor) (void)hipFree(top_cursor);
         if (split_sub) (void)hipFree(split_sub);
         if (host_word) (void)hipHostFree(host_word);
         map_dev = nullptr;
         plan = nullptr; hist = nullptr; base = nullptr; tickets = nullptr;
-        split_hist = split_base = split_sub = split_cursor = top_cursor = nullptr; host_word = nullptr;
+        split_hist = split_base = split_sub = split_cursor = top_cursor = split_levels = nullptr; host_word = nullptr;
+        zero_arena = nullptr;
     }
 };
 
@@ -1006,14 +1045,16 @@
     SA_HIP_CHECK(hipMemcpyAsync(nw.map_dev, nw.map_host.code, sizeof(CodeMap), hipMemcpyHostToDevice, stream));
     const SortGeom g = make_geom(n, tile);
     const u32 spans = div_up(n, 4096);
-    const dim3 grid(spans < 2048u ? spans : 2048u), block(256);
-    decltype(&top_hist_kernel<1>) kernel;
+    const u32 cap = nw.hist_grid_force ? nw.hist_grid_force : 2048u;
+    const dim3 grid(spans < cap ? spans : cap), block(256);
+    const bool nt = (nw.nt_mask & NT_TEXT) != 0;
+    decltype(&top_hist_kernel<1, false>) kernel;
     switch ((8 + b - 1) / b) {
-        case 1: kernel = top_hist_kernel<1>; break;
-        case 2: kernel = top_hist_kernel<2>; break;
-        case 3: kernel = top_hist_kernel<3>; break;
-        case 4: kernel = top_hist_kernel<4>; break;
-        default: kernel = top_hist_kernel<8>; break;
+        case 1: kernel = nt ? top_hist_kernel<1, true> : top_hist_kernel<1, false>; break;
+        case 2: kernel = nt ? top_hist_kernel<2, true> : top_hist_kernel<2, false>; break;
+        case 3: kernel = nt ? top_hist_kernel<3, true> : top_hist_kernel<3, false>; break;
+        case 4: kernel = nt ? top_hist_kernel<4, true> : top_hist_kernel<4, false>; break;
+        default: kernel = nt ? top_hist_kernel<8, true> : top_hist_kernel<8, false>; break;
     }
     hipLaunchKernelGGL(kernel, grid, block, 0, stream, text, nw.map_dev, (u64)n, b, g, ws.hist(0), low_k0);
     return 0;
@@ -1034,7 +1075,7 @@
 
 enum TopForm { TOP_STABLE, TOP_CLAIM, TOP_EXT };
 inline int launch_text_top(RadixWorkspace& ws, NarrowWorkspace& nw, hipStream_t stream, const TextSource& src, u32 n, int begin_bit,
-                           TopForm form, u32* keys_out32, u16* ext_out16, u32* vals_out) {
+                           TopForm form, u32* keys_out32, u16* ext_out16, u32* vals_out, bool arena_zeroed = false) {
     const bool claim = form == TOP_CLAIM, ext = form == TOP_EXT;
     const SortGeom g = make_geom(n, TEXT_TILE);
     TextPassArgs t;
@@ -1042,8 +1083,9 @@
     t.keys_out32 = keys_out32; t.ext_out16 = ext_out16; t.vals_out = vals_out; t.g = g; t.digit_base = ws.base();
     t.status = ws.status; t.ticket = ws.tickets(); t.epoch = ws.epoch; t.dstat = ws.dstat; t.incl_mask = SA_INCL_MASK;
     t.cursor = ext ? nullptr : nw.top_cursor;
+    t.nt = nw.nt_mask & NT_TEXT;
     t.owned = (claim && nw.top_owned && TEXT_ITEMS == 16 && text_owned_applies(src.b, src.k0)) ? 1 : 0;
-    if (claim) SA_HIP_CHECK(hipMemsetAsync(nw.top_cursor, 0, NarrowWorkspace::top_cursor_bytes(), stream));
+    if (claim && !arena_zeroed) SA_HIP_CHECK(hipMemsetAsync(nw.top_cursor, 0, NarrowWorkspace::top_cursor_bytes(), stream));
     return ws.timed_pass(stream, 1, n, (u64)n * (ext ? 11u : 9u), [&] {
         if (claim) hipLaunchKernelGGL((text_top_pass_kernel<512, false, true>), dim3(g.tiles), dim3(512), 0, stream, t);
         else if (!ext) hipLaunchKernelGGL((text_top_pass_kernel<512>), dim3(g.tiles), dim3(512), 0, stream, t);
@@ -1064,7 +1106,7 @@
     int rc;
     if ((rc = ws.next_epoch(stream))) return rc;
     hipLaunchKernelGGL(radix_scan_hist_kernel, dim3(1), dim3(256), 0, stream, ws.hist(0), ws.base());
-    if (src) return launch_text_top(ws, nw, stream, *src, n, begin_bit, claim ? TOP_CLAIM : TOP_STABLE, keys_out32, nullptr, vals_out);
+    if (src) return launch_text_top(ws, nw, stream, *src, n, begin_bit, claim ? TOP_CLAIM : TOP_STABLE, keys_out32, nullptr, vals_out, true);
     SortPassArgs a;
     a.keys_in = keys_in; a.vals_in = nullptr; a.keys_out = nullptr; a.vals_out = vals_out;
     a.g = make_geom(n, ws.tile()); a.shift = 56; a.mask = 255u; a.next_shift = -1; a.next_mask = 0; a.digit_base = ws.base();
@@ -1082,11 +1124,12 @@
     Hist hist;
     Split split;
 };
-inline SplitKernels split_kernels(int split_items) {
+inline SplitKernels split_kernels(int split_items, u32 nt_mask = 0) {
     const int i = (split_items == 32) ? 0 : (split_items == 28) ? 1 : 2;
     static const SplitKernels::Hist hist[3] = {split_hist_kernel<512, 32>, split_hist_kernel<512, 28>, split_hist_kernel<512, 24>};
     static const SplitKernels::Split split[3] = {seg_split_kernel<512, 32>, seg_split_kernel<512, 28>, seg_split_kernel<512, 24>};
-    return {hist[i], split[i]};
+    static const SplitKernels::Split split_nt[3] = {seg_split_kernel<512, 32, true>, seg_split_kernel<512, 28, true>, seg_split_kernel<512, 24, true>};
+    return {hist[i], (nt_mask & NT_SPLIT) ? split_nt[i] : split[i]};
 }
 
 struct SplitLevel {
@@ -1109,11 +1152,9 @@
 
 inline int narrow_plan_look(NarrowWorkspace& nw, hipStream_t stream, const u32* keys32, int lo_bits, int hb, u32 split_flat_max,
                             SplitLevel* level) {
-    SA_HIP_CHECK(hipMemsetAsync(nw.split_hist, 0, NarrowWorkspace::split_table_bytes(), stream));
-    SA_HIP_CHECK(hipMemsetAsync(nw.split_levels_dev(), 0, 16 * sizeof(u32), stream));
     const u32 tpb = 4;
     hipLaunchKernelGGL(split_kernels(nw.split_items).hist, dim3(div_up(split_flat_max, tpb)), dim3(512), 0, stream, keys32, nw.plan,
-                       lo_bits - hb, (1u << hb) - 1u, nw.split_hist, tpb);
+                       lo_bits - hb, (1u << hb) - 1u, nw.split_hist, tpb, nw.nt_mask & NT_SPLIT);
     hipLaunchKernelGGL(split_levels_kernel, dim3(RADIX), dim3(SPLIT_NB), 0, stream, (const u32*)nw.split_hist, hb, nw.split_levels_dev());
     SA_HIP_CHECK(hipMemcpyAsync(nw.host_word, nw.split_levels_dev(), 16 * sizeof(u32), hipMemcpyDeviceToHost, stream));
     SA_HIP_CHECK(hipStreamSynchronize(stream));
@@ -1126,7 +1167,6 @@
     int rc;
     hipLaunchKernelGGL(split_scan_kernel, dim3(RADIX), dim3(SPLIT_NB), 0, stream, (const u32*)nw.split_hist, nw.plan, hb, rb,
                        nw.split_base, nw.split_sub);
-    SA_HIP_CHECK(hipMemsetAsync(nw.split_cursor, 0, NarrowWorkspace::split_table_bytes(), stream));
     if ((rc = ws.next_epoch(stream))) return rc;
     SplitPassArgs a;
     a.keys_in = keys_in; a.vals_in = vals_in;
@@ -1134,7 +1174,7 @@
     a.plan = nw.plan; a.shift = lo_bits - rb; a.mask = (1u << rb) - 1u; a.digit_base = nw.split_base;
     a.ticket = nw.tickets; a.cursor = nw.split_cursor;
     return ws.timed_pass(stream, 2, n, (u64)n * 16u, [&] {
-        hipLaunchKernelGGL(split_kernels(nw.split_items).split, dim3(split_flat_max), dim3(512), 0, stream, a);
+        hipLaunchKernelGGL(split_kernels(nw.split_items, nw.nt_mask).split, dim3(split_flat_max), dim3(512), 0, stream, a);
     });
 }
 
@@ -1145,7 +1185,7 @@
     Finish finish;
     int block, row;
 };
-inline LocalKernels local_kernels(bool big, bool flags, int bb) {
+inline LocalKernels local_kernels(bool big, bool flags, int bb, u32 nt_mask = 0) {
     const int row = big ? (flags ? 0 : 1) : 2 + (flags ? 0 : 2) + (bb == 12 ? 0 : 1);
     static const LocalKernels::Persist persist[6] = {
         local_persist_kernel<12, true, LOCAL_BLOCK_BIG>, local_persist_kernel<12, false, LOCAL_BLOCK_BIG>,
@@ -1153,7 +1193,12 @@
     static const LocalKernels::Finish finish[6] = {
         local_finish_kernel<12, true, LOCAL_BLOCK_BIG>, local_finish_kernel<12, false, LOCAL_BLOCK_BIG>,
         local_finish_kernel<12, true>, local_finish_kernel<11, true>, local_finish_kernel<12, false>, local_finish_kernel<11, false>};
-    return {persist[row], finish[row], big ? LOCAL_BLOCK_BIG : LOCAL_BLOCK, row};
+    static const LocalKernels::Persist persist_nt[2][3] = {
+        {local_persist_kernel<12, true, LOCAL_BLOCK_BIG, 4>, local_persist_kernel<12, true, LOCAL_BLOCK_BIG, 8>, local_persist_kernel<12, true, LOCAL_BLOCK_BIG, 12>},
+        {local_persist_kernel<12, true, LOCAL_BLOCK, 4>, local_persist_kernel<12, true, LOCAL_BLOCK, 8>, local_persist_kernel<12, true, LOCAL_BLOCK, 12>}};
+    const u32 nt = (nt_mask & (NT_LOCAL_LOAD | NT_LOCAL_STORE)) >> 2;
+    const bool has_nt = nt && (row == 0 || row == 2);
+    return {has_nt ? persist_nt[row / 2][nt - 1] : persist[row], finish[row], big ? LOCAL_BLOCK_BIG : LOCAL_BLOCK, row};
 }
 
 inline int narrow_local_pass(RadixWorkspace& ws, NarrowWorkspace& nw, hipStream_t stream, const u32* keys_in, const u32* vals_in,
@@ -1177,7 +1222,7 @@
         if (fr < 0) return fr;
         with_flags = (fr == 0) && l.dir.dir && l.dir.dbits >= 8 + rb && l.dir.dbits - 8 - rb <= bb && l.dir.dbits - 8 <= lo_bits;
     }
-    const LocalKernels k = local_kernels(big, with_flags, bb);
+    const LocalKernels k = local_kernels(big, with_flags, bb, nw.nt_mask);
     u32 pgrid = 0;
     if (nw.local_persist && (rc = nw.persist_grid(reinterpret_cast<const void*>(k.persist), k.block, k.row, nsub, &pgrid))) return rc;
     rc = ws.timed_pass(stream, 3, n, (u64)n * 16u + (vals_out64 ? (u64)n * 8u : 0u), [&] {
@@ -1288,7 +1333,7 @@
     const int lo_bits = 56 - begin_bit;
     u32* const k32A = reinterpret_cast<u32*>(keysA);
     u32* const k32B = reinterpret_cast<u32*>(keysB);
-    SA_HIP_CHECK(hipMemsetAsync(nw.tickets, 0, (size_t)NARROW_MAX_PASSES * NCHUNK * sizeof(u32), stream));
+    SA_HIP_CHECK(hipMemsetAsync(nw.zero_arena, 0, NarrowWorkspace::zero_arena_bytes(), stream));
     const bool try_split = nw.split_enabled && keep_narrow && ws.block == 512 && lo_bits - LOCAL_BIN_BITS >= 1;
     const bool optimistic = try_split && src && nw.top_claims;
     if ((rc = narrow_top_digit(ws, nw, stream, keysA, k32B, valsB, n, begin_bit, src, optimistic))) return rc;
diff --git a/suffixarray_amd/csrc/radix_split.hpp b/suffixarray_amd/csrc/radix_split.hpp
--- a/suffixarray_amd/csrc/radix_split.hpp
+++ b/suffixarray_amd/csrc/radix_split.hpp
@@ -19,7 +19,7 @@
 
 template <int BLOCK, int ITEMS>
 __global__ __launch_bounds__(BLOCK) void split_hist_kernel(const u32* __restrict__ keys, const SegPlan* __restrict__ plan, int shift,
-                                                           u32 mask, u32* __restrict__ hist, u32 tiles_per_block) {
+                                                           u32 mask, u32* __restrict__ hist, u32 tiles_per_block, u32 nt) {
     constexpr u32 TILE = BLOCK * ITEMS;
     constexpr int CS = SPLIT_NB + 1;
     __shared__ u32 s_h[SPLIT_HIST_COPIES * CS];
@@ -51,8 +51,10 @@
         const u32 len = (end - start) < TILE ? (end - start) : TILE;
         if (len == TILE) {
             u32 k[ITEMS];
-#pragma unroll
-            for (int j = 0; j < ITEMS; ++j) k[j] = keys[start + j * BLOCK + threadIdx.x];
+            with_nt(nt != 0, [&](auto NT) {
+#pragma unroll
+                for (int j = 0; j < ITEMS; ++j) k[j] = ld_stream<decltype(NT)::value>(keys + start + j * BLOCK + threadIdx.x);
+            });
 #pragma unroll
             for (int j = 0; j < ITEMS; ++j) atomicAdd(&my[(k[j] >> shift) & mask], 1u);
         } else {
@@ -120,7 +122,7 @@
     u32* cursor;
 };
 
-template <bool FULL, int BLOCK, int ITEMS>
+template <bool FULL, int BLOCK, int ITEMS, bool NT>
 __device__ __forceinline__ void split_tile(const SplitPassArgs& a, const u32 bucket, const u32 start, const u32 tile_n,
                                            u32* s_keys, u32* s_cnt, u32* s_gdelta, u32* s_wsum) {
     static_assert(SPLIT_NB == 2 * BLOCK, "two bins per thread");
@@ -134,7 +136,7 @@
 #pragma unroll
     for (int j = 0; j < ITEMS; ++j) {
         const u32 p = woff + j * WAVE;
-        key[j] = (FULL || p < tile_n) ? kin[p] : 0u;
+        key[j] = (FULL || p < tile_n) ? ld_stream<NT>(kin + p) : 0u;
     }
     u32 pos[ITEMS];
 #pragma unroll
@@ -189,7 +191,7 @@
 #pragma unroll
     for (int j = 0; j < ITEMS; ++j) {
         const u32 p = woff + j * WAVE;
-        val[j] = (FULL || p < tile_n) ? vin[p] : 0u;
+        val[j] = (FULL || p < tile_n) ? ld_stream<NT>(vin + p) : 0u;
     }
     __syncthreads();
     u32* s_vals = s_keys;
@@ -204,7 +206,7 @@
     }
 }
 
-template <int BLOCK, int ITEMS>
+template <int BLOCK, int ITEMS, bool NT = false>
 __global__ __launch_bounds__(BLOCK, 4) void seg_split_kernel(SplitPassArgs a) {
     constexpr u32 TILE = BLOCK * ITEMS;
     __shared__ __attribute__((aligned(16))) u32 s_keys[TILE];
@@ -245,8 +247,8 @@
     const u32 first_flat = s_t[bucket];
     const u32 start = s_b[bucket] + (flat - first_flat) * TILE;
     const u32 rest = s_b[bucket + 1] - start;
-    if (rest >= TILE) split_tile<true, BLOCK, ITEMS>(a, bucket, start, TILE, s_keys, s_cnt, s_gdelta, s_wsum);
-    else split_tile<false, BLOCK, ITEMS>(a, bucket, start, rest, s_keys, s_cnt, s_gdelta, s_wsum);
+    if (rest >= TILE) split_tile<true, BLOCK, ITEMS, NT>(a, bucket, start, TILE, s_keys, s_cnt, s_gdelta, s_wsum);
+    else split_tile<false, BLOCK, ITEMS, NT>(a, bucket, start, rest, s_keys, s_cnt, s_gdelta, s_wsum);
 }
 
 struct LocalArgs {
@@ -271,7 +273,7 @@
     void* ctx = nullptr;
 };
 
-template <int BB, bool FLAGS, int BLOCK, bool PERSIST, typename Mid>
+template <int BB, bool FLAGS, int BLOCK, bool PERSIST, bool NTS, typename Mid>
 __device__ __forceinline__ void local_finish_sub(const LocalArgs& a, const u32 sb, const u32 s, const u32 m, u32 (&key)[LOCAL_ITEMS],
                                                  u32 (&val)[LOCAL_ITEMS], u64* s_rec, u32* s_cw, u32* s_wsum, Mid&& mid) {
     constexpr int ITEMS = LOCAL_ITEMS;
@@ -390,9 +392,9 @@
             const u64 x = s_rec[p];
             const u32 k = (u32)(x >> 32);
             if (p < m) {
-                a.keys_out[s + p] = k;
-                a.vals_out[s + p] = (u32)x;
-                if (a.vals_out64) a.vals_out64[s + p] = (int64_t)(u32)x;
+                st_stream<NTS>(a.keys_out + s + p, k);
+                st_stream<NTS>(a.vals_out + s + p, (u32)x);
+                if (a.vals_out64) st_stream<NTS>(a.vals_out64 + s + p, (int64_t)(u32)x);
             }
             if (FLAGS && !(SA_ABL & 2)) {
                 const u32 kn = (u32)__builtin_amdgcn_update_dpp((int)~k, (int)k, 0x101, 0xF, 0xF, false);
@@ -409,7 +411,7 @@
     }
 }
 
-template <int BLOCK>
+template <int BLOCK, bool NTL>
 __device__ __forceinline__ void local_load(const LocalArgs& a, const u32 s, const u32 m, u32 (&key)[LOCAL_ITEMS], u32 (&val)[LOCAL_ITEMS]) {
     const u32* kin = a.keys_in + s;
     const u32* vin = a.vals_in + s;
@@ -417,7 +419,7 @@
     for (int j = 0; j < LOCAL_ITEMS; ++j) {
         const u32 p = (u32)j * BLOCK + threadIdx.x;
         key[j] = 0; val[j] = 0;
-        if ((u32)j * BLOCK < m && p < m) { key[j] = kin[p]; val[j] = vin[p]; }
+        if ((u32)j * BLOCK < m && p < m) { key[j] = ld_stream<NTL>(kin + p); val[j] = ld_stream<NTL>(vin + p); }
     }
 }
 
@@ -464,8 +466,8 @@
     for (int i = 0; i < WPT; ++i) s_cw[WPT * threadIdx.x + i] = 0;
     __syncthreads();
     u32 key[LOCAL_ITEMS], val[LOCAL_ITEMS];
-    local_load<BLOCK>(a, s, m, key, val);
-    local_finish_sub<BB, FLAGS, BLOCK, false>(a, sb, s, m, key, val, s_rec, s_cw, s_wsum, [] {});
+    local_load<BLOCK, false>(a, s, m, key, val);
+    local_finish_sub<BB, FLAGS, BLOCK, false, false>(a, sb, s, m, key, val, s_rec, s_cw, s_wsum, [] {});
 }
 
 __device__ __forceinline__ u32 wave_lower_bound(const u32* __restrict__ sub, const u32 nsub, const u64 t) {
@@ -483,7 +485,7 @@
     return lo;
 }
 
-template <int BB, bool FLAGS, int BLOCK = LOCAL_BLOCK>
+template <int BB, bool FLAGS, int BLOCK = LOCAL_BLOCK, u32 NT = 0>
 __global__ __launch_bounds__(BLOCK, 4) void local_persist_kernel(LocalArgs a, const u32* __restrict__ sub, u32 nsub, u32* ticket, u32 run) {
     constexpr u32 CAP = (u32)BLOCK * LOCAL_ITEMS;
     constexpr int NB = 1 << BB, WORDS = NB / 2, WPT = WORDS / BLOCK;
@@ -541,12 +543,13 @@
     u32 key[LOCAL_ITEMS], val[LOCAL_ITEMS];
     u32 s = 0, m = 0;
     u32 i = next(0, s, m);
-    if (i < nsub) local_load<BLOCK>(a, s, m, key, val);
+    constexpr bool NTL = (NT & NT_LOCAL_LOAD) != 0, NTS = (NT & NT_LOCAL_STORE) != 0;
+    if (i < nsub) local_load<BLOCK, NTL>(a, s, m, key, val);
     while (i < nsub) {
         u32 ns = 0, nm = 0;
         const u32 nx = next(i + 1, ns, nm);
-        local_finish_sub<BB, FLAGS, BLOCK, true>(a, i, s, m, key, val, s_rec, s_cw, s_wsum, [&] {
-            if (nx < nsub) local_load<BLOCK>(a, ns, nm, key, val);
+        local_finish_sub<BB, FLAGS, BLOCK, true, NTS>(a, i, s, m, key, val, s_rec, s_cw, s_wsum, [&] {
+            if (nx < nsub) local_load<BLOCK, NTL>(a, ns, nm, key, val);
         });
         i = nx; s = ns; m = nm;
     }
diff --git a/suffixarray_amd/csrc/sa_build.hpp b/suffixarray_amd/csrc/sa_build.hpp
--- a/suffixarray_amd/csrc/sa_build.hpp
+++ b/suffixarray_amd/csrc/sa_build.hpp
@@ -20,8 +20,22 @@
 
 
 constexpr int HIST_COPIES = 8;
+constexpr int BYTE_HIST_UNROLL = 4;
+constexpr u32 BYTE_HIST_PER_BLOCK = 256u * 16u * BYTE_HIST_UNROLL;
+__device__ __forceinline__ void byte_hist_count(u32* my, const uint4 x) {
+    const u32 w[4] = {x.x, x.y, x.z, x.w};
+#pragma unroll
+    for (int k = 0; k < 4; ++k) {
+        atomicAdd(&my[w[k] & 255u], 1u);
+        atomicAdd(&my[(w[k] >> 8) & 255u], 1u);
+        atomicAdd(&my[(w[k] >> 16) & 255u], 1u);
+        atomicAdd(&my[w[k] >> 24], 1u);
+    }
+}
+template <bool NT>
 __global__ __launch_bounds__(256) void byte_hist_kernel(const u8* __restrict__ text, u64 n, u64* __restrict__ hist) {
     constexpr int CS = 257;
+    constexpr int U = BYTE_HIST_UNROLL;
     __shared__ u32 s_h[HIST_COPIES * CS];
     for (int i = threadIdx.x; i < HIST_COPIES * CS; i += 256) s_h[i] = 0;
     __syncthreads();
@@ -29,17 +43,15 @@
     const u64 nvec = n / 16;
     const uint4* v = reinterpret_cast<const uint4*>(text);
     const u64 stride = (u64)gridDim.x * blockDim.x;
-    for (u64 i = (u64)blockIdx.x * blockDim.x + threadIdx.x; i < nvec; i += stride) {
-        const uint4 x = v[i];
-        const u32 w[4] = {x.x, x.y, x.z, x.w};
-#pragma unroll
-        for (int k = 0; k < 4; ++k) {
-            atomicAdd(&my[w[k] & 255u], 1u);
-            atomicAdd(&my[(w[k] >> 8) & 255u], 1u);
-            atomicAdd(&my[(w[k] >> 16) & 255u], 1u);
-            atomicAdd(&my[w[k] >> 24], 1u);
-        }
-    }
+    u64 i = (u64)blockIdx.x * blockDim.x + threadIdx.x;
+    for (; i + (U - 1) * stride < nvec; i += U * stride) {
+        uint4 x[U];
+#pragma unroll
+        for (int u = 0; u < U; ++u) x[u] = load_stream<NT>(v + i + u * stride);
+#pragma unroll
+        for (int u = 0; u < U; ++u) byte_hist_count(my, x[u]);
+    }
+    for (; i < nvec; i += stride) byte_hist_count(my, load_stream<NT>(v + i));
     if (blockIdx.x == 0) {
         for (u64 i = nvec * 16 + threadIdx.x; i < n; i += blockDim.x) atomicAdd(&my[text[i]], 1u);
     }
@@ -950,6 +962,9 @@
     u64 freq[256];
     sa_hip_build_stats stats;
     hipEvent_t ev_begin = nullptr, ev_end = nullptr;
+    hipStream_t side = nullptr;
+    hipEvent_t ev_fork = nullptr, ev_join = nullptr;
+    bool touch_forked = false;
     int chunk_rounds_before_doubling = 2;
     bool adaptive_doubling = true;
     int initial_chars_override = 0;
@@ -1072,6 +1087,9 @@
         if ((rc = narrow.init())) return rc;
         SA_HIP_CHECK(hipEventCreate(&ev_begin));
         SA_HIP_CHECK(hipEventCreate(&ev_end));
+        SA_HIP_CHECK(hipStreamCreateWithFlags(&side, hipStreamNonBlocking));
+        SA_HIP_CHECK(hipEventCreateWithFlags(&ev_fork, hipEventDisableTiming));
+        SA_HIP_CHECK(hipEventCreateWithFlags(&ev_join, hipEventDisableTiming));
         memset(&stats, 0, sizeof stats);
         memset(freq, 0, sizeof freq);
         return 0;
@@ -1101,6 +1119,12 @@
         if (ev_begin) (void)hipEventDestroy(ev_begin);
         if (ev_end) (void)hipEventDestroy(ev_end);
         ev_begin = ev_end = nullptr;
+        if (side) { (void)hipStreamSynchronize(side); (void)hipStreamDestroy(side); }
+        if (ev_fork) (void)hipEventDestroy(ev_fork);
+        if (ev_join) (void)hipEventDestroy(ev_join);
+        side = nullptr;
+        ev_fork = ev_join = nullptr;
+        touch_forked = false;
         if (mbox) (void)hipHostFree(mbox);
         mbox = nullptr;
     }
@@ -1109,22 +1133,30 @@
         n = n_;
         SA_HIP_CHECK(hipMemsetAsync(text.as<u8>() + n, 0, TEXT_PAD + 16, stream));
         u64* dh = small.as<u64>();
-        SA_HIP_CHECK(hipMemsetAsync(dh, 0, 256 * sizeof(u64), stream));
-        if (n) hipLaunchKernelGGL(byte_hist_kernel, dim3(stream_grid(n, 256 * 64)), dim3(256), 0, stream, text.as<u8>(), n, dh);
-        static_assert(sizeof freq == 2048, "mailbox layout");
-        SA_HIP_CHECK(hipMemcpyAsync(mbox + MB_FREQ, dh, sizeof freq, hipMemcpyDeviceToHost, stream));
+        SA_HIP_CHECK(hipMemsetAsync(dh, 0, 4096, stream));
         u32 pilot_dups = 0;
         pilot_dup_share = 0.0;
         const bool run_pilot = use_pilot && n >= (u64)16 * PILOT_SAMPLES;
         if (run_pilot) {
             int rc = pilot.ensure((size_t)PILOT_SLOTS * 8 + 64);
             if (rc) return rc;
-            SA_HIP_CHECK(hipMemsetAsync(pilot.p, 0, (size_t)PILOT_SLOTS * 8 + 64, stream));
+            SA_HIP_CHECK(hipEventRecord(ev_fork, stream));
+            SA_HIP_CHECK(hipStreamWaitEvent(side, ev_fork, 0));
+            SA_HIP_CHECK(hipMemsetAsync(pilot.p, 0, (size_t)PILOT_SLOTS * 8 + 64, side));
             u32* pd = reinterpret_cast<u32*>(pilot.as<u8>() + (size_t)PILOT_SLOTS * 8);
-            hipLaunchKernelGGL(pilot_kernel, dim3(PILOT_SAMPLES / 256), dim3(256), 0, stream, text.as<u8>(), n, 8,
+            hipLaunchKernelGGL(pilot_kernel, dim3(PILOT_SAMPLES / 256), dim3(256), 0, side, text.as<u8>(), n, 8,
                                pilot.as<unsigned long long>(), pd);
-            SA_HIP_CHECK(hipMemcpyAsync(mbox + MB_PILOT, pd, 4, hipMemcpyDeviceToHost, stream));
-        }
+            SA_HIP_CHECK(hipMemcpyAsync(mbox + MB_PILOT, pd, 4, hipMemcpyDeviceToHost, side));
+            SA_HIP_CHECK(hipEventRecord(ev_join, side));
+        }
+        if (n) {
+            const u32 grid = narrow.hist_grid_force ? narrow.hist_grid_force : stream_grid(n, BYTE_HIST_PER_BLOCK);
+            if (narrow.nt_mask & NT_TEXT) hipLaunchKernelGGL(byte_hist_kernel<true>, dim3(grid), dim3(256), 0, stream, text.as<u8>(), n, dh);
+            else hipLaunchKernelGGL(byte_hist_kernel<false>, dim3(grid), dim3(256), 0, stream, text.as<u8>(), n, dh);
+        }
+        static_assert(sizeof freq == 2048, "mailbox layout");
+        SA_HIP_CHECK(hipMemcpyAsync(mbox + MB_FREQ, dh, sizeof freq, hipMemcpyDeviceToHost, stream));
+        if (run_pilot) SA_HIP_CHECK(hipStreamWaitEvent(stream, ev_join, 0));
         SA_HIP_CHECK(hipStreamSynchronize(stream));
         memcpy(freq, mbox + MB_FREQ, sizeof freq);
         if (run_pilot) memcpy(&pilot_dups, mbox + MB_PILOT, 4);
@@ -1258,13 +1290,11 @@
         d.gap_cap = dir_gap_cap(nb);
         d.gap_count = reinterpret_cast<u32*>(b->small.as<u8>() + 3584);
         d.dstat = b->radix.dstat;
-        SA_HIP_CHECK(hipMemsetAsync(d.gap_count, 0, 4, b->stream));
         b->lite.sa = nullptr;
         b->lite.st_pos = b->lite_stage.as<u32>();
         b->lite.st_idx = b->lite.st_pos + (size_t)nsub * LITE_CAP;
         b->lite.st_head = reinterpret_cast<u8*>(b->lite.st_idx + (size_t)nsub * LITE_CAP);
         b->lite.overflow = b->totals_dev() + 2;
-        SA_HIP_CHECK(hipMemsetAsync(b->lite.overflow, 0, 4, b->stream));
         SA_HIP_CHECK(hipMemsetAsync(b->counts.p, 0, (size_t)nsub * sizeof(uint2), b->stream));
         b->split_dir = d;
         b->lite_tiles = nsub;
@@ -1277,8 +1307,9 @@
         dir_ready = true;
         dir_by_local_pass = true;
         lite_nk = nk;
-        int rc = scan_counts(lite_tiles, totals_host);
+        int rc = fork_dir_touch();
         if (rc) return rc;
+        if ((rc = scan_counts(lite_tiles, totals_host))) return rc;
         *overflow = lite_overflow_seen != 0;
         return 0;
     }
@@ -1370,14 +1401,36 @@
         return qdir.ensure(dir_gap_offset(nb) + (size_t)dir_gap_cap(nb) * sizeof(uint4));
     }
 
+    void launch_dir_touch(hipStream_t s) {
+        const u64 n16 = ((1ull << q_dbits) + 1) / 4;
+        hipLaunchKernelGGL(dir_touch_kernel, dim3(stream_grid(n16, 256)), dim3(256), 0, s, qdir.as<uint4>(), n16,
+                           reinterpret_cast<u32*>(small.as<u8>() + 3588));
+    }
+    static bool dir_touch_wanted() {
+        if (const char* e = diag_env("SA_HIP_DIR_TOUCH")) return atoi(e) != 0;
+        return true;
+    }
+    int fork_dir_touch() {
+        if (!dir_touch_wanted()) return 0;
+        SA_HIP_CHECK(hipEventRecord(ev_fork, stream));
+        SA_HIP_CHECK(hipStreamWaitEvent(side, ev_fork, 0));
+        launch_dir_touch(side);
+        SA_HIP_CHECK(hipEventRecord(ev_join, side));
+        touch_forked = true;
+        return 0;
+    }
+    int join_side() {
+        if (touch_forked) SA_HIP_CHECK(hipStreamWaitEvent(stream, ev_join, 0));
+        touch_forked = false;
+        return 0;
+    }
+
     int build_directory() {
         if ((!qkeys && !qkeys32) || n < 2) { qkeys = nullptr; qkeys32 = nullptr; k2_ready = false; return 0; }
         if (qkeys32 && !dir_ready) return fail(SA_HIP_EINTERNAL, "narrow keys without a fused directory");
         if (dir_ready) {
-            const u64 n16 = ((1ull << q_dbits) + 1) / 4;
-            if (const char* e = diag_env("SA_HIP_DIR_TOUCH")) { if (atoi(e) == 0) return 0; }
-            hipLaunchKernelGGL(dir_touch_kernel, dim3(stream_grid(n16, 256)), dim3(256), 0, stream, qdir.as<uint4>(), n16,
-                               reinterpret_cast<u32*>(small.as<u8>() + 3588));
+            if (touch_forked || !dir_touch_wanted()) return 0;
+            launch_dir_touch(stream);
             return 0;
         }
         int rc = directory_layout(n);
@@ -1644,6 +1697,7 @@
         stats.n = n_;
         if (n_ > n_max) return fail(SA_HIP_EINVAL, "text longer than the index capacity");
         if ((rc = ensure_build_buffers())) return rc;
+        if ((rc = join_side())) return rc;
         SA_HIP_CHECK(hipEventRecord(ev_begin, stream));
         CodeMap map;
         u32 sigma = 0;
@@ -1907,6 +1961,8 @@
     }
 
     int finish_stats() {
+        int rcj = join_side();
+        if (rcj) return rcj;
         SA_HIP_CHECK(hipEventRecord(ev_end, stream));
         SA_HIP_CHECK(hipEventSynchronize(ev_end));
         float ms = 0.f;
```

Result: no change. 78.84 billion, median of 6 (+0.5%).
